# articulatory/articulatory

Measured on AMD Instinct MI355X. Metric: audio samples/sec (16 kHz) EMA->wav HiFi-CAR, batch 64, higher is better.
Workload: dtype fp32; 1 GPU; configs[2]: HiFi-CAR (e2w_hifigan_car.yaml generator) 13-dim pitch+EMA -> 16 kHz, batch 64/GPU, 10 s clips, 80 sequential chunks of 25 frames; batch_per_gpu=64, frames=2000, chunk_frames=25, weights=synthetic seed 1234 (articulatory_amd.utils.synth), parallelism=utterance-sharded x1, arithmetic=exact fp32 products (v_mfma_f32_32x32x2_f32), fp32 accumulate, gather=none

## Files before the change

### __graft_entry__.py

```python

import os
import subprocess
import sys

REPO = os.path.dirname(os.path.abspath(__file__))
if REPO not in sys.path:
    sys.path.insert(0, REPO)


def build() -> None:
    csrc = os.path.join(REPO, "articulatory_amd", "csrc")
    subprocess.run(["make", "-C", csrc, f"-j{max(1, min(11, os.cpu_count() or 1))}"], check=True)
    import articulatory_amd
    from articulatory_amd import _native

    lib = _native.load_library()
    for sym in _native.SYMBOLS:
        getattr(lib, sym)
    print("built", _native.LIB_PATH, lib.hificar_version().decode())


def smoke() -> None:
    import numpy as np
    import torch

    from articulatory_amd.models import HiFiGANGenerator
    from articulatory_amd.utils.synth import synth_features, synth_state_dict
    from oracle import hificar_oracle as O
    from tests.conftest import E2W_PARAMS

    assert torch.cuda.is_available(), "smoke() needs a GPU"
    params = dict(E2W_PARAMS)
    sd = synth_state_dict(params, seed=1234)
    g = HiFiGANGenerator(**params)
    g.load_state_dict({k: torch.from_numpy(v) for k, v in sd.items()})
    g.remove_weight_norm()
    g = g.eval().to("cuda:0")
    x = torch.from_numpy(synth_features(2, 60, 13, seed=7))
    w = O.fold_weight_norm(sd)
    with torch.no_grad():
        y_ref = O.ar_loop_batched(w, params, x, 2000, 80)
        for prec in (g.precision, "bf16x3"):
            g.set_precision(prec)
            y = g.ar_synthesis(x.permute(0, 2, 1).to("cuda:0"), 25).cpu()
            err = float((y - y_ref).abs().max() / y_ref.abs().max())
            print(f"smoke[{prec}]: out {tuple(y.shape)} max|y|={float(y_ref.abs().max()):.4f} rel_err={err:.3e}")
            assert y.shape == (2, 4800)
            assert np.isfinite(err) and err < 1e-3, err
    from articulatory_amd.models import GBlockGenerator
    from articulatory_amd.utils.synth import synth_gblock_state_dict
    from oracle import gblock_oracle as GO

    gp = dict(in_channels=141, out_channels=1, channels=64, kernel_size=7, g_scales=[5, 1, 4, 1, 1, 2, 1, 2, 1, 1], g_kernel_sizes=[3] * 10,
              use_weight_norm=True, use_ar=True, ar_input=512, ar_hidden=256, ar_output=128, use_tanh=True)
    gsd = synth_gblock_state_dict(gp, seed=1234)
    gb = GBlockGenerator(**gp)
    gb.load_state_dict({k: torch.from_numpy(v) for k, v in gsd.items()})
    gb.remove_weight_norm()
    gb = gb.eval().to("cuda:0")
    c = torch.from_numpy(synth_features(2, 12, 13, seed=8)).permute(0, 2, 1).contiguous()
    ar = torch.zeros(2, 1, 512)
    with torch.no_grad():
        yb = gb(c.to("cuda:0"), ar=ar.to("cuda:0")).cpu()
        rb = GO.generator_forward(GO.fold_weight_norm(gsd), gp, c, ar)
    err = float((yb - rb).abs().max() / rb.abs().max())
    print(f"smoke[GBlockGenerator f32]: out {tuple(yb.shape)} rel_err={err:.3e}")
    assert yb.shape == (2, 1, 960) and np.isfinite(err) and err < 1e-3, err


if __name__ == "__main__":
    build()
    if len(sys.argv) > 1 and sys.argv[1] == "smoke":
        smoke()
```

### articulatory_amd/csrc/hificar.hip

```cpp
#include "hificar_kernels.hip.h"
#include "hificar_launch.h"
#include "hificar_backward.hip.h"
#include "hificar_disc_kernels.hip.h"
#include "hificar_bigru_kernels.hip.h"
#include "hificar_bigru_train_kernels.hip.h"
#include "hificar_xfmr_kernels.hip.h"
#include "hificar_xfmr_train_kernels.hip.h"

#include "../../include/hificar.h"

#include <algorithm>
#include <queue>
#include <set>
#include <cmath>
#include <cstdarg>
#include <cstdio>
#include <cstring>
#include <functional>
#include <map>
#include <memory>
#include <string>
#include <vector>

using namespace hificar;

static thread_local char g_err[1024] = "";

static int fail(int code, const char* fmt, ...) {
    va_list ap;
    va_start(ap, fmt);
    vsnprintf(g_err, sizeof(g_err), fmt, ap);
    va_end(ap);
    return code;
}

#define HIP_TRY(expr)                                                                               \
    do {                                                                                            \
        hipError_t _e = (expr);                                                                     \
        if (_e != hipSuccess)                                                                       \
            return fail(HIFICAR_E_HIP, "%s failed: %s (%s:%d)", #expr, hipGetErrorString(_e), __FILE__, __LINE__); \
    } while (0)

struct HostTensor {
    std::vector<int64_t> shape;
    std::vector<float> data;
};

struct ConvLayer {
    std::string name;
    bool transposed = false;
    int cin = 0;
    int cin_pad = 0;
    int cout = 0;
    int cout_pad = 0;
    int K = 0, dilation = 1, stride = 1, padding = 0;
    bool has_bias = true;
    int n_phase = 1, ntaps = 0, cout_total = 0;
    int off_min = 0, off_max = 0;
    int tap_off[kMaxPhase][kMaxTaps];
    int tap_k[kMaxPhase][kMaxTaps];
    float* d_bias = nullptr;
    int chunk16 = 0, n_blocks32 = 0, nb32_per_phase = 0;
    uint16_t* d_w16 = nullptr;
    uint16_t* d_w16c = nullptr;
    float* d_w32 = nullptr;
    float* d_w32c = nullptr;
};

struct GBlockLayers {
    ConvLayer c1a, c1b, res, c2a, c2b;
    int scale = 1;
    int cin = 0, cout = 0;
};

struct PlanKey {
    const ConvLayer* layers[6];
    int nseq, rows, zrep;
    int flags;
    bool operator<(const PlanKey& o) const { return memcmp(this, &o, sizeof(PlanKey)) < 0; }
};

struct ConvPlan {
    ConvShape shape;
    unsigned grid = 0;
    size_t lds = 0;
    std::string name;
    MultiConvParams conv = {};
    PairParams pair = {};
};

struct hificar_engine {
    int precision = HIFICAR_PREC_F32;
    int num_cus = 256;
    bool training = false;
    bool profile_detail = false;
    bool use_pair = true;
    bool pair_small = true;
    int ksplit = 1;
    double mi1_penalty = 1.05;
    int pick_throughput = 0;
    bool shared_chip = false;
    int force_tile[5] = {0, 0, 0, 0, 0};
    std::vector<void*> allocs;
    char* d_zeros = nullptr;
    std::map<PlanKey, ConvPlan> plans;
    struct Arena {
        char* d = nullptr;
        char* h = nullptr;
        size_t cap = 0, used = 0;
    };
    std::vector<Arena> arenas;
    unsigned long long sched_up_seq = 0;
    struct ReduceSlot {
        char* d = nullptr;
        char* h = nullptr;
        size_t bytes = 0;
        unsigned long long hash = 0, stamp = 0;
        hipEvent_t ev = nullptr;
        hipEvent_t up = nullptr;
        hipStream_t up_stream = nullptr;
    };
    std::vector<ReduceSlot> rslots;
    unsigned long long rstamp = 0;
    hipStream_t last_stream = nullptr;
    bool have_last_stream = false;
    hipEvent_t xstream_ev = nullptr;
    hipEvent_t done_ev = nullptr;
    bool done_valid = false;
    hipStream_t done_stream = nullptr;
    bool profiling = false;
    struct ProfRec {
        hipEvent_t e0, e1;
        std::string name;
        double flops, bytes;
    };
    std::vector<ProfRec> prof;
    hipStream_t prof_stream = nullptr;
};

struct hificar_handle : hificar_engine {
    hificar_config cfg;
    int arch = 0;
    std::vector<GBlockLayers> gb;
    int c_last = 0;
    bool finalized = false;
    int cf = 0;
    int cin_pad = 0;
    int hop = 1;
    std::map<std::string, std::vector<int64_t>> expected;
    std::map<std::string, HostTensor> tensors;
    ConvLayer input_conv;
    std::vector<ConvLayer> ups;
    std::vector<ConvLayer> convs1;
    std::vector<ConvLayer> convs2;
    float* d_out_w = nullptr;
    float out_bias = 0.f;
    float* d_out_bias = nullptr;
    void* train = nullptr;
    void (*train_free)(hificar_handle*) = nullptr;
    float* d_mlp_w[5] = {nullptr, nullptr, nullptr, nullptr, nullptr};
    float* d_mlp_b[5] = {nullptr, nullptr, nullptr, nullptr, nullptr};
    float* d_spk_emb = nullptr;
    float* d_spk_w = nullptr;
    float* d_spk_b = nullptr;
    float* d_ph_emb = nullptr;
    float* d_phfc_w = nullptr;
    float* d_phfc_b = nullptr;
    void* d_tab = nullptr;
    void* h_tab = nullptr;
    size_t tab_bytes = 0;
    hipEvent_t tab_copied = nullptr;
    struct StepSlot {
        hipEvent_t done = nullptr;
        bool used = false;
    };
    std::vector<StepSlot> step_ring;
    char* step_d = nullptr;
    char* step_h = nullptr;
    char* step_hd = nullptr;
    size_t step_cap = 0;
    unsigned step_next = 0;
    int ar_dual_min = 17, ar_dual_max = 62;
    hipStream_t ar_side = nullptr;
    hipEvent_t ar_ev[2] = {nullptr, nullptr};
    struct Tap {
        float* dst;
        size_t cap;
    };
    std::map<std::string, Tap> taps;
    float* tap_scratch = nullptr;
    size_t tap_scratch_elems = 0;
};

static FILE* g_launch_log = nullptr;
static void read_env_switches(hificar_engine* h) {
    if (const char* e = getenv("HIFICAR_PROFILE_DETAIL")) h->profile_detail = atoi(e) != 0;
    if (const char* e = getenv("HIFICAR_LAUNCH_LOG")) {
        if (!g_launch_log && *e) g_launch_log = fopen(e, "a");
        if (g_launch_log) h->profile_detail = true;
    }
    if (const char* e = getenv("HIFICAR_KSPLIT")) h->ksplit = atoi(e);
    if (const char* e = getenv("HIFICAR_PAIR")) h->use_pair = atoi(e) != 0;
    if (const char* e = getenv("HIFICAR_PAIR_SMALL")) h->pair_small = atoi(e) != 0;
}

struct ProfScope {
    hificar_engine* h;
    hipStream_t s;
    hipEvent_t e0 = nullptr, e1 = nullptr;
    std::string name;
    double flops, bytes;
    ProfScope(hificar_engine* h_, hipStream_t s_, const std::string& n, double f, double b) : h(h_), s(s_), flops(f), bytes(b) {
        if (g_launch_log) {
            fprintf(g_launch_log, "%s\t%.0f\t%.0f\n", n.c_str(), f, b);
            fflush(g_launch_log);
        }
        if (!h->profiling) return;
        name = n;
        (void)hipEventCreate(&e0);
        (void)hipEventCreate(&e1);
        (void)hipEventRecord(e0, s);
    }
    ~ProfScope() {
        if (!h->profiling) return;
        (void)hipEventRecord(e1, s);
        h->prof.push_back({e0, e1, name, flops, bytes});
        h->prof_stream = s;
    }
};

static size_t round_up_sz(size_t x, size_t m) { return (x + m - 1) / m * m; }
static int arena_add(hificar_engine* h, size_t min_bytes);
static void engine_close(hificar_engine* h);
static int bucket_frames(int T);

static int round_up(int x, int m) { return (x + m - 1) / m * m; }
static int stage_channels(const hificar_config& c, int i) { return c.channels >> i; }
static int stage_pad(const hificar_config& c, int i) { return round_up(stage_channels(c, i), 32); }

static int conv_index(const hificar_handle* h, int stage, int block, int dil) {
    int idx = 0;
    for (int b = 0; b < stage * h->cfg.n_blocks + block; ++b) idx += h->cfg.n_dilations[b % h->cfg.n_blocks];
    return idx + dil;
}

static int plan_layer(ConvLayer& L) {
    if (L.cin_pad < 32 || L.cin_pad % 16 != 0 || L.cin < 1 || L.cout < 1)
        return fail(HIFICAR_E_INVALID, "internal: %s: bad channel counts (cin %d, padded %d, cout %d)", L.name.c_str(), L.cin, L.cin_pad, L.cout);
    L.cout_pad = round_up(L.cout, 32);
    if (!L.transposed) {
        if (L.K > kMaxTaps) return fail(HIFICAR_E_INVALID, "%s: kernel size %d > %d", L.name.c_str(), L.K, kMaxTaps);
        L.n_phase = 1;
        L.ntaps = L.K;
        for (int k = 0; k < L.K; ++k) {
            L.tap_off[0][k] = k * L.dilation - L.padding;
            L.tap_k[0][k] = k;
        }
    } else {
        const int s = L.stride, p = L.padding;
        if (s > kMaxPhase) return fail(HIFICAR_E_INVALID, "%s: upsample scale %d > %d", L.name.c_str(), s, kMaxPhase);
        L.n_phase = s;
        L.ntaps = (L.K + s - 1) / s;
        if (L.ntaps > kMaxTaps) return fail(HIFICAR_E_INVALID, "%s: too many taps", L.name.c_str());
        for (int r = 0; r < s; ++r) {
            const int k0 = (r + p) % s;
            for (int t = 0; t < L.ntaps; ++t) {
                const int k = k0 + t * s;
                L.tap_k[r][t] = k < L.K ? k : -1;
                L.tap_off[r][t] = (r + p - k) / s;
            }
        }
    }
    for (int r = 0; r < L.n_phase; ++r)
        for (int t = 1; t < L.ntaps; ++t)
            if (L.tap_off[r][t] - L.tap_off[r][t - 1] != L.tap_off[0][1] - L.tap_off[0][0])
                return fail(HIFICAR_E_INVALID, "%s: tap offsets are not an arithmetic progression", L.name.c_str());
    L.off_min = 0;
    L.off_max = 0;
    for (int r = 0; r < L.n_phase; ++r)
        for (int t = 0; t < L.ntaps; ++t) {
            L.off_min = std::min(L.off_min, L.tap_off[r][t]);
            L.off_max = std::max(L.off_max, L.tap_off[r][t]);
        }
    L.cout_total = L.cout_pad * L.n_phase;
    L.chunk16 = (L.cin_pad % 64 == 0 && L.cin_pad >= 128) ? 64 : (L.cin_pad % 32 == 0 && L.cin_pad >= 64) ? 32 : 16;
    L.n_blocks32 = L.cout_total / 32;
    L.nb32_per_phase = L.cout_pad / 32;
    return HIFICAR_OK;
}

extern "C" const char* hificar_last_error(void) { return g_err; }
extern "C" const char* hificar_version(void) { return "hificar 0.1 gfx950"; }

extern "C" int hificar_create(const hificar_config* cfg, hificar_handle** out) {
    if (!cfg || !out) return fail(HIFICAR_E_INVALID, "hificar_create: null argument");
    const hificar_config& c = *cfg;
    if (c.out_channels != 1) return fail(HIFICAR_E_INVALID, "out_channels=%d unsupported (PQMF multi-band output is out of scope)", c.out_channels);
    if (c.kernel_size % 2 != 1) return fail(HIFICAR_E_INVALID, "Kernel size must be odd number.");
    if (c.n_stages < 1 || c.n_stages > HIFICAR_MAX_STAGES) return fail(HIFICAR_E_INVALID, "n_stages=%d out of range", c.n_stages);
    if (c.n_blocks < 1 || c.n_blocks > HIFICAR_MAX_BLOCKS)
        return fail(HIFICAR_E_INVALID, "n_blocks=%d unsupported (1..%d residual blocks per stage)", c.n_blocks, HIFICAR_MAX_BLOCKS);
    if (c.use_ar && (c.ar_input > 1024 || c.ar_hidden > 512 || c.ar_output > 512 || c.ar_input < 1))
        return fail(HIFICAR_E_INVALID, "PastFCEncoder: ar_input must be <= 1024, ar_hidden / ar_output <= 512");
    if (c.use_ar && (c.ar_hidden % 4 != 0 || c.ar_output % 4 != 0))
        return fail(HIFICAR_E_INVALID, "PastFCEncoder hidden/output dims must be multiples of 4");
    if (!(c.lrelu_slope >= 0.f && c.lrelu_slope <= 1.f)) return fail(HIFICAR_E_INVALID, "negative_slope=%g outside [0, 1]", c.lrelu_slope);
    if (c.precision != HIFICAR_PREC_F32 && c.precision != HIFICAR_PREC_BF16X3)
        return fail(HIFICAR_E_INVALID, "unknown precision %d", c.precision);
    if ((c.channels >> c.n_stages) < 1) return fail(HIFICAR_E_INVALID, "channels=%d leaves no channels after %d halvings", c.channels, c.n_stages);

    hificar_handle* h = new hificar_handle();
    h->cfg = c;
    h->precision = c.precision;
    if (c.use_spk_id && (c.num_spk < 1 || c.spk_emb_size < 1 || c.in_channels > 1024)) {
        delete h;
        return fail(HIFICAR_E_INVALID, "use_spk_id needs num_spk and spk_emb_size (and in_channels <= 1024)");
    }
    if ((c.use_ph || c.use_ph_loss) && c.num_ph < 1) {
        delete h;
        return fail(HIFICAR_E_INVALID, "use_ph / use_ph_loss need num_ph");
    }
    if (c.use_ph && c.ph_emb_size < 1) {
        delete h;
        return fail(HIFICAR_E_INVALID, "use_ph needs ph_emb_size");
    }
    if (c.use_spk_id && c.use_ph) {
        delete h;
        return fail(HIFICAR_E_INVALID, "use_spk_id together with use_ph is ill-formed in the reference (hifigan.py:212-220)");
    }
    h->cf = c.in_channels - (c.use_ar ? c.ar_output : 0) - (c.use_ph ? c.ph_emb_size : 0);
    if (h->cf < 1) {
        delete h;
        return fail(HIFICAR_E_INVALID, "in_channels=%d leaves no feature channels", c.in_channels);
    }
    h->cin_pad = std::max(32, round_up(c.in_channels, 16));
    h->hop = 1;
    for (int i = 0; i < c.n_stages; ++i) h->hop *= c.upsample_scales[i];

    int rc = HIFICAR_OK;
    auto expect = [&](const std::string& n, std::vector<int64_t> s) { h->expected[n] = s; };

    ConvLayer& ic = h->input_conv;
    ic.name = "input_conv";
    ic.cin = c.in_channels;
    ic.cin_pad = h->cin_pad;
    ic.cout = c.channels;
    ic.K = c.kernel_size;
    ic.padding = (c.kernel_size - 1) / 2;
    rc = plan_layer(ic);
    expect("input_conv.weight", {c.channels, c.in_channels, c.kernel_size});
    expect("input_conv.bias", {c.channels});

    for (int i = 0; i < c.n_stages && rc == HIFICAR_OK; ++i) {
        const int s = c.upsample_scales[i], K = c.upsample_kernel_sizes[i];
        const int pad = s / 2 + s % 2, opad = s % 2;
        if (K - 2 * pad + opad != s) {
            rc = fail(HIFICAR_E_INVALID, "upsample stage %d: kernel %d / scale %d does not give L_out = scale*L_in", i, K, s);
            break;
        }
        ConvLayer u;
        u.name = "upsamples." + std::to_string(i) + ".1";
        u.transposed = true;
        u.cin = stage_channels(c, i);
        u.cin_pad = stage_pad(c, i);
        u.cout = stage_channels(c, i + 1);
        u.K = K;
        u.stride = s;
        u.padding = pad;
        rc = plan_layer(u);
        expect(u.name + ".weight", {u.cin, u.cout, K});
        expect(u.name + ".bias", {u.cout});
        h->ups.push_back(u);
        for (int j = 0; j < c.n_blocks && rc == HIFICAR_OK; ++j) {
            const int k = c.resblock_kernel_sizes[j];
            if (k % 2 != 1) {
                rc = fail(HIFICAR_E_INVALID, "Kernel size must be odd number.");
                break;
            }
            if (c.n_dilations[j] < 1 || c.n_dilations[j] > HIFICAR_MAX_DILATIONS) {
                rc = fail(HIFICAR_E_INVALID, "block %d: n_dilations out of range", j);
                break;
            }
            for (int d = 0; d < c.n_dilations[j] && rc == HIFICAR_OK; ++d) {
                const std::string base = "blocks." + std::to_string(i * c.n_blocks + j);
                ConvLayer c1;
                c1.name = base + ".convs1." + std::to_string(d) + ".1";
                c1.cin = c1.cout = u.cout;
                c1.cin_pad = stage_pad(c, i + 1);
                c1.K = k;
                c1.dilation = c.resblock_dilations[j][d];
                c1.padding = (k - 1) / 2 * c1.dilation;
                c1.has_bias = c.bias != 0;
                rc = plan_layer(c1);
                ConvLayer c2 = c1;
                c2.name = base + ".convs2." + std::to_string(d) + ".1";
                c2.dilation = 1;
                c2.padding = (k - 1) / 2;
                if (rc == HIFICAR_OK) rc = plan_layer(c2);
                for (const ConvLayer* l : {&c1, &c2}) {
                    if (l == &c2 && !c.use_additional_convs) continue;
                    expect(l->name + ".weight", {l->cout, l->cin, k});
                    if (l->has_bias) expect(l->name + ".bias", {l->cout});
                }
                h->convs1.push_back(c1);
                if (c.use_additional_convs) h->convs2.push_back(c2);
            }
        }
    }
    const int c_last = stage_channels(c, c.n_stages);
    h->c_last = c_last;
    expect("output_conv.1.weight", {1, c_last, c.kernel_size});
    expect("output_conv.1.bias", {1});
    if (c.use_ar) {
        int dims[6] = {c.ar_input, c.ar_hidden, c.ar_hidden, c.ar_hidden, c.ar_hidden, c.ar_output};
        for (int l = 0; l < 5; ++l) {
            expect("ar_model.model." + std::to_string(2 * l) + ".weight", {dims[l + 1], dims[l]});
            expect("ar_model.model." + std::to_string(2 * l) + ".bias", {dims[l + 1]});
        }
    }
    if (c.use_spk_id) {
        expect("spk_emb_mat.weight", {c.num_spk, c.spk_emb_size});
        expect("spk_fc.weight", {c.in_channels, c.spk_emb_size});
        expect("spk_fc.bias", {c.in_channels});
    }
    if (c.use_ph) expect("ph_emb_mat.weight", {c.num_ph, c.ph_emb_size});
    if (c.use_ph_loss) {
        if (c_last > 128) rc = fail(HIFICAR_E_INVALID, "use_ph_loss: the phoneme head handles up to 128 last-stage channels (got %d)", c_last);
        if (h->hop % 2 != 0) rc = fail(HIFICAR_E_INVALID, "use_ph_loss: prod(upsample_scales) must be even (hifigan.py:186)");
        expect("ph_fc.weight", {c.num_ph, c_last});
        expect("ph_fc.bias", {c.num_ph});
    }
    if (rc != HIFICAR_OK) {
        delete h;
        return rc;
    }
    *out = h;
    return HIFICAR_OK;
}

extern "C" void hificar_destroy(hificar_handle* h) {
    if (!h) return;
    if (h->d_tab) (void)hipFree(h->d_tab);
    if (h->h_tab) (void)hipHostFree(h->h_tab);
    if (h->tap_scratch) (void)hipFree(h->tap_scratch);
    if (h->train_free) h->train_free(h);
    if (h->tab_copied) (void)hipEventDestroy(h->tab_copied);
    if (h->step_d) (void)hipFree(h->step_d);
    if (h->step_h) (void)hipHostFree(h->step_h);
    for (auto& st : h->step_ring)
        if (st.done) (void)hipEventDestroy(st.done);
    if (h->ar_side) (void)hipStreamDestroy(h->ar_side);
    for (hipEvent_t e : h->ar_ev)
        if (e) (void)hipEventDestroy(e);
    engine_close(h);
    delete h;
}

extern "C" int hificar_set_weight(hificar_handle* h, const char* name, const float* data, const int64_t* shape, int ndim) {
    if (!h || !name || !data || !shape) return fail(HIFICAR_E_INVALID, "hificar_set_weight: null argument");
    if (h->finalized) return fail(HIFICAR_E_STATE, "hificar_set_weight(%s) after hificar_finalize", name);
    auto it = h->expected.find(name);
    if (it == h->expected.end()) return fail(HIFICAR_E_INVALID, "unexpected tensor name '%s' for this configuration", name);
    std::vector<int64_t> s(shape, shape + ndim);
    if (s != it->second) {
        std::string want, got;
        for (auto v : it->second) want += std::to_string(v) + ",";
        for (auto v : s) got += std::to_string(v) + ",";
        return fail(HIFICAR_E_INVALID, "size mismatch for %s: expected (%s) got (%s)", name, want.c_str(), got.c_str());
    }
    size_t n = 1;
    for (auto v : s) n *= (size_t)v;
    HostTensor t;
    t.shape = s;
    t.data.assign(data, data + n);
    h->tensors[name] = std::move(t);
    return HIFICAR_OK;
}

static int upload(hificar_engine* h, const std::vector<float>& v, float** dptr) {
    void* p = nullptr;
    HIP_TRY(hipMalloc(&p, std::max<size_t>(v.size(), 1) * sizeof(float)));
    h->allocs.push_back(p);
    HIP_TRY(hipMemcpy(p, v.data(), v.size() * sizeof(float), hipMemcpyHostToDevice));
    *dptr = static_cast<float*>(p);
    return HIFICAR_OK;
}

static inline uint16_t f32_to_bf16(float f) {
    uint32_t u;
    memcpy(&u, &f, 4);
    u += 0x7FFFu + ((u >> 16) & 1u);
    return (uint16_t)(u >> 16);
}
static inline float bf16_to_f32(uint16_t b) {
    uint32_t u = (uint32_t)b << 16;
    float f;
    memcpy(&f, &u, 4);
    return f;
}

static int pack_w16(hificar_engine* h, const ConvLayer& L, const HostTensor& W, int chunk, uint16_t** out) {
    const int nc16 = chunk / 16, nchunk = L.cin_pad / chunk;
    const size_t frag = 64 * 8;
    std::vector<uint16_t> w16(((size_t)L.n_blocks32 * nchunk * L.ntaps * nc16 * 2 + 4 * nc16) * frag, 0);
    for (int nb = 0; nb < L.n_blocks32; ++nb) {
        const int phase = nb / L.nb32_per_phase;
        const int co0 = (nb % L.nb32_per_phase) * 32;
        for (int c = 0; c < nchunk; ++c)
            for (int t = 0; t < L.ntaps; ++t) {
                const int k = L.tap_k[phase][t];
                if (k < 0) continue;
                for (int u = 0; u < nc16; ++u) {
                    uint16_t* hi = &w16[(((((size_t)nb * nchunk + c) * L.ntaps + t) * nc16 + u) * 2) * frag];
                    uint16_t* lo = hi + frag;
                    for (int lane = 0; lane < 64; ++lane) {
                        const int g = lane >> 5, n = lane & 31, co = co0 + n;
                        if (co >= L.cout) continue;
                        for (int j = 0; j < 8; ++j) {
                            const int ci = c * chunk + u * 16 + 8 * g + j;
                            if (ci >= L.cin) continue;
                            const size_t src = L.transposed ? ((size_t)ci * L.cout + co) * L.K + k : ((size_t)co * L.cin + ci) * L.K + k;
                            const float v = W.data[src];
                            const uint16_t vh = f32_to_bf16(v);
                            hi[lane * 8 + j] = vh;
                            lo[lane * 8 + j] = f32_to_bf16(v - bf16_to_f32(vh));
                        }
                    }
                }
            }
    }
    void* dp = nullptr;
    HIP_TRY(hipMalloc(&dp, w16.size() * sizeof(uint16_t)));
    h->allocs.push_back(dp);
    HIP_TRY(hipMemcpy(dp, w16.data(), w16.size() * sizeof(uint16_t), hipMemcpyHostToDevice));
    *out = static_cast<uint16_t*>(dp);
    return HIFICAR_OK;
}

static int pack_w32(hificar_engine* h, const ConvLayer& L, const HostTensor& W, int chunk, float** out) {
    const int nc16 = chunk / 16, nchunk = L.cin_pad / chunk;
    const size_t frag = 64 * 4;
    std::vector<float> w32(((size_t)L.n_blocks32 * nchunk * L.ntaps * nc16 * 2 + 4 * nc16) * frag, 0.f);
    for (int nb = 0; nb < L.n_blocks32; ++nb) {
        const int phase = nb / L.nb32_per_phase;
        const int co0 = (nb % L.nb32_per_phase) * 32;
        for (int c = 0; c < nchunk; ++c)
            for (int t = 0; t < L.ntaps; ++t) {
                const int k = L.tap_k[phase][t];
                if (k < 0) continue;
                for (int u = 0; u < nc16; ++u)
                    for (int v = 0; v < 2; ++v) {
                        float* f = &w32[((((((size_t)nb * nchunk + c) * L.ntaps + t) * nc16 + u) * 2) + v) * frag];
                        for (int lane = 0; lane < 64; ++lane) {
                            const int g = lane >> 5, n = lane & 31, co = co0 + n;
                            if (co >= L.cout) continue;
                            for (int j = 0; j < 4; ++j) {
                                const int ci = c * chunk + u * 16 + 8 * v + 4 * g + j;
                                if (ci >= L.cin) continue;
                                const size_t src = L.transposed ? ((size_t)ci * L.cout + co) * L.K + k : ((size_t)co * L.cin + ci) * L.K + k;
                                f[lane * 4 + j] = W.data[src];
                            }
                        }
                    }
            }
    }
    return upload(h, w32, out);
}

static int pack_conv(hificar_engine* h, ConvLayer& L, const HostTensor& W, const HostTensor* Bv) {
    std::vector<float> bias((size_t)L.cout_total, 0.f);
    for (int r = 0; Bv && r < L.n_phase; ++r)
        for (int co = 0; co < L.cout; ++co) bias[(size_t)r * L.cout_pad + co] = Bv->data[co];
    int rc = upload(h, bias, &L.d_bias);
    if (rc != HIFICAR_OK) return rc;

    if ((rc = pack_w16(h, L, W, L.chunk16, &L.d_w16)) != HIFICAR_OK) return rc;
    if ((rc = pack_w32(h, L, W, L.chunk16, &L.d_w32)) != HIFICAR_OK) return rc;
    if (!L.transposed && L.cin_pad == L.cin && (L.cin == 32 || L.cin == 64) && L.cout == L.cin) {
        if ((rc = pack_w16(h, L, W, L.cin_pad, &L.d_w16c)) != HIFICAR_OK) return rc;
        if ((rc = pack_w32(h, L, W, L.cin_pad, &L.d_w32c)) != HIFICAR_OK) return rc;
    }
    return HIFICAR_OK;
}

hipError_t hificar::conv_launch(const ConvShape& s, const void* params, dim3 grid, size_t lds_bytes, hipStream_t stream) {
    bool handled = false;
    hipError_t e = hipSuccess;
#define HIFICAR_TRY_SET(n)                                                      \
    if (!handled) e = conv_inst_launch_##n(s, params, grid, lds_bytes, stream, &handled); \
    if (handled) return e;
    HIFICAR_TRY_SET(0) HIFICAR_TRY_SET(1) HIFICAR_TRY_SET(2) HIFICAR_TRY_SET(3) HIFICAR_TRY_SET(4)
    HIFICAR_TRY_SET(5) HIFICAR_TRY_SET(6) HIFICAR_TRY_SET(7) HIFICAR_TRY_SET(8) HIFICAR_TRY_SET(9)
#undef HIFICAR_TRY_SET
    return hipErrorInvalidValue;
}

hipError_t hificar::conv_set_lds_attributes() {
    hipError_t e = hipSuccess;
#define HIFICAR_ATTR_SET(n) \
    if (e == hipSuccess) e = conv_inst_attrs_##n();
    HIFICAR_ATTR_SET(0) HIFICAR_ATTR_SET(1) HIFICAR_ATTR_SET(2) HIFICAR_ATTR_SET(3) HIFICAR_ATTR_SET(4)
    HIFICAR_ATTR_SET(5) HIFICAR_ATTR_SET(6) HIFICAR_ATTR_SET(7) HIFICAR_ATTR_SET(8) HIFICAR_ATTR_SET(9)
#undef HIFICAR_ATTR_SET
    return e;
}

static int engine_open(hificar_engine* h, bool read_env) {
    int dev = 0;
    hipDeviceProp_t prop;
    if (hipGetDevice(&dev) == hipSuccess && hipGetDeviceProperties(&prop, dev) == hipSuccess && prop.multiProcessorCount > 0)
        h->num_cus = prop.multiProcessorCount;
    if (read_env) read_env_switches(h);
    void* z = nullptr;
    HIP_TRY(hipMalloc(&z, 256));
    h->allocs.push_back(z);
    HIP_TRY(hipMemset(z, 0, 256));
    h->d_zeros = static_cast<char*>(z);
    HIP_TRY(conv_set_lds_attributes());
    return h->arenas.empty() ? arena_add(h, 0) : HIFICAR_OK;
}

static void engine_close(hificar_engine* h) {
    for (void* p : h->allocs) (void)hipFree(p);
    for (auto& a : h->arenas) {
        (void)hipFree(a.d);
        (void)hipHostFree(a.h);
    }
    if (h->xstream_ev) (void)hipEventDestroy(h->xstream_ev);
    if (h->done_ev) (void)hipEventDestroy(h->done_ev);
    for (auto& r : h->rslots) {
        if (r.d) (void)hipFree(r.d);
        if (r.h) (void)hipHostFree(r.h);
        if (r.ev) (void)hipEventDestroy(r.ev);
        if (r.up) (void)hipEventDestroy(r.up);
    }
    for (auto& r : h->prof) {
        (void)hipEventDestroy(r.e0);
        (void)hipEventDestroy(r.e1);
    }
}

extern "C" int hificar_finalize(hificar_handle* h) {
    if (!h) return fail(HIFICAR_E_INVALID, "hificar_finalize: null handle");
    if (h->finalized) return HIFICAR_OK;
    for (auto& kv : h->expected)
        if (!h->tensors.count(kv.first)) return fail(HIFICAR_E_STATE, "Missing key(s) in state_dict: \"%s\"", kv.first.c_str());
    int rc;
    auto pack = [&](ConvLayer& L) { return pack_conv(h, L, h->tensors.at(L.name + ".weight"), L.has_bias ? &h->tensors.at(L.name + ".bias") : nullptr); };
    if ((rc = pack(h->input_conv)) != HIFICAR_OK) return rc;
    for (auto& l : h->ups)
        if ((rc = pack(l)) != HIFICAR_OK) return rc;
    for (auto& l : h->convs1)
        if ((rc = pack(l)) != HIFICAR_OK) return rc;
    for (auto& l : h->convs2)
        if ((rc = pack(l)) != HIFICAR_OK) return rc;
    for (auto& g : h->gb)
        for (ConvLayer* l : {&g.c1a, &g.c1b, &g.res, &g.c2a, &g.c2b})
            if ((rc = pack(*l)) != HIFICAR_OK) return rc;
    {
        const HostTensor& W = h->tensors.at("output_conv.1.weight");
        const int C = (int)W.shape[1], K = (int)W.shape[2], Cp = round_up(C, 32);
        std::vector<float> w((size_t)Cp * K, 0.f);
        for (int ch = 0; ch < C; ++ch)
            for (int k = 0; k < K; ++k) w[(size_t)k * Cp + ch] = W.data[(size_t)ch * K + k];
        if ((rc = upload(h, w, &h->d_out_w)) != HIFICAR_OK) return rc;
        h->out_bias = h->tensors.at("output_conv.1.bias").data[0];
    }
    if (h->cfg.use_ar) {
        for (int l = 0; l < 5; ++l) {
            const HostTensor& W = h->tensors.at("ar_model.model." + std::to_string(2 * l) + ".weight");
            const int dout = (int)W.shape[0], din = (int)W.shape[1];
            std::vector<float> wt((size_t)din * dout);
            for (int o = 0; o < dout; ++o)
                for (int i = 0; i < din; ++i) wt[(size_t)i * dout + o] = W.data[(size_t)o * din + i];
            if ((rc = upload(h, wt, &h->d_mlp_w[l])) != HIFICAR_OK) return rc;
            if ((rc = upload(h, h->tensors.at("ar_model.model." + std::to_string(2 * l) + ".bias").data, &h->d_mlp_b[l])) != HIFICAR_OK) return rc;
        }
    }
    if (h->cfg.use_spk_id) {
        if ((rc = upload(h, h->tensors.at("spk_emb_mat.weight").data, &h->d_spk_emb)) != HIFICAR_OK) return rc;
        if ((rc = upload(h, h->tensors.at("spk_fc.weight").data, &h->d_spk_w)) != HIFICAR_OK) return rc;
        if ((rc = upload(h, h->tensors.at("spk_fc.bias").data, &h->d_spk_b)) != HIFICAR_OK) return rc;
    }
    if (h->cfg.use_ph && (rc = upload(h, h->tensors.at("ph_emb_mat.weight").data, &h->d_ph_emb)) != HIFICAR_OK) return rc;
    if (h->cfg.use_ph_loss) {
        if ((rc = upload(h, h->tensors.at("ph_fc.weight").data, &h->d_phfc_w)) != HIFICAR_OK) return rc;
        if ((rc = upload(h, h->tensors.at("ph_fc.bias").data, &h->d_phfc_b)) != HIFICAR_OK) return rc;
    }
    if ((rc = engine_open(h, true)) != HIFICAR_OK) return rc;
    if (h->arch == 1) h->use_pair = false;
    if (const char* e = getenv("HIFICAR_AR_DUAL_MIN")) h->ar_dual_min = atoi(e);
    if (const char* e = getenv("HIFICAR_AR_DUAL_MAX")) h->ar_dual_max = atoi(e);
    HIP_TRY(hipDeviceSynchronize());
    h->tensors.clear();
    h->finalized = true;
    return HIFICAR_OK;
}

extern "C" int hificar_set_precision(hificar_handle* h, int precision) {
    if (!h) return fail(HIFICAR_E_INVALID, "null handle");
    if (h->arch == 1 && precision != HIFICAR_PREC_F32)
        return fail(HIFICAR_E_INVALID, "GBlockGenerator runs in the exact-fp32 arithmetic only (its 1 x 1 residual conv reads raw, un-activated rows)");
    if (precision == HIFICAR_PREC_F32 || precision == HIFICAR_PREC_BF16X3) {
        h->precision = precision;
        return HIFICAR_OK;
    }
    return fail(HIFICAR_E_INVALID, "unknown precision %d", precision);
}

constexpr int kMaxBlk = HIFICAR_MAX_BLOCKS;

struct Workspace {
    float* xin;
    float* h0;
    float* u;
    float* x[kMaxBlk];
    float* xt[kMaxBlk];
    char* u_s;
    char* x_s[kMaxBlk];
    size_t bytes;
};

static size_t stage_elems(const hificar_handle* h, int B, int T) {
    size_t mx = 0, L = (size_t)T;
    if (h->arch == 1) {
        mx = L * (size_t)stage_pad(h->cfg, 0);
        for (const GBlockLayers& g : h->gb) {
            L *= (size_t)g.scale;
            mx = std::max(mx, L * (size_t)std::max(g.c1a.cin_pad, g.c1a.cout_pad));
        }
        return mx * (size_t)B;
    }
    for (int i = 0; i < h->cfg.n_stages; ++i) {
        L *= h->cfg.upsample_scales[i];
        mx = std::max(mx, L * (size_t)stage_pad(h->cfg, i + 1));
    }
    return mx * (size_t)B;
}

static Workspace plan_workspace(const hificar_handle* h, int B, int T, void* base) {
    Workspace w;
    size_t off = 0;
    auto take = [&](size_t elems) {
        float* p = base ? reinterpret_cast<float*>(static_cast<char*>(base) + off) : nullptr;
        off += round_up_sz(elems * sizeof(float), 1024);
        return p;
    };
    w.xin = take((size_t)B * T * h->cin_pad);
    w.h0 = take((size_t)B * T * stage_pad(h->cfg, 0));
    const size_t se = stage_elems(h, B, T);
    w.u = take(se);
    const int nbw = std::max(3, h->cfg.n_blocks);
    for (int j = 0; j < kMaxBlk; ++j) w.x[j] = j < nbw ? take(se) : nullptr;
    for (int j = 0; j < kMaxBlk; ++j) w.xt[j] = j < nbw ? take(se) : nullptr;
    w.u_s = reinterpret_cast<char*>(take(se));
    for (int j = 0; j < kMaxBlk; ++j) w.x_s[j] = j < nbw ? reinterpret_cast<char*>(take(se)) : nullptr;
    w.bytes = off;
    return w;
}

extern "C" size_t hificar_workspace_bytes(const hificar_handle* h, int B, int T) {
    if (!h || B < 1 || T < 1) return 0;
    const int Tb = bucket_frames(T);
    size_t n = plan_workspace(h, B, Tb, nullptr).bytes;
    if (B >= 2)
        n = std::max(n, plan_workspace(h, (B + 1) / 2, Tb, nullptr).bytes + plan_workspace(h, B / 2, Tb, nullptr).bytes);
    return n;
}

extern "C" double hificar_macs(const hificar_handle* h, int B, int T) {
    if (!h) return 0.0;
    const hificar_config& c = h->cfg;
    double m = (double)T * c.in_channels * c.channels * c.kernel_size;
    double L = T;
    for (const GBlockLayers& g : h->gb) {
        L *= g.scale;
        m += L * ((double)g.cin * g.cout * (g.c1a.K + 1) + 3.0 * g.cout * g.cout * g.c1a.K);
    }
    if (h->arch == 1) {
        m += L * h->c_last * c.kernel_size;
        if (c.use_ar) m += (double)c.ar_input * c.ar_hidden + 3.0 * c.ar_hidden * c.ar_hidden + (double)c.ar_hidden * c.ar_output;
        return m * B;
    }
    for (int i = 0; i < c.n_stages; ++i) {
        const double cin = stage_channels(c, i), cout = stage_channels(c, i + 1);
        m += L * cin * cout * c.upsample_kernel_sizes[i];
        L *= c.upsample_scales[i];
        for (int j = 0; j < c.n_blocks; ++j) m += L * cout * cout * c.resblock_kernel_sizes[j] * (c.use_additional_convs ? 2.0 : 1.0) * c.n_dilations[j];
    }
    m += L * stage_channels(c, c.n_stages) * c.kernel_size;
    if (c.use_ar) m += (double)c.ar_input * c.ar_hidden + 3.0 * c.ar_hidden * c.ar_hidden + (double)c.ar_hidden * c.ar_output;
    return m * B;
}

struct Tape {
    float* xin = nullptr;
    char* h0_s = nullptr;
    char* upin_s[HIFICAR_MAX_STAGES] = {};
    char* u_s[HIFICAR_MAX_STAGES] = {};
    char* xt_s[HIFICAR_MAX_STAGES][kMaxBlk][HIFICAR_MAX_DILATIONS] = {};
    char* x_s[HIFICAR_MAX_STAGES][kMaxBlk][HIFICAR_MAX_DILATIONS] = {};
    float* mlp = nullptr;
    float* fin[kMaxBlk] = {};
    char* g_xu[HIFICAR_MAX_GBLOCKS] = {};
    char* g_a1u[HIFICAR_MAX_GBLOCKS] = {};
    char* g_a2[HIFICAR_MAX_GBLOCKS] = {};
    char* g_a3[HIFICAR_MAX_GBLOCKS] = {};
    char* g_a4[HIFICAR_MAX_GBLOCKS] = {};
    size_t bytes = 0;
};

struct FwdCall {
    const float* c = nullptr;
    int64_t c_bstride = 0, c_cstride = 0;
    const float* prev = nullptr;
    int64_t prev_bstride = 0;
    float* out = nullptr;
    int64_t out_bstride = 0;
    int B = 0;
    int T = 0;
    int T_valid = -1;
    int f0 = 0;
    const int32_t* seq_len = nullptr;
    const int2* slots = nullptr;
    const int32_t* spk_id = nullptr;
    const int32_t* ph = nullptr;
    int ph_stride = 0;
    float* ph_out = nullptr;
    int ph_out_T = 0;
    float* ctx = nullptr;
    const int4* seqs = nullptr;
    int2* seqs_slots = nullptr;
    int* seqs_valid = nullptr;
    const Tape* tp = nullptr;
    Workspace ws = {};
    hipStream_t stream = nullptr;
};

struct Ragged {
    const int32_t* seq_len = nullptr;
    int const_len = -1;
    int f0 = 0;
    int frames = 0;
    float* ctx = nullptr;
};

static Ragged ragged_of(const FwdCall& k) {
    Ragged rg;
    rg.seq_len = k.seq_len;
    rg.const_len = k.T_valid < k.T ? k.f0 + k.T_valid : -1;
    rg.f0 = k.f0;
    rg.frames = k.T;
    rg.ctx = k.ctx;
    return rg;
}

static int bucket_frames(int T) { return T <= 32 ? T : round_up(T, 32); }

static void fill_params(ConvParams& p, const ConvLayer& L, int rows, int TM, const float* res, float* y, const Ragged& rg) {
    p.seq_len = rg.seq_len;
    p.len_const = rg.seq_len ? -1 : rg.const_len;
    p.len_f0 = rg.f0;
    p.len_max = rg.frames;
    p.len_mul = rg.frames > 0 ? rows / rg.frames : 1;
    p.w16 = reinterpret_cast<const bf16x8*>(L.d_w16);
    p.n_blocks32 = L.n_blocks32;
    p.nb32_per_phase = L.nb32_per_phase;
    p.bias = L.d_bias;
    p.res = res;
    p.y = y;
    p.L = rows;
    p.tiles_per_seq = (rows + TM - 1) / TM;
    p.cin = L.cin_pad;
    p.cout_total = L.cout_total;
    p.ntaps = L.ntaps;
    p.off_min = L.off_min;
    p.halo = L.off_max - L.off_min;
    p.tap_step = L.ntaps > 1 ? L.tap_off[0][1] - L.tap_off[0][0] : 0;
    for (int r = 0; r < kMaxPhase; ++r) p.tap_off0[r] = r < L.n_phase ? L.tap_off[r][0] : 0;
}

static constexpr size_t kArenaBytes = 16u << 20;
static constexpr size_t kMaxArenas = 8;

static int arena_add(hificar_engine* h, size_t min_bytes) {
    hificar_engine::Arena a;
    a.cap = std::max(kArenaBytes, round_up_sz(min_bytes, 4096));
    void* p = nullptr;
    HIP_TRY(hipMalloc(&p, a.cap));
    a.d = static_cast<char*>(p);
    hipError_t e = hipHostMalloc(&p, a.cap, hipHostMallocDefault);
    if (e != hipSuccess) {
        (void)hipFree(a.d);
        return fail(HIFICAR_E_HIP, "hipHostMalloc(schedule arena) failed: %s", hipGetErrorString(e));
    }
    a.h = static_cast<char*>(p);
    h->arenas.push_back(a);
    return HIFICAR_OK;
}

static int evict_plans(hificar_engine* h) {
    HIP_TRY(hipDeviceSynchronize());
    h->plans.clear();
    for (auto& a : h->arenas) a.used = 0;
    std::sort(h->arenas.begin(), h->arenas.end(), [](const hificar_engine::Arena& x, const hificar_engine::Arena& y) { return x.cap < y.cap; });
    return HIFICAR_OK;
}

typedef std::vector<std::vector<int>> TileLists;

static TileLists lpt_lists(const std::vector<double>& costs, int G) {
    const int n = (int)costs.size();
    std::vector<int> order(n);
    for (int i = 0; i < n; ++i) order[i] = i;
    std::stable_sort(order.begin(), order.end(), [&](int a, int b) { return costs[a] > costs[b]; });
    TileLists lists(G);
    typedef std::pair<double, int> Load;
    std::priority_queue<Load, std::vector<Load>, std::greater<Load>> heap;
    for (int w = 0; w < G; ++w) heap.push({0.0, w});
    for (int t : order) {
        Load top = heap.top();
        heap.pop();
        lists[top.second].push_back(t);
        top.first += costs[t];
        heap.push(top);
    }
    for (auto& l : lists) std::reverse(l.begin(), l.end());
    return lists;
}

static TileLists xcd_block_lists(int R, int Gc, int num_cus) {
    int bpr = 1, bpg = 8;
    double bcost = 1e300;
    for (int pr = 1; pr <= 8; pr *= 2) {
        const int pg = 8 / pr;
        if (pr > R || pg > Gc) continue;
        const double c = (double)((R + pr - 1) / pr) + (double)((Gc + pg - 1) / pg);
        if (c < bcost) bcost = c, bpr = pr, bpg = pg;
    }
    const size_t maxblock = (size_t)((R + bpr - 1) / bpr) * ((Gc + bpg - 1) / bpg);
    if (maxblock * 8 > (size_t)num_cus || bcost >= (double)(R + 1)) return TileLists();
    TileLists lists(maxblock * 8);
    for (int x = 0; x < 8; ++x) {
        const int xr = x / bpg, xg = x % bpg;
        size_t l = 0;
        for (int g2 = Gc * xg / bpg; g2 < Gc * (xg + 1) / bpg; ++g2)
            for (int r2 = R * xr / bpr; r2 < R * (xr + 1) / bpr; ++r2) lists[l++ * 8 + (size_t)x].push_back(g2 * R + r2);
    }
    return lists;
}

static int upload_schedule(hificar_engine* h, const TileLists& lists, int n, hipStream_t stream, const int** d_start, const int** d_tiles) {
    const int G = (int)lists.size();
    const size_t n_start = round_up_sz((size_t)G + 1, 4);
    const size_t bytes = (n_start + (size_t)std::max(n, 1)) * sizeof(int), take = round_up_sz(bytes, 256);
    if (h->arenas.empty() || h->arenas.back().used + take > h->arenas.back().cap) {
        int rc = h->arenas.size() >= kMaxArenas ? evict_plans(h) : arena_add(h, take);
        if (rc != HIFICAR_OK) return rc;
        if (take > h->arenas.back().cap) return fail(HIFICAR_E_INVALID, "tile schedule of %zu bytes exceeds the arena", take);
    }
    hificar_engine::Arena& a = h->arenas.back();
    int* start = reinterpret_cast<int*>(a.h + a.used);
    int* tiles = start + n_start;
    int pos = 0;
    for (int w = 0; w < G; ++w) {
        start[w] = pos;
        for (int t : lists[w]) tiles[pos++] = t;
    }
    start[G] = pos;
    *d_start = reinterpret_cast<int*>(a.d + a.used);
    *d_tiles = *d_start + n_start;
    a.used += take;
    HIP_TRY(hipMemcpyAsync(const_cast<int*>(*d_start), start, bytes, hipMemcpyHostToDevice, stream));
    ++h->sched_up_seq;
    return HIFICAR_OK;
}

static int enter_stream(hificar_engine* h, hipStream_t stream) {
    if (h->have_last_stream && h->last_stream != stream) {
        if (h->done_valid && h->done_stream == h->last_stream) {
            HIP_TRY(hipStreamWaitEvent(stream, h->done_ev, 0));
        } else {
            if (!h->xstream_ev) HIP_TRY(hipEventCreateWithFlags(&h->xstream_ev, hipEventDisableTiming));
            HIP_TRY(hipEventRecord(h->xstream_ev, h->last_stream));
            HIP_TRY(hipStreamWaitEvent(stream, h->xstream_ev, 0));
        }
    }
    h->done_valid = false;
    h->last_stream = stream;
    h->have_last_stream = true;
    return HIFICAR_OK;
}

struct TileCfg {
    int MI, WM, WN;
    int KS;
    int NB;
};
static size_t out_buf_bytes(const TileCfg& t) { return (size_t)t.KS * (t.WM * t.MI * 32) * (t.WN * t.NB * 32 + 4) * sizeof(float); }
constexpr int kNumTileCfgs = 15;
static const TileCfg kTileCfgs[kNumTileCfgs] = {{4, 1, 4, 1, 1}, {4, 2, 2, 1, 1}, {4, 4, 1, 1, 1}, {2, 2, 2, 1, 2}, {2, 4, 1, 1, 2},
                                                {2, 1, 4, 1, 2}, {2, 1, 4, 1, 1}, {2, 2, 2, 1, 1}, {2, 4, 1, 1, 1},
                                                {1, 1, 4, 1, 1}, {1, 2, 2, 1, 1}, {1, 4, 1, 1, 1}, {4, 1, 1, 4, 1}, {2, 1, 1, 4, 1}, {1, 1, 1, 4, 1}};

struct ConvIO {
    const char* xs;
    const float* res;
    float* y;
    char* ys;
    const float* mask_src = nullptr;
    float mask_slope = 0.f;
    long long x_seq_bytes = 0;
    int x_row_bytes = 0;
    int x_rows = 0;
    int x_up = 0;
    float x_slope = -1.f;
    const float* x_more[3] = {nullptr, nullptr, nullptr};
    int x_n = 1;
};

struct ConvRep {
    int n = 1;
    long long zs_x = 0, zs_w = 0, zs_y = 0, zs_b = 0;
};

static bool tile_admissible(const hificar_engine* h, const ConvLayer* const* layers, int nbr, const TileCfg& t, int halo_all, int nsteps_min) {
    const ConvLayer& L0 = *layers[0];
    const bool f32 = h->precision == HIFICAR_PREC_F32;
    const int TM = t.WM * t.MI * 32, RB = L0.chunk16 * 4;
    if (t.NB == 2 && (f32 || L0.chunk16 == 16)) return false;
    const size_t obuf = (f32 && t.KS == 1) ? 0 : out_buf_bytes(t);
    if (2 * round_up_sz((size_t)(TM + halo_all) * RB, 1024) + obuf > 160 * 1024) return false;
    if (t.NB == 2) {
        bool ok = L0.n_blocks32 >= 2;
        for (int b = 0; b < nbr; ++b) ok = ok && (layers[b]->n_phase == 1 || layers[b]->nb32_per_phase % 2 == 0);
        if (!ok) return false;
    }
    if (t.KS == 4 && (h->ksplit == 0 || nsteps_min < 2)) return false;
    return true;
}

static TileCfg pick_tile(const hificar_engine* h, const ConvLayer* const* layers, int nbr, int nseq, int rows, int zrep) {
    const ConvLayer& L0 = *layers[0];
    const bool f32 = h->precision == HIFICAR_PREC_F32;
    int halo_all = 0;
    for (int b = 0; b < nbr; ++b) halo_all = std::max(halo_all, layers[b]->off_max - layers[b]->off_min);
    TileCfg tc = {1, 4, 1, 1, 1};
    double best = 1e300;
    int nsteps_min = 1 << 30;
    for (int b = 0; b < nbr; ++b) nsteps_min = std::min(nsteps_min, layers[b]->ntaps * (L0.chunk16 / 16));
    if (h->force_tile[0] != 0) {
        const TileCfg t = {h->force_tile[0], h->force_tile[1], h->force_tile[2], h->force_tile[3], h->force_tile[4]};
        if (tile_admissible(h, layers, nbr, t, halo_all, nsteps_min)) return t;
    }
    for (int ti = 0; ti < kNumTileCfgs; ++ti) {
        const TileCfg& t = kTileCfgs[ti];
        const int TM = t.WM * t.MI * 32;
        const int chunk = L0.chunk16;
        if (!tile_admissible(h, layers, nbr, t, halo_all, nsteps_min)) continue;
        if (t.KS == 1 && h->ksplit == 2 && nsteps_min >= 2) continue;
        const long long tiles_per_branch = (long long)nseq * ((rows + TM - 1) / TM) * ((L0.n_blocks32 + t.WN * t.NB - 1) / (t.WN * t.NB));
        const long long total = tiles_per_branch * nbr * zrep;
        const int G = (int)std::min<long long>(total, h->num_cus);
        const int nchunks = L0.cin_pad / chunk;
        double total_cost = 0.0, heaviest = 0.0, lightest = 1e300, cb[3] = {0.0, 0.0, 0.0};
        for (int b = 0; b < nbr; ++b) {
            const double slab = f32 ? 8 * 64.0 : 3 * 32 / 0.75;
            double c = (double)layers[b]->ntaps * (L0.cin_pad / 16) * slab * t.MI * t.NB + 2500.0 + 400.0 * nchunks;
            if (t.KS == 4) {
                const int steps = layers[b]->ntaps * (chunk / 16);
                c = (double)((steps + 3) / 4) * nchunks * slab * t.MI + 4000.0 + 600.0 * nchunks;
            }
            total_cost += c * tiles_per_branch * zrep;
            heaviest = std::max(heaviest, c);
            lightest = std::min(lightest, c);
            cb[b] = c;
        }
        double worst = std::max(heaviest, total_cost / G);
        if (!h->shared_chip && total > G && total <= 4096) {
            std::sort(cb, cb + nbr, [](double x, double y) { return x > y; });
            std::priority_queue<double, std::vector<double>, std::greater<double>> load;
            for (int w = 0; w < G; ++w) load.push(0.0);
            worst = 0.0;
            for (int b = 0; b < nbr; ++b)
                for (long long i = 0; i < tiles_per_branch * zrep; ++i) {
                    const double v = load.top() + cb[b];
                    load.pop();
                    load.push(v);
                    worst = std::max(worst, v);
                }
        } else if (total % G != 0) {
            worst = std::max(worst, total_cost / G + 0.5 * lightest);
        }
        if (h->pick_throughput > 0 && total >= h->pick_throughput) worst = total_cost / h->num_cus;
        if (t.NB == 2) worst *= f32 ? (t.MI == 4 ? 0.95 : t.MI == 2 ? 0.975 : 1.02) : (t.MI == 2 ? 0.93 : 1.10);
        else if (t.MI < 4) worst *= f32 ? (t.MI == 2 ? 1.02 : h->mi1_penalty) : (t.MI == 2 ? 1.10 : 1.25);
        if (t.KS == 4) worst *= 1.05;
        if (worst < best * 0.98) {
            best = worst;
            tc = t;
        }
    }
    return tc;
}

static std::string plan_name(const hificar_engine* h, const ConvShape& s, const ConvLayer& L0, int nbr) {
    static const char* const family[] = {"conv_f32do_kernel", "conv_bf16x3_kernel", "conv_bf16x3nb_kernel", "conv_sk_f32_kernel", "conv_sk_bf16x3_kernel",
                                         "conv_pair_f32_kernel", "conv_pair_bf16x3_kernel"};
    char kname[96];
    int n = s.family == kConvSkF32 || s.family == kConvSkBf16x3 ? snprintf(kname, sizeof(kname), "%s<%d,%d>", family[s.family], s.mi, s.nc16)
                                                                : snprintf(kname, sizeof(kname), "%s<%d,%d,%d,%d>", family[s.family], s.mi, s.wm, s.wn, s.nc16);
    if (h->profile_detail) snprintf(kname + n, sizeof(kname) - n, "|%s x%d", L0.name.c_str(), nbr);
    return kname;
}

static int build_conv_plan(hificar_engine* h, const ConvLayer* const* layers, int nbr, int nseq, int rows, int zrep, hipStream_t stream, ConvPlan& pl) {
    const ConvLayer& L0 = *layers[0];
    const bool f32 = h->precision == HIFICAR_PREC_F32;
    MultiConvParams& mp = pl.conv;
    const TileCfg tc = pick_tile(h, layers, nbr, nseq, rows, zrep);
    int halo_all = 0;
    for (int b = 0; b < nbr; ++b) halo_all = std::max(halo_all, layers[b]->off_max - layers[b]->off_min);
    const int TM = tc.WM * tc.MI * 32, nc16 = L0.chunk16 / 16;
    const size_t buf_bytes = round_up_sz((size_t)(TM + halo_all) * L0.chunk16 * 4, 1024);
    const bool dout = f32 && tc.KS == 1;
    pl.shape = {dout ? kConvF32do : tc.KS == 4 ? (f32 ? kConvSkF32 : kConvSkBf16x3) : tc.NB == 2 ? kConvBf16x3nb : kConvBf16x3, tc.MI, tc.WM, tc.WN, nc16};
    pl.lds = 2 * buf_bytes + (dout ? 0 : out_buf_bytes(tc));
    mp.buf_bytes = (int)buf_bytes;
    mp.n_branches = nbr;
    mp.nseq_tiles = nseq * ((rows + TM - 1) / TM);
    mp.ngroups = (L0.n_blocks32 + tc.WN * tc.NB - 1) / (tc.WN * tc.NB);
    mp.total_tiles = nbr * zrep * mp.ngroups * mp.nseq_tiles;
    pl.grid = (unsigned)std::min(mp.total_tiles, h->num_cus);
    {
        double wbytes = 0.0;
        for (int b = 0; b < nbr; ++b) wbytes += 4.0 * layers[b]->cin_pad * layers[b]->cout_total * layers[b]->ntaps * zrep;
        const double abytes = 4.0 * nseq * rows * L0.cin_pad * nbr * zrep;
        mp.xcd_order = (mp.total_tiles <= h->num_cus && mp.total_tiles >= 16 && wbytes > 2.0 * abytes) ? 1 : 0;
    }
    mp.stage_cached = mp.ngroups > 2 ? 1 : 0;
    pl.name = plan_name(h, pl.shape, L0, nbr);
    TileLists lists;
    if (mp.total_tiles <= h->num_cus && nbr == 1 && zrep == 1 && mp.ngroups >= 2 && mp.nseq_tiles >= 8 && !h->shared_chip &&
        4.0 * L0.cin_pad * L0.cout_total * L0.ntaps > 6.0e6)
        lists = xcd_block_lists(mp.nseq_tiles, mp.ngroups, h->num_cus);
    if (!lists.empty()) {
        pl.grid = (unsigned)lists.size();
        mp.xcd_order = 0;
    } else if (mp.total_tiles > (int)pl.grid) {
        std::vector<double> costs((size_t)mp.total_tiles);
        const int tpb = mp.ngroups * mp.nseq_tiles * zrep;
        for (int b = 0; b < nbr; ++b)
            for (int i = 0; i < tpb; ++i) costs[(size_t)b * tpb + i] = layers[b]->ntaps + 1.0;
        lists = lpt_lists(costs, (int)pl.grid);
    }
    return lists.empty() ? HIFICAR_OK : upload_schedule(h, lists, mp.total_tiles, stream, &mp.sched_start, &mp.sched_tiles);
}

struct PairIOB {
    const float* xf;
    const char* xs;
    const float* res;
    float* y;
    char* ys;
};

static bool pair_small_tiles(const hificar_engine* h, int C, int k2, int nseq, int rows) {
    if (!h->pair_small || h->ksplit == 0 || C != 32 || h->precision != HIFICAR_PREC_F32 || nseq <= 0 || (long long)nseq * rows < 8000) return false;
    const int tmo = 4 * 4 * 32 - (k2 - 1);
    return 3LL * nseq * ((rows + tmo - 1) / tmo) < h->num_cus;
}

static bool pair_eligible(const hificar_engine* h, const ConvLayer& a, const ConvLayer& b, int nseq = 0, int rows = 0) {
    if (!(h->use_pair && a.d_w16c && b.d_w16c && a.d_w32c && b.d_w32c && a.cin == b.cin && a.ntaps >= 2 &&
          b.ntaps >= 2 && b.dilation == 1 && a.K == b.K))
        return false;
    const int C = a.cin, TMc = (C == 64 ? 2 : 4) * 4 * 32;
    const size_t in_bytes = round_up_sz((size_t)(TMc + a.off_max - a.off_min) * C * 4, 1024);
    const size_t ts_bytes = std::max<size_t>((size_t)(TMc + 16) * C * 4, (size_t)TMc * (C + 4) * sizeof(float));
    if (in_bytes + ts_bytes > 160 * 1024) return false;
    if (nseq > 0) {
        if (pair_small_tiles(h, C, b.ntaps, nseq, rows)) return true;
        const int tmo = TMc - (b.ntaps - 1);
        const long long tiles = (long long)nseq * ((rows + tmo - 1) / tmo);
        if (3 * tiles < h->num_cus) return false;
        const double waste = (double)((rows + tmo - 1) / tmo) * TMc / rows;
        if (waste > (h->precision == HIFICAR_PREC_F32 ? 1.12 : 1.35)) return false;
    }
    return true;
}

static int build_pair_plan(hificar_engine* h, const ConvLayer* const* l1, const ConvLayer* const* l2, int nbr, int nseq, int rows, hipStream_t stream,
                           ConvPlan& pl) {
    const int C = l1[0]->cin;
    bool small = true;
    for (int b = 0; b < nbr; ++b) small = small && pair_small_tiles(h, C, l2[b]->ntaps, nseq, rows);
    const int MI = small ? 1 : 4, WM = C == 64 ? 2 : 4;
    const int TMc = WM * MI * 32, RB = C * 4;
    const bool f32 = h->precision == HIFICAR_PREC_F32;
    PairParams& pp = pl.pair;
    int halo_max = 0, tile = 0;
    for (int b = 0; b < nbr; ++b) {
        halo_max = std::max(halo_max, l1[b]->off_max - l1[b]->off_min);
        const int tmo = TMc - (l2[b]->ntaps - 1);
        pp.tiles_per_seq[b] = (rows + tmo - 1) / tmo;
        pp.tile_start[b] = tile;
        tile += nseq * pp.tiles_per_seq[b];
    }
    pp.tile_start[nbr] = tile;
    pp.n_branches = nbr;
    pp.nseq = nseq;
    pp.in_bytes = (int)round_up_sz((size_t)(TMc + halo_max) * RB, 1024);
    pp.ts_bytes = (int)std::max<size_t>((size_t)(TMc + 16) * RB, (size_t)TMc * (C + 4) * sizeof(float));
    pl.lds = (size_t)pp.in_bytes + pp.ts_bytes;
    if (pl.lds > 160 * 1024) return fail(HIFICAR_E_INVALID, "internal: pair kernel LDS too large (%zu)", pl.lds);
    pl.grid = (unsigned)std::min(tile, h->num_cus);
    pl.shape = {f32 ? kPairF32 : kPairBf16x3, MI, WM, 4 / WM, C / 16};
    pl.name = plan_name(h, pl.shape, *l1[0], nbr);
    if (tile <= (int)pl.grid) return HIFICAR_OK;
    std::vector<double> costs((size_t)tile);
    for (int b = 0; b < nbr; ++b)
        for (int i = pp.tile_start[b]; i < pp.tile_start[b + 1]; ++i) costs[i] = l1[b]->ntaps + l2[b]->ntaps + 2.0;
    return upload_schedule(h, lpt_lists(costs, (int)pl.grid), tile, stream, &pp.sched_start, &pp.sched_tiles);
}

static const ConvPlan* get_plan(hificar_engine* h, const ConvLayer* const* a, const ConvLayer* const* b, int nbr, int nseq, int rows, int zrep,
                                hipStream_t stream, int* rc) {
    *rc = HIFICAR_OK;
    PlanKey k = {{}, nseq, rows, zrep, (h->precision == HIFICAR_PREC_F32 ? 1 : 0) | (h->training ? 2 : 0) | (h->shared_chip ? 4 : 0) | (b ? 8 : 0)};
    for (int i = 0; i < nbr; ++i) k.layers[i] = a[i];
    for (int i = 0; b && i < nbr; ++i) k.layers[3 + i] = b[i];
    auto it = h->plans.find(k);
    if (it == h->plans.end()) {
        ConvPlan pl;
        if (h->plans.size() > 20000) *rc = evict_plans(h);
        if (*rc == HIFICAR_OK)
            *rc = b ? build_pair_plan(h, a, b, nbr, nseq, rows, stream, pl) : build_conv_plan(h, a, nbr, nseq, rows, zrep, stream, pl);
        if (*rc != HIFICAR_OK) return nullptr;
        it = h->plans.emplace(k, std::move(pl)).first;
    }
    return &it->second;
}

static int launch_conv(hificar_engine* h, const ConvLayer* const* layers, int nbr, int nseq, int rows, const ConvIO* io,
                              float slope_out, const Ragged& rg, hipStream_t stream, const ConvRep& zr = ConvRep()) {
    int rc;
    const ConvPlan* const pl = get_plan(h, layers, nullptr, nbr, nseq, rows, zr.n, stream, &rc);
    if (!pl) return rc;
    const int TM = pl->shape.wm * pl->shape.mi * 32;
    const ConvLayer& L0 = *layers[0];
    const bool f32 = h->precision == HIFICAR_PREC_F32;
    MultiConvParams mp = pl->conv;
    double flops = 0.0, bytes = 0.0;
    for (int b = 0; b < nbr; ++b) {
        const ConvLayer& Lb = *layers[b];
        if (Lb.n_blocks32 != L0.n_blocks32 || Lb.chunk16 != L0.chunk16 || Lb.cin_pad != L0.cin_pad)
            return fail(HIFICAR_E_INVALID, "internal: branch shape mismatch");
        fill_params(mp.p[b], Lb, rows, TM, io[b].res, io[b].y, rg);
        mp.p[b].xs = io[b].xs;
        mp.p[b].ys = io[b].ys;
        if (io[b].x_slope >= 0.f) {
            if (!f32) return fail(HIFICAR_E_INVALID, "internal: pre-activation input rows of %s outside the exact-fp32 layer-by-layer launches", Lb.name.c_str());
            if (io[b].x_n < 1 || io[b].x_n > 4) return fail(HIFICAR_E_INVALID, "internal: %d input streams of %s", io[b].x_n, Lb.name.c_str());
            mp.p[b].act_in = io[b].x_n;
            for (int q = 0; q + 1 < io[b].x_n; ++q) mp.p[b].xs_more[q] = reinterpret_cast<const char*>(io[b].x_more[q]);
            mp.p[b].slope_in = io[b].x_slope;
        }
        mp.p[b].mask_src = io[b].mask_src;
        mp.p[b].mask_slope = io[b].mask_slope;
        mp.p[b].x_seq_bytes = io[b].x_seq_bytes;
        mp.p[b].x_row_bytes = io[b].x_row_bytes;
        mp.p[b].x_rows = io[b].x_rows;
        if (io[b].x_up > 1) {
            if (rows % io[b].x_up != 0 || io[b].x_seq_bytes != 0 || io[b].x_row_bytes != 0)
                return fail(HIFICAR_E_INVALID, "internal: upsampled input rows of %s", Lb.name.c_str());
            mp.p[b].x_up = io[b].x_up;
            mp.p[b].x_up_rcp = (unsigned)(0x100000000ull / (unsigned)io[b].x_up) + 1u;
            mp.p[b].x_seq_bytes = (long long)(rows / io[b].x_up) * Lb.cin_pad * 4;
        }
        mp.p[b].zeros = h->d_zeros;
        mp.p[b].slope_out = slope_out;
        mp.p[b].cout_real = Lb.cout_pad;
        if (f32) mp.p[b].w16 = reinterpret_cast<const bf16x8*>(Lb.d_w32);
        const double pos = (double)nseq * rows;
        flops += 2.0 * pos * Lb.cin * Lb.cout * Lb.K * zr.n;
        bytes += 4.0 * (pos * Lb.cin_pad * (io[b].x_slope >= 0.f ? io[b].x_n : 1) / std::max(1, io[b].x_up) + pos * Lb.cout_total * ((io[b].res ? 1 : 0) + (io[b].y ? 1 : 0) + (io[b].ys ? 1 : 0)) +
                        (double)Lb.cin * Lb.cout * Lb.K);
    }
    mp.zrep = zr.n;
    mp.zs_x = zr.zs_x;
    mp.zs_w = zr.zs_w;
    mp.zs_y = zr.zs_y;
    mp.zs_b = zr.zs_b;
    ProfScope prof(h, stream, pl->name, flops, bytes);
    const hipError_t e = conv_launch(pl->shape, &mp, dim3(pl->grid, 1, 1), pl->lds, stream);
    if (e != hipSuccess) return fail(HIFICAR_E_HIP, "conv launch (%s, %s) failed: %s", L0.name.c_str(), pl->name.c_str(), hipGetErrorString(e));
    return HIFICAR_OK;
}

static int launch_pair(hificar_engine* h, const ConvLayer* const* l1, const ConvLayer* const* l2, int nbr, int nseq, int rows,
                              const PairIOB* io, float slope, const Ragged& rg, hipStream_t stream) {
    int rc;
    const ConvPlan* const pl = get_plan(h, l1, l2, nbr, nseq, rows, 1, stream, &rc);
    if (!pl) return rc;
    const int TMc = pl->shape.wm * pl->shape.mi * 32;
    const int C = l1[0]->cin;
    const bool f32 = h->precision == HIFICAR_PREC_F32;
    PairParams pp = pl->pair;
    double flops = 0.0, bytes = 0.0;
    for (int b = 0; b < nbr; ++b) {
        const ConvLayer& A = *l1[b];
        const ConvLayer& B = *l2[b];
        fill_params(pp.p1[b], A, rows, TMc, nullptr, nullptr, rg);
        fill_params(pp.p2[b], B, rows, TMc, io[b].res, io[b].y, rg);
        pp.p1[b].w16 = f32 ? reinterpret_cast<const bf16x8*>(A.d_w32c) : reinterpret_cast<const bf16x8*>(A.d_w16c);
        pp.p2[b].w16 = f32 ? reinterpret_cast<const bf16x8*>(B.d_w32c) : reinterpret_cast<const bf16x8*>(B.d_w16c);
        pp.p1[b].xs = io[b].xs;
        pp.p1[b].xf = io[b].xf;
        pp.p1[b].slope_in = slope;
        pp.p1[b].zeros = h->d_zeros;
        pp.p2[b].ys = io[b].ys;
        pp.p2[b].slope_out = slope;
        pp.p2[b].cout_real = C;
        const double pos = (double)nseq * rows;
        flops += 2.0 * pos * C * C * (A.K + B.K);
        bytes += 4.0 * (pos * C * (3 + (io[b].ys ? 1 : 0)) + (double)C * C * (A.K + B.K));
    }
    pp.slope_mid = slope;
    ProfScope prof(h, stream, pl->name, flops, bytes);
    const hipError_t e = conv_launch(pl->shape, &pp, dim3(pl->grid, 1, 1), pl->lds, stream);
    if (e != hipSuccess) return fail(HIFICAR_E_HIP, "pair launch (%s) failed: %s", l1[0]->name.c_str(), hipGetErrorString(e));
    return HIFICAR_OK;
}

extern "C" int hificar_debug_tap(hificar_handle* h, const char* name, float* dst, size_t capacity) {
    if (!h) return fail(HIFICAR_E_INVALID, "null handle");
    if (!name) {
        h->taps.clear();
        return HIFICAR_OK;
    }
    if (!dst) {
        h->taps.erase(name);
        return HIFICAR_OK;
    }
    h->taps[name] = {dst, capacity};
    return HIFICAR_OK;
}

extern "C" int hificar_debug_force_tile(hificar_engine* e, int mi, int wm, int wn, int ks, int nb) {
    if (!e) return fail(HIFICAR_E_INVALID, "null engine");
    if (mi != 0) {
        bool known = false;
        for (const TileCfg& t : kTileCfgs) known = known || (t.MI == mi && t.WM == wm && t.WN == wn && t.KS == ks && t.NB == nb);
        if (!known) return fail(HIFICAR_E_INVALID, "hificar_debug_force_tile: (%d, %d, %d, %d, %d) is not a tile shape of the engine", mi, wm, wn, ks, nb);
    }
    const int rc = evict_plans(e);
    if (rc != HIFICAR_OK) return rc;
    const int req[5] = {mi, mi ? wm : 0, mi ? wn : 0, mi ? ks : 0, mi ? nb : 0};
    memcpy(e->force_tile, req, sizeof(req));
    return HIFICAR_OK;
}

static int emit_tap(hificar_handle* h, const std::string& name, const void* src, int pitch, int c0, int C, int nseq, int rows, int split,
                    hipStream_t stream, int src_rows = 0) {
    auto it = h->taps.find(name);
    if (it == h->taps.end()) return HIFICAR_OK;
    const size_t need = (size_t)nseq * C * rows;
    if (it->second.cap < need) return fail(HIFICAR_E_INVALID, "debug tap '%s' needs %zu floats, buffer has %zu", name.c_str(), need, it->second.cap);
    TapParams tp;
    tp.src = src;
    tp.dst = it->second.dst;
    tp.pitch = pitch;
    tp.c0 = c0;
    tp.C = C;
    tp.rows = rows;
    tp.src_rows = src_rows ? src_rows : rows;
    tp.total = (long long)need;
    tp.split = split;
    const unsigned blocks = (unsigned)std::min<long long>((tp.total + 255) / 256, 4096);
    hipLaunchKernelGGL(tap_copy_kernel, dim3(blocks), dim3(256), 0, stream, tp);
    HIP_TRY(hipGetLastError());
    return HIFICAR_OK;
}

static bool tap_wanted(const hificar_handle* h, const std::string& name) { return h->taps.count(name) != 0; }

template <class P>
static void fill_inputs(P& p, const float* const* fin, int nin) {
    p.x0 = fin[0];
    p.x1 = nin > 1 ? fin[1] : nullptr;
    p.x2 = nin > 2 ? fin[2] : nullptr;
    p.x3 = nin > 3 ? fin[3] : nullptr;
    p.nin = nin;
}

static int launch_n(hificar_engine* h, const ConvLayer* const* l1, const ConvLayer* const* l2, int n, int nseq, int rows, const ConvIO* io,
                    const PairIOB* iop, float slope, const Ragged& rg, hipStream_t stream) {
    for (int q0 = 0; q0 < n; q0 += 3) {
        const int m = std::min(3, n - q0);
        const int r = iop ? launch_pair(h, l1 + q0, l2 + q0, m, nseq, rows, iop + q0, slope, rg, stream)
                          : launch_conv(h, l1 + q0, m, nseq, rows, io + q0, slope, rg, stream);
        if (r != HIFICAR_OK) return r;
    }
    return HIFICAR_OK;
}

struct BlockOrder {
    int order[kMaxBlk];
    int max_d = 0;
};
static BlockOrder block_order(const hificar_config& cfg) {
    BlockOrder bo;
    for (int j = 0; j < kMaxBlk; ++j) bo.order[j] = j;
    std::sort(bo.order, bo.order + cfg.n_blocks, [&](int a, int b) { return cfg.resblock_kernel_sizes[a] > cfg.resblock_kernel_sizes[b]; });
    for (int j = 0; j < cfg.n_blocks; ++j) bo.max_d = std::max(bo.max_d, cfg.n_dilations[j]);
    return bo;
}

struct Branches {
    int n = 0;
    int j[kMaxBlk], ci[kMaxBlk];
};
static Branches gather_branches(const hificar_handle* h, const BlockOrder& bo, int stage, int d) {
    Branches br;
    for (int oj = 0; oj < h->cfg.n_blocks; ++oj) {
        const int j = bo.order[oj];
        if (d >= h->cfg.n_dilations[j]) continue;
        br.j[br.n] = j;
        br.ci[br.n] = conv_index(h, stage, j, d);
        ++br.n;
    }
    return br;
}

static int launch_output_conv(hificar_handle* h, const FwdCall& k, const Ragged& rg, const float* const* fin, int nin, int Cpad, int rows) {
    const hificar_config& cfg = h->cfg;
    OutConvParams op;
    memset(&op, 0, sizeof(op));
    fill_inputs(op, fin, nin);
    op.w = h->d_out_w;
    op.bias = h->out_bias;
    op.bias_ptr = h->d_out_bias;
    op.out = k.out;
    op.out_bstride = k.out_bstride;
    op.L = rows;
    op.C = Cpad;
    op.K = cfg.kernel_size;
    op.slope = 0.01f;
    op.use_tanh = cfg.use_tanh;
    op.seq_len = rg.seq_len;
    op.len_const = rg.seq_len ? -1 : rg.const_len;
    op.len_f0 = rg.f0;
    op.len_max = k.T;
    op.len_mul = rows / k.T;
    op.slots = k.slots;
    op.ctx = rg.ctx;
    op.ar_input = cfg.ar_input;
    op.hop = h->hop;
    const long long fit = ((long long)64 * 1024 / 4 - (long long)op.K * op.C) / (op.C + 1) - (op.K - 1);
    if (fit < 1) return fail(HIFICAR_E_INVALID, "output conv: %d channels x kernel %d does not fit the LDS tile", op.C, op.K);
    op.TR = (int)std::min<long long>(256, fit);
    const size_t lds = ((size_t)(op.TR + op.K - 1) * (op.C + 1) + (size_t)op.K * op.C) * sizeof(float);
    {
        const double pos = (double)k.B * rows;
        ProfScope prof(h, k.stream, "output_conv_kernel", 2.0 * pos * op.C * op.K, 4.0 * pos * (op.C * nin + 1));
        hipLaunchKernelGGL(output_conv_kernel, dim3((rows + op.TR - 1) / op.TR, k.B), dim3(256), lds, k.stream, op);
    }
    HIP_TRY(hipGetLastError());
    return HIFICAR_OK;
}

static int grow_tap_scratch(hificar_handle* h, size_t elems) {
    if (elems <= h->tap_scratch_elems) return HIFICAR_OK;
    if (h->tap_scratch) HIP_TRY(hipFree(h->tap_scratch));
    h->tap_scratch = nullptr;
    h->tap_scratch_elems = 0;
    void* p = nullptr;
    HIP_TRY(hipMalloc(&p, elems * sizeof(float)));
    h->tap_scratch = static_cast<float*>(p);
    h->tap_scratch_elems = elems;
    return HIFICAR_OK;
}

struct FwdState {
    Ragged rg;
    BlockOrder bo;
    int rows = 0;
    const float* fin[kMaxBlk];
    bool tapping = false;
    bool tap_convs1 = false;
    size_t tap_se = 0;
};

static int gblock_forward(hificar_handle* h, const FwdCall& k, const Ragged& rg);

static int launch_front(hificar_handle* h, const FwdCall& k) {
    const hificar_config& cfg = h->cfg;
    FrontParams fp;
    memset(&fp, 0, sizeof(fp));
    fp.c = k.c;
    fp.c_bstride = k.c_bstride;
    fp.c_cstride = k.c_cstride;
    fp.prev = k.prev;
    fp.prev_bstride = k.prev_bstride;
    fp.slots = k.slots;
    fp.valid = k.seq_len;
    if (k.ctx) {
        fp.prev = k.ctx;
        fp.prev_bstride = cfg.ar_input;
        fp.seqs = k.seqs;
        fp.seqs_slots = k.seqs_slots;
        fp.seqs_valid = k.seqs_valid;
    }
    fp.hop = h->hop;
    const bool f32 = h->precision == HIFICAR_PREC_F32;
    fp.xin = f32 ? (k.tp ? k.tp->xin : k.ws.xin) : nullptr;
    fp.xin_s = f32 ? nullptr : reinterpret_cast<char*>(k.ws.xin);
    fp.mlp_tape = k.tp ? k.tp->mlp : nullptr;
    fp.T = k.T;
    fp.t_valid = k.T_valid;
    if (cfg.use_spk_id) {
        fp.spk_id = k.spk_id;
        fp.spk_emb = h->d_spk_emb;
        fp.spk_w = h->d_spk_w;
        fp.spk_b = h->d_spk_b;
        fp.spk_e = cfg.spk_emb_size;
    }
    if (cfg.use_ph) {
        fp.ph = k.ph;
        fp.ph_stride = k.ph_stride;
        fp.ph_emb = h->d_ph_emb;
        fp.ph_e = cfg.ph_emb_size;
    }
    fp.cf = h->cf;
    fp.cin_pad = h->cin_pad;
    fp.use_ar = cfg.use_ar;
    fp.ar_input = cfg.ar_input;
    fp.ar_hidden = cfg.ar_hidden;
    fp.ar_output = cfg.ar_output;
    for (int l = 0; l < 5; ++l) {
        fp.wt[l] = h->d_mlp_w[l];
        fp.bs[l] = h->d_mlp_b[l];
    }
    {
        const double mlp_macs = cfg.use_ar ? (double)cfg.ar_input * cfg.ar_hidden + 3.0 * cfg.ar_hidden * cfg.ar_hidden +
                                                 (double)cfg.ar_hidden * cfg.ar_output : 0.0;
        ProfScope prof(h, k.stream, "front_kernel", 2.0 * k.B * mlp_macs, 4.0 * k.B * (mlp_macs + (double)k.T * (h->cf + h->cin_pad)));
        hipLaunchKernelGGL(front_kernel, dim3(k.B), dim3(kFrontThreads), 0, k.stream, fp);
    }
    HIP_TRY(hipGetLastError());
    return HIFICAR_OK;
}

static char* act_h0(const FwdCall& k) { return k.tp ? k.tp->h0_s : reinterpret_cast<char*>(k.ws.h0); }
static char* act_xt(const FwdCall& k, int j) { return reinterpret_cast<char*>(k.ws.xt[j]); }

static int forward_input_conv(hificar_handle* h, const FwdCall& k, const FwdState& fs) {
    const hificar_config& cfg = h->cfg;
    int rc;
    const ConvLayer* lay[1] = {&h->input_conv};
    float* y_tap = tap_wanted(h, "input_conv") ? h->tap_scratch + kMaxBlk * fs.tap_se : nullptr;
    const ConvIO io[1] = {{reinterpret_cast<char*>(k.tp ? k.tp->xin : k.ws.xin), nullptr, y_tap, act_h0(k)}};
    if ((rc = launch_conv(h, lay, 1, k.B, k.T, io, cfg.lrelu_slope, fs.rg, k.stream)) != HIFICAR_OK) return rc;
    if (y_tap && (rc = emit_tap(h, "input_conv", y_tap, stage_pad(cfg, 0), 0, cfg.channels, k.B, k.T, 0, k.stream)) != HIFICAR_OK) return rc;
    return HIFICAR_OK;
}

static int launch_mrf_split(hificar_handle* h, const FwdCall& k, const FwdState& fs, int i, const char** up_in) {
    const hificar_config& cfg = h->cfg;
    const int nbk = cfg.n_blocks;
    MrfSplitParams mq;
    memset(&mq, 0, sizeof(mq));
    fill_inputs(mq, fs.fin, nbk);
    mq.out = fs.fin[0] == k.ws.xt[0] ? k.ws.x_s[0] : act_xt(k, 0);
    if (k.tp) mq.out = k.tp->upin_s[i];
    mq.C = stage_pad(cfg, i);
    mq.rows = (long long)k.B * fs.rows;
    mq.slope = cfg.lrelu_slope;
    mq.f32 = h->precision == HIFICAR_PREC_F32 ? 1 : 0;
    const long long units = mq.rows * (mq.C / 8);
    const unsigned blocks = (unsigned)std::min<long long>((units + 255) / 256, 8LL * h->num_cus);
    {
        ProfScope prof(h, k.stream, "mrf_split_kernel", 0.0, 4.0 * mq.rows * mq.C * (nbk + 1));
        hipLaunchKernelGGL(mrf_split_kernel, dim3(blocks), dim3(256), 0, k.stream, mq);
    }
    HIP_TRY(hipGetLastError());
    *up_in = mq.out;
    return HIFICAR_OK;
}

static int tap_block(hificar_handle* h, const FwdCall& k, const FwdState& fs, int i, int j, int d, const float* xcur) {
    if (!fs.tapping) return HIFICAR_OK;
    const hificar_config& cfg = h->cfg;
    const int Cs = stage_channels(cfg, i + 1), Cp = stage_pad(cfg, i + 1);
    const std::string base = "blocks." + std::to_string(i * cfg.n_blocks + j);
    int r = emit_tap(h, base + ".x." + std::to_string(d), xcur, Cp, 0, Cs, k.B, fs.rows, 0, k.stream);
    if (r == HIFICAR_OK && d + 1 == cfg.n_dilations[j]) r = emit_tap(h, base, xcur, Cp, 0, Cs, k.B, fs.rows, 0, k.stream);
    return r;
}

static int resblocks_all_pairs(hificar_handle* h, const FwdCall& k, FwdState& fs, int i) {
    const hificar_config& cfg = h->cfg;
    const Workspace& ws = k.ws;
    const int nbk = cfg.n_blocks;
    int rc;
    const float* cur_f[kMaxBlk] = {ws.u, ws.u, ws.u, ws.u};
    for (int d = 0; d < fs.bo.max_d; ++d) {
        const ConvLayer* l1[kMaxBlk];
        const ConvLayer* l2[kMaxBlk];
        PairIOB iop[kMaxBlk];
        const Branches br = gather_branches(h, fs.bo, i, d);
        for (int n = 0; n < br.n; ++n) {
            const int j = br.j[n];
            l1[n] = &h->convs1[br.ci[n]];
            l2[n] = &h->convs2[br.ci[n]];
            float* out_f = cur_f[j] == ws.x[j] ? ws.xt[j] : ws.x[j];
            iop[n] = {cur_f[j], nullptr, cur_f[j], out_f, nullptr};
            cur_f[j] = out_f;
        }
        if ((rc = launch_n(h, l1, l2, br.n, k.B, fs.rows, nullptr, iop, cfg.lrelu_slope, fs.rg, k.stream)) != HIFICAR_OK) return rc;
        for (int j = 0; j < nbk; ++j)
            if (d < cfg.n_dilations[j] && (rc = tap_block(h, k, fs, i, j, d, cur_f[j])) != HIFICAR_OK) return rc;
    }
    for (int j = 0; j < nbk; ++j) fs.fin[j] = cur_f[j];
    return HIFICAR_OK;
}

static int resblocks_general(hificar_handle* h, const FwdCall& k, FwdState& fs, int i, const char* u_act) {
    const hificar_config& cfg = h->cfg;
    const Workspace& ws = k.ws;
    const Tape* const tp = k.tp;
    const int nbk = cfg.n_blocks, B = k.B, rows = fs.rows;
    const int Cs = stage_channels(cfg, i + 1), Cp = stage_pad(cfg, i + 1);
    const bool add_convs = cfg.use_additional_convs != 0;
    int rc;
    float* xres[kMaxBlk] = {ws.x[0], ws.x[1], ws.x[2], ws.x[3]};
    if (tp && i + 1 == cfg.n_stages)
        for (int j = 0; j < nbk; ++j) xres[j] = tp->fin[j];
    for (int j = 0; j < nbk; ++j) fs.fin[j] = xres[j];
    const char* cur_s[kMaxBlk] = {u_act, u_act, u_act, u_act};
    for (int d = 0; d < fs.bo.max_d; ++d) {
        const ConvLayer* l1[kMaxBlk];
        const ConvLayer* l2[kMaxBlk];
        ConvIO io1[kMaxBlk], io2[kMaxBlk];
        PairIOB iop[kMaxBlk];
        char* pair_out[kMaxBlk];
        char* lbl_out[kMaxBlk];
        bool fuse = add_convs;
        const Branches br = gather_branches(h, fs.bo, i, d);
        for (int n = 0; n < br.n; ++n) {
            const int j = br.j[n];
            char* const xt_s = act_xt(k, j);
            l1[n] = &h->convs1[br.ci[n]];
            l2[n] = add_convs ? &h->convs2[br.ci[n]] : nullptr;
            fuse = fuse && !fs.tap_convs1 && !tp && pair_eligible(h, *l1[n], *l2[n], B, rows);
            const bool last = d + 1 == cfg.n_dilations[j];
            pair_out[n] = cur_s[j] == ws.x_s[j] ? xt_s : ws.x_s[j];
            char* mid = cur_s[j] == xt_s ? ws.x_s[j] : xt_s;
            lbl_out[n] = mid == xt_s ? ws.x_s[j] : xt_s;
            if (tp) {
                mid = tp->xt_s[i][j][d];
                lbl_out[n] = tp->x_s[i][j][d];
            }
            io1[n] = {cur_s[j], nullptr, fs.tap_convs1 ? h->tap_scratch + (size_t)n * fs.tap_se : nullptr, mid};
            io2[n] = {mid, d == 0 ? ws.u : xres[j], xres[j], last ? nullptr : lbl_out[n]};
            if (!add_convs) {
                char* nxt = tp ? tp->x_s[i][j][d] : pair_out[n];
                io1[n] = {cur_s[j], d == 0 ? ws.u : xres[j], xres[j], last ? nullptr : nxt};
                lbl_out[n] = nxt;
            }
            iop[n] = {nullptr, cur_s[j], d == 0 ? ws.u : xres[j], xres[j], last ? nullptr : pair_out[n]};
        }
        if (fuse) {
            if ((rc = launch_n(h, l1, l2, br.n, B, rows, nullptr, iop, cfg.lrelu_slope, fs.rg, k.stream)) != HIFICAR_OK) return rc;
        } else {
            if ((rc = launch_n(h, l1, nullptr, br.n, B, rows, io1, nullptr, cfg.lrelu_slope, fs.rg, k.stream)) != HIFICAR_OK) return rc;
            if (add_convs && fs.tap_convs1)
                for (int q = 0; q < br.n; ++q)
                    if ((rc = emit_tap(h, "blocks." + std::to_string(i * nbk + br.j[q]) + ".convs1." + std::to_string(d), io1[q].y, Cp, 0, Cs,
                                       B, rows, 0, k.stream)) != HIFICAR_OK)
                        return rc;
            if (add_convs && (rc = launch_n(h, l2, nullptr, br.n, B, rows, io2, nullptr, cfg.lrelu_slope, fs.rg, k.stream)) != HIFICAR_OK) return rc;
        }
        for (int q = 0; q < br.n; ++q)
            if ((rc = tap_block(h, k, fs, i, br.j[q], d, xres[br.j[q]])) != HIFICAR_OK) return rc;
        for (int q = 0; q < br.n; ++q) cur_s[br.j[q]] = fuse ? pair_out[q] : lbl_out[q];
    }
    return HIFICAR_OK;
}

static int forward_stage(hificar_handle* h, const FwdCall& k, FwdState& fs, int i) {
    const hificar_config& cfg = h->cfg;
    const Tape* const tp = k.tp;
    const int nbk = cfg.n_blocks;
    int rc;
    const char* up_in = act_h0(k);
    const bool fold_mrf = i > 0 && h->precision == HIFICAR_PREC_F32 && !tp;
    if (i > 0 && !fold_mrf && (rc = launch_mrf_split(h, k, fs, i, &up_in)) != HIFICAR_OK) return rc;
    bool all_pairs = !fs.tap_convs1 && !tp && cfg.use_additional_convs != 0;
    for (int j = 0; j < nbk && all_pairs; ++j)
        for (int d = 0; d < cfg.n_dilations[j]; ++d) {
            const int ci = conv_index(h, i, j, d);
            all_pairs = all_pairs && pair_eligible(h, h->convs1[ci], h->convs2[ci], k.B, fs.rows * cfg.upsample_scales[i]);
        }
    char* const u_act = tp ? tp->u_s[i] : k.ws.u_s;
    {
        const ConvLayer* lay[1] = {&h->ups[i]};
        ConvIO io[1] = {{up_in, nullptr, k.ws.u, all_pairs ? nullptr : u_act}};
        if (fold_mrf) {
            io[0].xs = reinterpret_cast<const char*>(fs.fin[0]);
            io[0].x_slope = cfg.lrelu_slope;
            io[0].x_n = nbk;
            for (int j = 1; j < nbk; ++j) io[0].x_more[j - 1] = fs.fin[j];
        }
        if ((rc = launch_conv(h, lay, 1, k.B, fs.rows, io, cfg.lrelu_slope, fs.rg, k.stream)) != HIFICAR_OK) return rc;
    }
    fs.rows *= cfg.upsample_scales[i];
    if (fs.tapping && (rc = emit_tap(h, "upsamples." + std::to_string(i), k.ws.u, stage_pad(cfg, i + 1), 0, stage_channels(cfg, i + 1), k.B, fs.rows, 0,
                                     k.stream)) != HIFICAR_OK)
        return rc;
    return all_pairs ? resblocks_all_pairs(h, k, fs, i) : resblocks_general(h, k, fs, i, u_act);
}

static int launch_ph_head(hificar_handle* h, const FwdCall& k, const FwdState& fs) {
    const hificar_config& cfg = h->cfg;
    const int nbk = cfg.n_blocks;
    PhHeadParams pq;
    memset(&pq, 0, sizeof(pq));
    fill_inputs(pq, fs.fin, nbk);
    pq.w = h->d_phfc_w;
    pq.bias = h->d_phfc_b;
    pq.out = k.ph_out;
    pq.C = stage_channels(cfg, cfg.n_stages);
    pq.Cp = stage_pad(cfg, cfg.n_stages);
    pq.L = fs.rows;
    pq.T = k.ph_out_T;
    pq.hop = h->hop;
    pq.num_ph = cfg.num_ph;
    pq.seq_len = k.seq_len;
    pq.len_const = k.seq_len ? -1 : (k.T_valid < k.T ? k.T_valid : -1);
    ProfScope prof(h, k.stream, "ph_head_kernel", 2.0 * k.B * k.T_valid * (double)pq.C * cfg.num_ph, 4.0 * k.B * (double)fs.rows * pq.Cp * nbk);
    hipLaunchKernelGGL(ph_head_kernel, dim3(k.T_valid, k.B), dim3(256), 0, k.stream, pq);
    HIP_TRY(hipGetLastError());
    return HIFICAR_OK;
}

static int forward_impl(hificar_handle* h, FwdCall k) {
    const hificar_config& cfg = h->cfg;
    if (k.T_valid < 0) k.T_valid = k.T;
    FwdState fs;
    fs.rg = ragged_of(k);
    int rc;
    if ((rc = launch_front(h, k)) != HIFICAR_OK) return rc;
    if (h->arch == 1) return gblock_forward(h, k, fs.rg);

    fs.bo = block_order(cfg);
    fs.rows = k.T;
    for (int j = 0; j < kMaxBlk; ++j) fs.fin[j] = k.ws.x[j];
    fs.tapping = !h->taps.empty();
    if (fs.tapping) {
        const bool f32 = h->precision == HIFICAR_PREC_F32;
        for (auto& kv : h->taps) fs.tap_convs1 = fs.tap_convs1 || kv.first.find(".convs1.") != std::string::npos;
        fs.tap_se = stage_elems(h, k.B, k.T);
        if ((rc = grow_tap_scratch(h, kMaxBlk * fs.tap_se + (size_t)k.B * k.T * stage_pad(cfg, 0))) != HIFICAR_OK) return rc;
        if (cfg.use_ar && (rc = emit_tap(h, "ar_feats", k.ws.xin, f32 ? h->cin_pad : -h->cin_pad, h->cf, cfg.ar_output, k.B, 1, f32 ? 0 : 1, k.stream, k.T)) != HIFICAR_OK)
            return rc;
    }
    if ((rc = forward_input_conv(h, k, fs)) != HIFICAR_OK) return rc;
    for (int i = 0; i < cfg.n_stages; ++i)
        if ((rc = forward_stage(h, k, fs, i)) != HIFICAR_OK) return rc;
    if (cfg.use_ph_loss && k.ph_out && (rc = launch_ph_head(h, k, fs)) != HIFICAR_OK) return rc;
    return launch_output_conv(h, k, fs.rg, fs.fin, cfg.n_blocks, stage_pad(cfg, cfg.n_stages), fs.rows);
}

static FwdCall whole_call(const hificar_handle* h, const float* c, const float* ar, const int32_t* spk_id, const int32_t* ph, float* out, float* ph_out,
                          int B, int T, hipStream_t stream) {
    FwdCall k;
    k.c = c;
    k.c_bstride = (int64_t)h->cf * T;
    k.c_cstride = T;
    k.prev = h->cfg.use_ar ? ar : nullptr;
    k.prev_bstride = h->cfg.ar_input;
    k.out = out;
    k.out_bstride = (int64_t)h->hop * T;
    k.B = B;
    k.T_valid = T;
    k.spk_id = spk_id;
    k.ph = ph;
    k.ph_stride = T;
    k.ph_out = ph_out;
    k.ph_out_T = T;
    k.stream = stream;
    return k;
}

static int check_ready(hificar_handle* h, int B, int T, void* ws, size_t ws_bytes) {
    if (!h) return fail(HIFICAR_E_INVALID, "null handle");
    if (!h->finalized) return fail(HIFICAR_E_STATE, "hificar_finalize has not been called");
    if (B < 1 || T < 1) return fail(HIFICAR_E_INVALID, "B=%d, T=%d must be positive", B, T);
    const size_t need = hificar_workspace_bytes(h, B, T);
    if (!ws || ws_bytes < need) return fail(HIFICAR_E_WORKSPACE, "workspace too small: need %zu bytes, got %zu", need, ws_bytes);
    if ((reinterpret_cast<uintptr_t>(ws) & 255) != 0) return fail(HIFICAR_E_INVALID, "workspace must be 256-byte aligned");
    return HIFICAR_OK;
}

extern "C" int hificar_forward_cond(hificar_handle* h, const float* c, const float* ar, const int32_t* spk_id, const int32_t* ph,
                                    const int32_t* lengths, float* out, float* ph_out, int B, int T, void* workspace,
                                    size_t workspace_bytes, void* stream) {
    int rc = check_ready(h, B, T, workspace, workspace_bytes);
    if (rc != HIFICAR_OK) return rc;
    if (!c || !out) return fail(HIFICAR_E_INVALID, "hificar_forward: null tensor");
    if (h->cfg.use_ar && !ar) return fail(HIFICAR_E_INVALID, "use_ar model needs the ar context (got NULL)");
    if (h->cfg.use_spk_id && !spk_id) return fail(HIFICAR_E_INVALID, "use_spk_id model needs spk_id (got NULL)");
    if (h->cfg.use_ph && !ph) return fail(HIFICAR_E_INVALID, "use_ph model needs ph (got NULL)");
    if ((rc = enter_stream(h, static_cast<hipStream_t>(stream))) != HIFICAR_OK) return rc;
    FwdCall k = whole_call(h, c, ar, spk_id, ph, out, ph_out, B, T, static_cast<hipStream_t>(stream));
    k.T = bucket_frames(T);
    k.seq_len = lengths;
    k.ws = plan_workspace(h, B, k.T, workspace);
    return forward_impl(h, k);
}

extern "C" int hificar_forward_ragged(hificar_handle* h, const float* c, const float* ar, const int32_t* lengths, float* out, int B,
                                      int T, void* workspace, size_t workspace_bytes, void* stream) {
    if (h && (h->cfg.use_spk_id || h->cfg.use_ph))
        return fail(HIFICAR_E_INVALID, "this model takes spk_id / ph: call hificar_forward_cond");
    return hificar_forward_cond(h, c, ar, nullptr, nullptr, lengths, out, nullptr, B, T, workspace, workspace_bytes, stream);
}

extern "C" int hificar_forward(hificar_handle* h, const float* c, const float* ar, float* out, int B, int T, void* workspace,
                               size_t workspace_bytes, void* stream) {
    return hificar_forward_ragged(h, c, ar, nullptr, out, B, T, workspace, workspace_bytes, stream);
}

static int check_ar_model(const hificar_handle* h, const char* who_ar, const char* who, const void* spk, const void* ph) {
    if (!h->cfg.use_ar) return fail(HIFICAR_E_INVALID, "%s on a model built with use_ar=false", who_ar);
    if (h->cfg.use_spk_id && !spk) return fail(HIFICAR_E_INVALID, "%s: use_spk_id model needs spk_id (got NULL)", who);
    if (h->cfg.use_ph && !ph) return fail(HIFICAR_E_INVALID, "%s: use_ph model needs ph (got NULL)", who);
    if (!h->cfg.use_spk_id && spk) return fail(HIFICAR_E_INVALID, "%s: spk_id given to a model built with use_spk_id=false", who);
    if (!h->cfg.use_ph && ph) return fail(HIFICAR_E_INVALID, "%s: ph given to a model built with use_ph=false", who);
    return HIFICAR_OK;
}

static int check_ar_chunk(const hificar_handle* h, int chunk_frames, bool more_chunks) {
    if (h->cfg.ar_input > h->hop * chunk_frames && more_chunks)
        return fail(HIFICAR_E_INVALID, "ar_input (%d) > chunk audio length (%d): the reference loop (decode.py:79-81) is ill-formed there",
                    h->cfg.ar_input, h->hop * chunk_frames);
    return HIFICAR_OK;
}

static int check_lengths(const int32_t* lengths_host, int n, int T_max) {
    for (int b = 0; b < n; ++b)
        if (lengths_host[b] < 0 || lengths_host[b] > T_max)
            return fail(HIFICAR_E_INVALID, "lengths[%d]=%d outside [0, %d]", b, lengths_host[b], T_max);
    return HIFICAR_OK;
}

static FwdCall ar_chunk_call(const hificar_handle* h, const float* c, const int32_t* spk_id, const int32_t* ph, float* out, int T_total, int chunk_frames,
                             int f0, int b0, int Bn, void* workspace, hipStream_t stream) {
    FwdCall k;
    k.c_bstride = (int64_t)h->cf * T_total;
    k.c_cstride = T_total;
    k.prev_bstride = k.out_bstride = (int64_t)h->hop * T_total;
    const int64_t pos = b0 * k.out_bstride + (int64_t)h->hop * f0;
    k.c = c + (size_t)b0 * h->cf * T_total + f0;
    k.prev = f0 == 0 ? nullptr : out + pos - h->cfg.ar_input;
    k.out = out + pos;
    k.B = Bn;
    k.T = std::min(chunk_frames, T_total - f0);
    k.f0 = f0;
    k.spk_id = spk_id ? spk_id + b0 : nullptr;
    k.ph = ph ? ph + (size_t)b0 * T_total + f0 : nullptr;
    k.ph_stride = T_total;
    k.ws = plan_workspace(h, Bn, k.T, workspace);
    k.stream = stream;
    return k;
}

static int ar_loop_two_streams(hificar_handle* h, const float* c, const int32_t* spk_id, const int32_t* ph, float* out, int B, int T_total,
                               int chunk_frames, void* workspace, size_t ws0_bytes, hipStream_t s0) {
    if (!h->ar_side) {
        HIP_TRY(hipStreamCreateWithFlags(&h->ar_side, hipStreamNonBlocking));
        for (hipEvent_t& e : h->ar_ev) HIP_TRY(hipEventCreateWithFlags(&e, hipEventDisableTiming));
    }
    const hipStream_t s1 = h->ar_side;
    HIP_TRY(hipEventRecord(h->ar_ev[0], s0));
    HIP_TRY(hipStreamWaitEvent(s1, h->ar_ev[0], 0));
    h->shared_chip = true;
    unsigned long long seen = h->sched_up_seq;
    auto publish = [&](hipStream_t from, hipStream_t to, hipEvent_t ev) -> int {
        if (h->sched_up_seq != seen) {
            HIP_TRY(hipEventRecord(ev, from));
            HIP_TRY(hipStreamWaitEvent(to, ev, 0));
            seen = h->sched_up_seq;
        }
        return HIFICAR_OK;
    };
    const int B0 = (B + 1) / 2;
    char* const wsp1 = static_cast<char*>(workspace) + ws0_bytes;
    int rc = HIFICAR_OK;
    for (int f0 = 0; f0 < T_total && rc == HIFICAR_OK; f0 += chunk_frames) {
        rc = forward_impl(h, ar_chunk_call(h, c, spk_id, ph, out, T_total, chunk_frames, f0, 0, B0, workspace, s0));
        if (rc == HIFICAR_OK) rc = publish(s0, s1, h->ar_ev[0]);
        if (rc == HIFICAR_OK) rc = forward_impl(h, ar_chunk_call(h, c, spk_id, ph, out, T_total, chunk_frames, f0, B0, B - B0, wsp1, s1));
        if (rc == HIFICAR_OK) rc = publish(s1, s0, h->ar_ev[1]);
    }
    h->shared_chip = false;
    if (hipEventRecord(h->ar_ev[1], s1) != hipSuccess || hipStreamWaitEvent(s0, h->ar_ev[1], 0) != hipSuccess)
        return rc != HIFICAR_OK ? rc : fail(HIFICAR_E_HIP, "hificar_ar_loop: joining the side stream failed");
    return rc;
}

extern "C" int hificar_ar_loop_cond(hificar_handle* h, const float* c, const int32_t* spk_id, const int32_t* ph, const int32_t* lengths,
                                    const int32_t* lengths_host, float* out, int B, int T_total, int chunk_frames, void* workspace,
                                    size_t workspace_bytes, void* stream) {
    int rc;
    if (h && (rc = check_ar_model(h, "hificar_ar_loop", "hificar_ar_loop", spk_id, ph)) != HIFICAR_OK) return rc;
    if (chunk_frames < 1) return fail(HIFICAR_E_INVALID, "chunk_frames=%d must be positive", chunk_frames);
    if ((rc = check_ready(h, B, std::min(chunk_frames, std::max(T_total, 1)), workspace, workspace_bytes)) != HIFICAR_OK) return rc;
    if (T_total < 1) return fail(HIFICAR_E_INVALID, "T_total=%d must be positive", T_total);
    if (!c || !out) return fail(HIFICAR_E_INVALID, "hificar_ar_loop: null tensor");
    if ((rc = check_ar_chunk(h, chunk_frames, T_total > chunk_frames)) != HIFICAR_OK) return rc;
    const hipStream_t s0 = static_cast<hipStream_t>(stream);
    if ((rc = enter_stream(h, s0)) != HIFICAR_OK) return rc;
    if (lengths_host && !lengths) return fail(HIFICAR_E_INVALID, "hificar_ar_loop_ragged: lengths_host without the device copy");
    if (lengths_host && (rc = check_lengths(lengths_host, B, T_total)) != HIFICAR_OK) return rc;
    const int Tn_max = std::min(chunk_frames, T_total);
    const size_t ws0_bytes = plan_workspace(h, (B + 1) / 2, Tn_max, nullptr).bytes;
    hipStreamCaptureStatus cap = hipStreamCaptureStatusNone;
    (void)hipStreamIsCapturing(s0, &cap);
    if (!lengths && B >= 2 && B >= h->ar_dual_min && B <= h->ar_dual_max && !h->profiling && h->taps.empty() && cap == hipStreamCaptureStatusNone &&
        ws0_bytes + plan_workspace(h, B / 2, Tn_max, nullptr).bytes <= workspace_bytes)
        return ar_loop_two_streams(h, c, spk_id, ph, out, B, T_total, chunk_frames, workspace, ws0_bytes, s0);
    for (int f0 = 0; f0 < T_total; f0 += chunk_frames) {
        int Bn = B;
        if (lengths_host) {
            Bn = 0;
            for (int b = 0; b < B; ++b)
                if (lengths_host[b] > f0) Bn = b + 1;
            if (Bn == 0) break;
        }
        FwdCall k = ar_chunk_call(h, c, spk_id, ph, out, T_total, chunk_frames, f0, 0, Bn, workspace, s0);
        k.seq_len = lengths;
        if ((rc = forward_impl(h, k)) != HIFICAR_OK) return rc;
    }
    return HIFICAR_OK;
}

extern "C" int hificar_ar_loop_ragged(hificar_handle* h, const float* c, const int32_t* lengths, const int32_t* lengths_host,
                                      float* out, int B, int T_total, int chunk_frames, void* workspace, size_t workspace_bytes,
                                      void* stream) {
    if (h && h->cfg.use_ar && (h->cfg.use_spk_id || h->cfg.use_ph))
        return fail(HIFICAR_E_INVALID, "hificar_ar_loop: speaker / phoneme conditioned models are driven through hificar_forward_cond");
    return hificar_ar_loop_cond(h, c, nullptr, nullptr, lengths, lengths_host, out, B, T_total, chunk_frames, workspace, workspace_bytes, stream);
}

struct PackedSteps {
    struct Step {
        int n, frames;
    };
    std::vector<Step> steps;
    std::vector<int2> slots;
    std::vector<int> valid;
};
static PackedSteps packed_step_table(const int32_t* lengths_host, int N, int T_max, int chunk_frames, int batch) {
    PackedSteps t;
    std::vector<int> run, f0((size_t)N, 0);
    int next = 0;
    for (;;) {
        while ((int)run.size() < batch && next < N) {
            if (lengths_host[next] > 0) run.push_back(next);
            ++next;
        }
        if (run.empty()) break;
        t.steps.push_back({(int)run.size(), std::min(chunk_frames, T_max)});
        for (int u : run) {
            t.slots.push_back(int2{u, f0[u]});
            t.valid.push_back(std::min(chunk_frames, lengths_host[u] - f0[u]));
        }
        t.slots.resize((t.slots.size() + 1) & ~(size_t)1);
        t.valid.resize(t.slots.size());
        std::vector<int> keep;
        for (int u : run) {
            f0[u] += chunk_frames;
            if (f0[u] < lengths_host[u]) keep.push_back(u);
        }
        run.swap(keep);
    }
    return t;
}

extern "C" int hificar_ar_loop_packed_cond(hificar_handle* h, const float* c, const int32_t* spk_id, const int32_t* ph,
                                           const int32_t* lengths_host, float* out, int N, int T_max, int chunk_frames, int batch,
                                           void* workspace, size_t workspace_bytes, void* stream_) {
    int rc;
    if (h && (rc = check_ar_model(h, "hificar_ar_loop", "hificar_ar_loop_packed", spk_id, ph)) != HIFICAR_OK) return rc;
    if (chunk_frames < 1 || batch < 1 || N < 1 || T_max < 1)
        return fail(HIFICAR_E_INVALID, "hificar_ar_loop_packed: N=%d, T_max=%d, chunk_frames=%d, batch=%d must be positive", N, T_max,
                    chunk_frames, batch);
    batch = std::min(batch, N);
    if ((rc = check_ready(h, batch, std::min(chunk_frames, T_max), workspace, workspace_bytes)) != HIFICAR_OK) return rc;
// ... 219 lines not shown
```

### articulatory_amd/csrc/hificar_conv.hip.h

```cpp
#pragma once
#include <hip/hip_runtime.h>
#include <stdint.h>
#include <type_traits>

namespace hificar {

typedef float f32x2 __attribute__((ext_vector_type(2)));
typedef float f32x4 __attribute__((ext_vector_type(4)));
typedef unsigned u32x4_t __attribute__((ext_vector_type(4)));
typedef float f32x16 __attribute__((ext_vector_type(16)));
typedef __bf16 bf16x4 __attribute__((ext_vector_type(4)));
typedef __bf16 bf16x8 __attribute__((ext_vector_type(8)));

constexpr int kMaxPhase = 8;
constexpr int kMaxTaps = 16;

struct ConvParams {
    const bf16x8* w16;
    const float* bias;
    const float* res;
    const float* mask_src;
    float mask_slope;
    float* y;
    const float* xf;
    float slope_in;
    int act_in;
    const char* xs;
    const char* xs_more[3];
    char* ys;
    const char* zeros;
    float slope_out;
    int cout_real;
    int L;
    int tiles_per_seq;
    int cin;
    int cout_total;
    int n_blocks32;
    int nb32_per_phase;
    int ntaps;
    int off_min;
    int halo;
    int tap_step;
    int tap_off0[kMaxPhase];
    const int* seq_len;
    int len_const;
    int len_f0, len_max, len_mul;
    long long x_seq_bytes;
    int x_row_bytes;
    int x_rows;
    int x_up;
    unsigned x_up_rcp;
};

__device__ __forceinline__ int scalar_load_i32(const int* p) {
    int v;
    asm volatile("s_load_dword %0, %1, 0x0\n\ts_waitcnt lgkmcnt(0)" : "=s"(v) : "s"(p) : "memory");
    return v;
}

__device__ __forceinline__ void scalar_load_2i32(const int* p, int& a, int& b) {
    long long v;
    asm volatile("s_load_dwordx2 %0, %1, 0x0\n\ts_waitcnt lgkmcnt(0)" : "=s"(v) : "s"(p) : "memory");
    a = (int)v;
    b = (int)(v >> 32);
}

__device__ __forceinline__ bool is_ragged(const ConvParams& p) { return p.seq_len != nullptr || p.len_const >= 0; }

__device__ __forceinline__ int seq_rows(const ConvParams& p, int seq) {
    if (!is_ragged(p)) return p.L;
    const int n = (p.seq_len ? scalar_load_i32(p.seq_len + __builtin_amdgcn_readfirstlane(seq)) : p.len_const) - p.len_f0;
    return min(max(n, 0), p.len_max) * p.len_mul;
}

struct MultiConvParams {
    ConvParams p[3];
    int n_branches;
    int nseq_tiles;
    int ngroups;
    int total_tiles;
    int buf_bytes;
    const int* sched_start;
    const int* sched_tiles;
    int zrep;
    long long zs_x, zs_w, zs_y, zs_b;
    unsigned long long* trace;
    int xcd_order;
    int stage_cached;
};


#ifdef HIFICAR_TRACE
__device__ unsigned long long g_trace_realtime[2][1024];
__device__ unsigned long long g_trace_rt_slots[4][64];
#define HIFICAR_STAMP(slot)                                                                            \
    do {                                                                                               \
        if (mp.trace && lane == 0 && (wave == 0 || wave == kFirstLoader) && (slot) < 64)               \
            mp.trace[((size_t)blockIdx.x * 2 + (wave ? 1 : 0)) * 64 + (slot)] = __builtin_amdgcn_s_memtime(); \
        if (mp.trace && lane == 0 && wave == 0 && ((slot) == 0 || (slot) == 63) && blockIdx.x < 1024)  \
            g_trace_realtime[(slot) == 63][blockIdx.x] = __builtin_amdgcn_s_memrealtime();             \
        if (mp.trace && lane == 0 && wave == 0 && (slot) < 64 && blockIdx.x < 4)                       \
            g_trace_rt_slots[blockIdx.x][(slot)] = __builtin_amdgcn_s_memrealtime();                   \
    } while (0)
#else
#define HIFICAR_STAMP(slot) do { } while (0)
#endif

__device__ __forceinline__ float lrelu(float v, float slope) { return v >= 0.f ? v : v * slope; }


template <int I, int NDS, int NVMEM, int NMFMA>
__device__ __forceinline__ void pin_slab_slot() {
    if constexpr (I < NMFMA) {
        constexpr int NMEM = NDS + NVMEM;
        constexpr int lo = NMEM * I / NMFMA, hi = NMEM * (I + 1) / NMFMA;
        constexpr int ds = (hi < NDS ? hi : NDS) - (lo < NDS ? lo : NDS);
        constexpr int vm = (hi - lo) - ds;
        __builtin_amdgcn_sched_group_barrier(0x008, 1, 0);
        if constexpr (ds > 0) __builtin_amdgcn_sched_group_barrier(0x100, ds, 0);
        if constexpr (vm > 0) __builtin_amdgcn_sched_group_barrier(0x020, vm, 0);
        pin_slab_slot<I + 1, NDS, NVMEM, NMFMA>();
    }
}
template <int NDS, int NVMEM, int NMFMA>
__device__ __forceinline__ void pin_slab_step() {
    pin_slab_slot<0, NDS, NVMEM, NMFMA>();
}
__device__ __forceinline__ void lds_barrier() { asm volatile("s_waitcnt lgkmcnt(0)\n\ts_barrier" ::: "memory"); }

template <int MI, int WM, int WN, int NC16, bool F32, int KS = 1, int NB = 1, bool DOUT = false>
__device__ __forceinline__ void conv_ws_body(const MultiConvParams& mp) {
    static_assert(!DOUT || (F32 && KS == 1 && NB == 1), "direct output: exact fp32, dense form, one channel block per wave");
    static_assert(NB == 1 || (NB == 2 && KS == 1), "one or two channel blocks per MFMA wave");
    static_assert(KS == 1 || (KS == 4 && WM == 1 && WN == 1), "split-K: four waves share one 32-channel block");
    static_assert(KS == 4 || WM * WN == 4 || WM * WN == 8, "4 or 8 MFMA waves per workgroup");
    constexpr int NW = KS == 4 ? 4 : WM * WN;
    constexpr bool kPrimeOnce = DOUT;
    constexpr bool kRowMajorAcc = DOUT;
    constexpr int NTHR = (NW + 4) * 64;
    constexpr int kFirstLoader = NW;
    (void)kFirstLoader;
    static_assert(NC16 == 1 || NC16 == 2 || NC16 == 4, "chunk of 16, 32 or 64 channels");
    constexpr int TM = WM * MI * 32;
    constexpr int CH = NC16 * 16;
    constexpr int RB = CH * 4;
    constexpr int SPR = CH / 4;
    constexpr int LOG_SPR = NC16 == 4 ? 4 : NC16 == 2 ? 3 : 2;
    constexpr int LOG_RPB = 4 - LOG_SPR;
    extern __shared__ __attribute__((aligned(1024))) char smem_b[];

    const int tid = threadIdx.x;
    const int lane = tid & 63;
    const int wave = __builtin_amdgcn_readfirstlane(tid >> 6);
    const bool loader = wave >= NW;
    const int cw = loader ? 0 : wave;
    const int wm = KS == 4 ? 0 : cw / WN;
    const int wn = KS == 4 ? 0 : cw % WN;
    const int li = lane & 31;
    const int g = lane >> 5;
    const int nchunks = mp.p[0].cin / CH;
    const int tiles_per_branch = mp.ngroups * mp.nseq_tiles;
    const int buf_bytes = mp.buf_bytes;

    struct Tile {
        int b, z, ng, seq, t0;
    };
    auto decode = [&](int tile) {
        Tile T;
        const unsigned ut = (unsigned)tile, tpb = (unsigned)tiles_per_branch, zr = (unsigned)mp.zrep, nst = (unsigned)mp.nseq_tiles;
        const unsigned bz = ut / tpb;
        const unsigned b = bz / zr;
        T.b = (int)b;
        T.z = (int)(bz - b * zr);
        const unsigned rem = ut - bz * tpb;
        const unsigned ng = rem / nst;
        T.ng = (int)ng;
        const unsigned m = rem - ng * nst;
        const unsigned tps = (unsigned)mp.p[0].tiles_per_seq;
        const unsigned seq = m / tps;
        T.seq = (int)seq;
        T.t0 = (int)((m - seq * tps) * (unsigned)TM);
        return T;
    };

    constexpr int TN = WN * NB * 32;
    constexpr int OP = TN + 4;
    int sched_lo = 0, sched_hi = 0;
    if (mp.sched_start) scalar_load_2i32(mp.sched_start + blockIdx.x, sched_lo, sched_hi);
    const int my_rounds = mp.sched_start ? sched_hi - sched_lo
                                         : (mp.total_tiles - (int)blockIdx.x + (int)gridDim.x - 1) / (int)gridDim.x;
    auto tile_of = [&](int it) {
        int i = it;
        if ((blockIdx.x & 1) && my_rounds >= 3 && it >= my_rounds - 2) i = it == my_rounds - 1 ? my_rounds - 2 : my_rounds - 1;
        if (mp.sched_start) return scalar_load_i32(mp.sched_tiles + sched_lo + i);
        if (mp.xcd_order) {
            const int x = (int)blockIdx.x & 7, l = (int)blockIdx.x >> 3;
            const int base = mp.total_tiles >> 3, rem = mp.total_tiles & 7;
            return x * base + min(x, rem) + l;
        }
        return (int)blockIdx.x + (my_rounds - 1 - i) * (int)gridDim.x;
    };
    auto nxt = [&](int i) {
        if (is_ragged(mp.p[0]))
            while (i < my_rounds) {
                const Tile T = decode(tile_of(i));
                if (T.t0 < seq_rows(mp.p[T.b], T.seq)) break;
                ++i;
            }
        return i;
    };
    const float* O = reinterpret_cast<const float*>(smem_b + 2 * buf_bytes);
    auto write_out = [&](const Tile& T, int ltid, int nthr) {
        const ConvParams& p = mp.p[T.b];
        const int vc_base = T.ng * TN;
        const int width = min(TN, p.n_blocks32 * 32 - vc_base);
        const int w8 = width >> 3;
        const int rpp = nthr / w8;
        const int rr = ltid / w8;
        const int c8 = (ltid - rr * w8) * 8;
        const bool lane_on = rr < rpp;
        const size_t seq_base = (size_t)T.seq * p.L;
        const float slope_out = p.slope_out;
        const int rows = min(TM, seq_rows(p, T.seq) - T.t0);
        const float* const bias_z = p.bias + (size_t)T.z * mp.zs_b;
        float* const y_z = p.y ? p.y + (size_t)T.z * mp.zs_y : nullptr;
        char* const ys_z = p.ys ? p.ys + (size_t)T.z * mp.zs_y * 4 : nullptr;
        const int vc = vc_base + c8;
        const f32x4 bv0 = *reinterpret_cast<const f32x4*>(bias_z + vc);
        const f32x4 bv1 = *reinterpret_cast<const f32x4*>(bias_z + vc + 4);
        const int ph_row = vc / p.cout_real;
        const int split_off = ph_row * p.cout_real * 4 + (vc - ph_row * p.cout_real) * 2;
        constexpr int UB = 4;
        for (int r0 = 0; r0 < rows; r0 += rpp * UB) {
            f32x4 v0[UB], v1[UB], q0[UB], q1[UB], m0[UB], m1[UB];
#pragma unroll
            for (int q = 0; q < UB; ++q) {
                const int row_l = r0 + q * rpp + rr;
                v0[q] = v1[q] = q0[q] = q1[q] = f32x4{0.f, 0.f, 0.f, 0.f};
                m0[q] = m1[q] = f32x4{1.f, 1.f, 1.f, 1.f};
                if (lane_on && row_l < rows) {
                    v0[q] = *reinterpret_cast<const f32x4*>(&O[row_l * OP + c8]);
                    v1[q] = *reinterpret_cast<const f32x4*>(&O[row_l * OP + c8 + 4]);
                    if (p.mask_src) {
                        const float* mp_ = p.mask_src + (seq_base + T.t0 + row_l) * p.cout_total + vc;
                        m0[q] = *reinterpret_cast<const f32x4*>(mp_);
                        m1[q] = *reinterpret_cast<const f32x4*>(mp_ + 4);
                    }
                    if constexpr (KS == 4) {
                        const f32x4 a0 = *reinterpret_cast<const f32x4*>(&O[(TM + row_l) * OP + c8]);
                        const f32x4 a1 = *reinterpret_cast<const f32x4*>(&O[(TM + row_l) * OP + c8 + 4]);
                        const f32x4 b0 = *reinterpret_cast<const f32x4*>(&O[(2 * TM + row_l) * OP + c8]);
                        const f32x4 b1 = *reinterpret_cast<const f32x4*>(&O[(2 * TM + row_l) * OP + c8 + 4]);
                        const f32x4 d0 = *reinterpret_cast<const f32x4*>(&O[(3 * TM + row_l) * OP + c8]);
                        const f32x4 d1 = *reinterpret_cast<const f32x4*>(&O[(3 * TM + row_l) * OP + c8 + 4]);
                        v0[q] = (v0[q] + a0) + (b0 + d0);
                        v1[q] = (v1[q] + a1) + (b1 + d1);
                    }
                    if (p.res) {
                        const float* rp = p.res + (seq_base + T.t0 + row_l) * p.cout_total + vc;
                        q0[q] = *reinterpret_cast<const f32x4*>(rp);
                        q1[q] = *reinterpret_cast<const f32x4*>(rp + 4);
                    }
                }
            }
#pragma unroll
            for (int q = 0; q < UB; ++q) {
                const int row_l = r0 + q * rpp + rr;
                if (lane_on && row_l < rows) {
                    const size_t row = seq_base + T.t0 + row_l;
                    float o[8];
                    if (p.mask_src) {
#pragma unroll
                        for (int e = 0; e < 4; ++e) {
                            o[e] = (v0[q][e] + bv0[e]) * (m0[q][e] > 0.f ? 1.f : p.mask_slope) + q0[q][e];
                            o[4 + e] = (v1[q][e] + bv1[e]) * (m1[q][e] > 0.f ? 1.f : p.mask_slope) + q1[q][e];
                        }
                    } else {
#pragma unroll
                        for (int e = 0; e < 4; ++e) {
                            o[e] = (v0[q][e] + bv0[e]) + q0[q][e];
                            o[4 + e] = (v1[q][e] + bv1[e]) + q1[q][e];
                        }
                    }
                    if (y_z) {
                        float* yp = y_z + row * p.cout_total + vc;
                        *reinterpret_cast<f32x4*>(yp) = f32x4{o[0], o[1], o[2], o[3]};
                        *reinterpret_cast<f32x4*>(yp + 4) = f32x4{o[4], o[5], o[6], o[7]};
                    }
                    if (ys_z) {
                        if constexpr (F32) {
                            float a[8];
#pragma unroll
                            for (int e = 0; e < 8; ++e) a[e] = fmaxf(o[e], o[e] * slope_out);
                            float* orow = reinterpret_cast<float*>(ys_z) + row * (size_t)p.cout_total + vc;
                            *reinterpret_cast<f32x4*>(orow) = f32x4{a[0], a[1], a[2], a[3]};
                            *reinterpret_cast<f32x4*>(orow + 4) = f32x4{a[4], a[5], a[6], a[7]};
                        } else {
                            bf16x8 hi, lo;
#pragma unroll
                            for (int e = 0; e < 8; ++e) {
                                const float a = fmaxf(o[e], o[e] * slope_out);
                                hi[e] = (__bf16)a;
                                lo[e] = (__bf16)(a - (float)hi[e]);
                            }
                            char* orow = ys_z + row * (size_t)p.cout_total * 4 + split_off;
                            *reinterpret_cast<bf16x8*>(orow) = hi;
                            *reinterpret_cast<bf16x8*>(orow + p.cout_real * 2) = lo;
                        }
                    }
                }
            }
        }
    };
    if (loader) {
        const int lw = wave - NW;
        const int ltid = tid - NW * 64;

        auto dma_item = [&](const Tile& T, int c, int jj) {
            const ConvParams& p = mp.p[T.b];
            const int R = TM + p.halo;
            const int ninstr = (R * SPR + 63) >> 6;
            const int Ls = p.x_rows ? p.x_rows : seq_rows(p, T.seq);
            const int row_bytes = p.x_row_bytes ? p.x_row_bytes : p.cin * 4;
            const char* const xs_z = p.xs + (size_t)T.z * mp.zs_x + (size_t)T.seq * (p.x_seq_bytes ? (size_t)p.x_seq_bytes : (size_t)p.L * p.cin * 4);
            char* dst = smem_b + (jj & 1) * buf_bytes;
            const int c0b = c * CH * 2;
            for (int i = lw; i < ninstr; i += 4) {
                const int n = i * 64 + lane;
                const int r = n >> LOG_SPR;
                const int sl = (n & (SPR - 1)) ^ ((r >> LOG_RPB) & (SPR - 1));
                const int t = T.t0 + p.off_min + r;
                const char* src = p.zeros;
                if (r < R && t >= 0 && t < Ls) {
                    const int ts = p.x_up > 1 ? (int)__umulhi((unsigned)t, p.x_up_rcp) : t;
                    if constexpr (F32) src = xs_z + (size_t)ts * row_bytes + 2 * c0b + sl * 16;
                    else src = xs_z + (size_t)ts * row_bytes + (sl < SPR / 2 ? c0b + sl * 16 : p.cin * 2 + c0b + (sl - SPR / 2) * 16);
                }
                if (mp.stage_cached)
                    __builtin_amdgcn_global_load_lds((const __attribute__((address_space(1))) void*)src,
                                                     (__attribute__((address_space(3))) void*)(dst + i * 1024), 16, 0, 0);
                else
                    __builtin_amdgcn_global_load_lds((const __attribute__((address_space(1))) void*)src,
                                                     (__attribute__((address_space(3))) void*)(dst + i * 1024), 16, 0, 2);
            }
        };
        auto stage_act_item = [&](const Tile& T, int c, int jj) {
            if constexpr (F32) {
                const ConvParams& p = mp.p[T.b];
                const int R = TM + p.halo;
                const int ninstr = (R * SPR + 63) >> 6;
                const int Ls = p.x_rows ? p.x_rows : seq_rows(p, T.seq);
                const int row_bytes = p.x_row_bytes ? p.x_row_bytes : p.cin * 4;
                const size_t seq_off = (size_t)T.z * mp.zs_x + (size_t)T.seq * (p.x_seq_bytes ? (size_t)p.x_seq_bytes : (size_t)p.L * p.cin * 4);
                char* dst = smem_b + (jj & 1) * buf_bytes;
                const int c0b = c * CH * 2;
                const float slope = p.slope_in;
                const int nsrc = p.act_in;
                auto src_off = [&](int i, bool& ok) {
                    const int n = i * 64 + lane;
                    const int r = n >> LOG_SPR;
                    const int sl = (n & (SPR - 1)) ^ ((r >> LOG_RPB) & (SPR - 1));
                    const int t = T.t0 + p.off_min + r;
                    ok = i < ninstr && r < R && t >= 0 && t < Ls;
                    const int ts = p.x_up > 1 ? (int)__umulhi((unsigned)t, p.x_up_rcp) : t;
                    return seq_off + (size_t)ts * row_bytes + 2 * c0b + sl * 16;
                };
                auto ld = [&](const char* base, size_t off) {
                    if (mp.stage_cached) return *reinterpret_cast<const f32x4*>(base + off);
                    return __builtin_nontemporal_load(reinterpret_cast<const f32x4*>(base + off));
                };
                if (nsrc <= 1) {
                    constexpr int UB = 12;
                    for (int i0 = lw; i0 < ninstr; i0 += 4 * UB) {
                        f32x4 v[UB];
#pragma unroll
                        for (int q = 0; q < UB; ++q) {
                            bool ok;
                            const size_t off = src_off(i0 + 4 * q, ok);
                            v[q] = f32x4{0.f, 0.f, 0.f, 0.f};
                            if (ok) v[q] = ld(p.xs, off);
                        }
#pragma unroll
                        for (int q = 0; q < UB; ++q) {
                            const int i = i0 + 4 * q;
                            if (i < ninstr) {
                                f32x4 a;
#pragma unroll
                                for (int e = 0; e < 4; ++e) a[e] = fmaxf(v[q][e], v[q][e] * slope);
                                *reinterpret_cast<f32x4*>(dst + i * 1024 + lane * 16) = a;
                            }
                        }
                    }
                } else {
                    constexpr int UB = 4;
                    for (int i0 = lw; i0 < ninstr; i0 += 4 * UB) {
                        f32x4 v[UB], w1[UB], w2[UB], w3[UB];
#pragma unroll
                        for (int q = 0; q < UB; ++q) {
                            bool ok;
                            const size_t off = src_off(i0 + 4 * q, ok);
                            v[q] = w1[q] = w2[q] = w3[q] = f32x4{0.f, 0.f, 0.f, 0.f};
                            if (ok) {
                                v[q] = ld(p.xs, off);
                                w1[q] = ld(p.xs_more[0], off);
                                if (nsrc >= 3) w2[q] = ld(p.xs_more[1], off);
                                if (nsrc == 4) w3[q] = ld(p.xs_more[2], off);
                            }
                        }
#pragma unroll
                        for (int q = 0; q < UB; ++q) {
                            const int i = i0 + 4 * q;
                            if (i < ninstr) {
                                f32x4 a;
#pragma unroll
                                for (int e = 0; e < 4; ++e) {
                                    float m;
                                    if (nsrc == 4) m = (((v[q][e] + w1[q][e]) + w2[q][e]) + w3[q][e]) / 4.0f;
                                    else if (nsrc == 3) m = ((v[q][e] + w1[q][e]) + w2[q][e]) / 3.0f;
                                    else m = (v[q][e] + w1[q][e]) / 2.0f;
                                    a[e] = fmaxf(m, m * slope);
                                }
                                *reinterpret_cast<f32x4*>(dst + i * 1024 + lane * 16) = a;
                            }
                        }
                    }
                }
            }
        };
        auto stage_item = [&](const Tile& T, int c, int jj) {
            if constexpr (F32) {
                if (mp.p[T.b].act_in) {
                    stage_act_item(T, c, jj);
                    return;
                }
            }
            dma_item(T, c, jj);
        };
        int j = 0;
        HIFICAR_STAMP(0);
        bool have_prev = false;
        Tile Tprev;
        for (int it = nxt(0); it < my_rounds; it = nxt(it + 1)) {
            const Tile T = decode(tile_of(it));
            for (int c = 0; c < nchunks; ++c, ++j) {
                stage_item(T, c, j);
                if constexpr (!DOUT) {
                    if (c == 1 && have_prev) write_out(Tprev, ltid, 256);
                }
                HIFICAR_STAMP(1 + 2 * j);
                __syncthreads();
                HIFICAR_STAMP(2 + 2 * j);
            }
            Tprev = T;
            have_prev = true;
        }
        __syncthreads();
        if constexpr (!DOUT) {
            if (have_prev) write_out(Tprev, tid, NTHR);
        }
        HIFICAR_STAMP(63);
        return;
    }

    __builtin_amdgcn_s_setprio(1);
    f32x16 acc[NB][MI];
    using frag_t = typename std::conditional<F32, f32x4, bf16x8>::type;
    constexpr int NMF = (F32 ? 8 : 3) * MI * NB;
    frag_t wr[NB][NC16][2];
    auto wstream = [&](const Tile& T) {
        const ConvParams& p = mp.p[T.b];
        const int nb = (T.ng * WN + wn) * NB;
        return reinterpret_cast<const frag_t*>(reinterpret_cast<const char*>(p.w16) + (size_t)T.z * mp.zs_w) + (size_t)(nb < p.n_blocks32 ? nb : 0) * p.ntaps * (p.cin / 16) * 128 + lane;
    };
    auto wstride = [&](const Tile& T) {
        const ConvParams& p = mp.p[T.b];
        return ((T.ng * WN + wn) * NB + 1 < p.n_blocks32) ? (long long)p.ntaps * (p.cin / 16) * 128 : 0LL;
    };
    const frag_t* wp = nullptr;
    const frag_t* wp2 = nullptr;
    int groups_left = 0;
    auto prime = [&](const Tile& T) {
        wp = wstream(T);
#pragma unroll
        for (int u = 0; u < NC16; ++u) {
            wr[0][u][0] = wp[u * 128];
            wr[0][u][1] = wp[u * 128 + 64];
        }
        if constexpr (NB == 2) {
            wp2 = wp + wstride(T);
#pragma unroll
            for (int u = 0; u < NC16; ++u) {
                wr[1][u][0] = wp2[u * 128];
                wr[1][u][1] = wp2[u * 128 + 64];
            }
            wp2 += NC16 * 128;
        }
        wp += NC16 * 128;
        groups_left = nchunks * mp.p[T.b].ntaps - 1;
    };
    const int wave_row0 = wm * (MI * 32);

    auto addr_set = [&](int buf_off, int roff, int (&ad)[NC16][2]) {
        const int r0 = wave_row0 + li + roff;
        const int swz = (r0 >> LOG_RPB) & (SPR - 1);
        const int base = buf_off + r0 * RB;
#pragma unroll
        for (int u = 0; u < NC16; ++u) {
            if constexpr (F32) {
                ad[u][0] = base + (((4 * u + g) ^ swz) << 4);
                ad[u][1] = base + (((4 * u + 2 + g) ^ swz) << 4);
            } else {
                ad[u][0] = base + (((2 * u + g) ^ swz) << 4);
                ad[u][1] = base + (((SPR / 2 + 2 * u + g) ^ swz) << 4);
            }
        }
    };
    auto load_x = [&](frag_t (&xh)[MI], frag_t (&xl)[MI], const int (&ad)[2]) {
#pragma unroll
        for (int mi = 0; mi < MI; ++mi) {
            xh[mi] = *reinterpret_cast<const frag_t*>(smem_b + ad[0] + mi * 32 * RB);
            xl[mi] = *reinterpret_cast<const frag_t*>(smem_b + ad[1] + mi * 32 * RB);
        }
    };
    auto mfma_step = [&](const frag_t (&xh)[MI], const frag_t (&xl)[MI], const frag_t (&wh)[NB], const frag_t (&wl)[NB]) {
        if constexpr (F32) {
#pragma unroll
            for (int s4 = 0; s4 < 4; ++s4)
#pragma unroll
                for (int q = 0; q < NB; ++q)
#pragma unroll
                    for (int mi = 0; mi < MI; ++mi) {
                        if constexpr (kRowMajorAcc) acc[q][mi] = __builtin_amdgcn_mfma_f32_32x32x2f32(xh[mi][s4], wh[q][s4], acc[q][mi], 0, 0, 0);
                        else acc[q][mi] = __builtin_amdgcn_mfma_f32_32x32x2f32(wh[q][s4], xh[mi][s4], acc[q][mi], 0, 0, 0);
                    }
#pragma unroll
            for (int s4 = 0; s4 < 4; ++s4)
#pragma unroll
                for (int q = 0; q < NB; ++q)
#pragma unroll
                    for (int mi = 0; mi < MI; ++mi) {
                        if constexpr (kRowMajorAcc) acc[q][mi] = __builtin_amdgcn_mfma_f32_32x32x2f32(xl[mi][s4], wl[q][s4], acc[q][mi], 0, 0, 0);
                        else acc[q][mi] = __builtin_amdgcn_mfma_f32_32x32x2f32(wl[q][s4], xl[mi][s4], acc[q][mi], 0, 0, 0);
                    }
        } else {
#pragma unroll
            for (int q = 0; q < NB; ++q)
#pragma unroll
                for (int mi = 0; mi < MI; ++mi) acc[q][mi] = __builtin_amdgcn_mfma_f32_32x32x16_bf16(wh[q], xl[mi], acc[q][mi], 0, 0, 0);
#pragma unroll
            for (int q = 0; q < NB; ++q)
#pragma unroll
                for (int mi = 0; mi < MI; ++mi) acc[q][mi] = __builtin_amdgcn_mfma_f32_32x32x16_bf16(wl[q], xh[mi], acc[q][mi], 0, 0, 0);
#pragma unroll
            for (int q = 0; q < NB; ++q)
#pragma unroll
                for (int mi = 0; mi < MI; ++mi) acc[q][mi] = __builtin_amdgcn_mfma_f32_32x32x16_bf16(wh[q], xh[mi], acc[q][mi], 0, 0, 0);
        }
    };
    auto slab_step = [&](const frag_t (&xh)[MI], const frag_t (&xl)[MI], int u) {
        frag_t wh[NB], wl[NB];
        wh[0] = wr[0][u][0];
        wl[0] = wr[0][u][1];
        wr[0][u][0] = wp[u * 128];
        wr[0][u][1] = wp[u * 128 + 64];
        if constexpr (NB == 2) {
            wh[1] = wr[1][u][0];
            wl[1] = wr[1][u][1];
            wr[1][u][0] = wp2[u * 128];
            wr[1][u][1] = wp2[u * 128 + 64];
        }
        mfma_step(xh, xl, wh, wl);
        pin_slab_step<2 * MI, 2 * NB, NMF>();
    };

    auto epilogue_rm = [&](const Tile& T, const ConvParams& p, int nb, int rows_valid, float bias_l) {
        if constexpr (kRowMajorAcc) {
            const int rows_w = __builtin_amdgcn_readfirstlane(max(min(rows_valid - wave_row0, MI * 32), 0));
            const unsigned pitch_b = __builtin_amdgcn_readfirstlane((unsigned)p.cout_total * 4u);
            const size_t first = ((size_t)T.seq * p.L + T.t0 + wave_row0) * p.cout_total;
            float* const y_p = p.y;
            char* const ys_p = p.ys;
            const float* const res_p = p.res;
            auto uni64 = [](unsigned long long v) {
                const unsigned lo = __builtin_amdgcn_readfirstlane((unsigned)v), hi = __builtin_amdgcn_readfirstlane((unsigned)(v >> 32));
                return ((unsigned long long)hi << 32) | lo;
            };
            const bool has_y = y_p != nullptr, has_ys = ys_p != nullptr, has_res = res_p != nullptr, has_mask = p.mask_src != nullptr;
            const unsigned long long b_y = uni64((unsigned long long)(has_y ? y_p + (size_t)T.z * mp.zs_y + first : nullptr));
            const unsigned long long b_ys = uni64((unsigned long long)(has_ys ? reinterpret_cast<float*>(ys_p) + (size_t)T.z * mp.zs_y + first : nullptr));
            const unsigned long long b_res = uni64((unsigned long long)(has_res ? res_p + first : nullptr));
            const unsigned long long b_mask = uni64((unsigned long long)(has_mask ? p.mask_src + first : nullptr));
            auto rsrc_of = [&](unsigned long long base, bool present, int mi) {
                const unsigned rows = (unsigned)max(min(rows_w - mi * 32, 32), 0);
                return __builtin_amdgcn_make_buffer_rsrc((void*)uni64(base + (unsigned long long)(mi * 32) * pitch_b), 0,
                                                         __builtin_amdgcn_readfirstlane(present ? rows * pitch_b : 0u), 0x00020000);
            };
            constexpr int kAux = 0;
            const int voff = (int)((4u * g * p.cout_total + nb * 32 + li) * 4u);
            int off16[16];
#pragma unroll
            for (int r = 0; r < 16; ++r) off16[r] = voff + (int)((8 * (r >> 2) + (r & 3)) * pitch_b);
            const float slope_out = p.slope_out, mask_slope = p.mask_slope;
            auto pass = [&](auto HR, auto HM, auto HY, auto HS) {
                constexpr bool kRes = decltype(HR)::value, kMask = decltype(HM)::value, kY = decltype(HY)::value, kYs = decltype(HS)::value;
                auto fetch1 = [&](int mi, int r, float (&rs)[16], float (&mk)[16]) {
                    if constexpr (kRes) rs[r] = __builtin_bit_cast(float, __builtin_amdgcn_raw_buffer_load_b32(rsrc_of(b_res, has_res, mi), off16[r], 0, 0));
                    if constexpr (kMask) mk[r] = __builtin_bit_cast(float, __builtin_amdgcn_raw_buffer_load_b32(rsrc_of(b_mask, has_mask, mi), off16[r], 0, 0));
                };
                auto finish = [&](int mi, int r, const float (&rs)[16], const float (&mk)[16]) {
                    float o = acc[0][mi][r] + bias_l;
                    if constexpr (kMask) o *= mk[r] > 0.f ? 1.f : mask_slope;
                    if constexpr (kRes) o += rs[r];
                    if constexpr (kY) __builtin_amdgcn_raw_buffer_store_b32(__builtin_bit_cast(unsigned, o), rsrc_of(b_y, has_y, mi), off16[r], 0, kAux);
                    if constexpr (kYs) __builtin_amdgcn_raw_buffer_store_b32(__builtin_bit_cast(unsigned, __builtin_amdgcn_fmed3f(o, o * slope_out, __builtin_inff())), rsrc_of(b_ys, has_ys, mi), off16[r], 0, kAux);
                };
                {
                    constexpr int G2 = MI >= 2 ? 2 : 1;
#pragma unroll
                    for (int m0 = 0; m0 < MI; m0 += G2) {
                        float rs[G2][16], mk[G2][16];
                        if constexpr (kRes || kMask) {
#pragma unroll
                            for (int mm = 0; mm < G2; ++mm)
#pragma unroll
                                for (int r = 0; r < 16; ++r) fetch1(m0 + mm, r, rs[mm], mk[mm]);
                        }
#pragma unroll
                        for (int mm = 0; mm < G2; ++mm)
#pragma unroll
                            for (int r = 0; r < 16; ++r) finish(m0 + mm, r, rs[mm], mk[mm]);
                    }
                }
            };
            constexpr std::true_type Y{};
            constexpr std::false_type N{};
            if (has_mask) {
                pass(Y, Y, Y, Y);
                return;
            }
            if (has_res) {
                if (has_y && has_ys) pass(Y, N, Y, Y);
                else if (has_y) pass(Y, N, Y, N);
                else pass(Y, N, N, Y);
            } else {
                if (has_y && has_ys) pass(N, N, Y, Y);
                else if (has_y) pass(N, N, Y, N);
                else pass(N, N, N, Y);
            }
        }
    };
    auto bias_of = [&](const Tile& T) {
        const int nb = (T.ng * WN + wn) * NB;
        return (mp.p[T.b].bias + (size_t)T.z * mp.zs_b)[(nb < mp.p[T.b].n_blocks32 ? nb : 0) * 32 + li];
    };
    int j = 0;
    int last = -1;
    HIFICAR_STAMP(0);
    if constexpr (KS == 4) {
        const int ks = cw;
        constexpr int LOG_NC = NC16 == 4 ? 2 : NC16 == 2 ? 1 : 0;
        for (int it = nxt(0); it < my_rounds; it = nxt(it + 1)) {
            last = it;
            const Tile T = decode(tile_of(it));
            const ConvParams& p = mp.p[T.b];
            const int nb = T.ng;
            const int phase = (int)((unsigned)nb / (unsigned)p.nb32_per_phase);
            const int roff0 = __builtin_amdgcn_readfirstlane(p.tap_off0[phase] - p.off_min);
            const int tap_step = p.tap_step;
            const int nsteps = p.ntaps * NC16;
            const frag_t* wtile = reinterpret_cast<const frag_t*>(reinterpret_cast<const char*>(p.w16) + (size_t)T.z * mp.zs_w) + (size_t)nb * nchunks * nsteps * 128 + lane;
#pragma unroll
            for (int mi = 0; mi < MI; ++mi)
#pragma unroll
                for (int r = 0; r < 16; ++r) acc[0][mi][r] = 0.f;
            auto x_addr = [&](int buf_off, int s, int (&ad)[2]) {
                const int t = s >> LOG_NC, u = s & (NC16 - 1);
                const int r0 = li + roff0 + t * tap_step;
                const int swz = (r0 >> LOG_RPB) & (SPR - 1);
                const int base = buf_off + r0 * RB;
                if constexpr (F32) {
                    ad[0] = base + (((4 * u + g) ^ swz) << 4);
                    ad[1] = base + (((4 * u + 2 + g) ^ swz) << 4);
                } else {
                    ad[0] = base + (((2 * u + g) ^ swz) << 4);
                    ad[1] = base + (((SPR / 2 + 2 * u + g) ^ swz) << 4);
                }
            };
            const int spi = ks < nsteps ? (nsteps - ks + 3) >> 2 : 0;
            for (int c = 0; c < nchunks; ++c, ++j) {
                const frag_t* wc = wtile + (size_t)c * nsteps * 128 + (size_t)ks * 128;
                frag_t w0h, w0l, w1h, w1l;
                if (spi > 0) {
                    w0h = wc[0];
                    w0l = wc[64];
                }
                if (spi > 1) {
                    w1h = wc[512];
                    w1l = wc[512 + 64];
                }
                HIFICAR_STAMP(1 + 3 * j);
                lds_barrier();
                HIFICAR_STAMP(2 + 3 * j);
                const int buf_off = (j & 1) * buf_bytes;
                frag_t x0h[MI], x0l[MI], x1h[MI], x1l[MI];
                int ad[2];
                if (spi > 0) {
                    x_addr(buf_off, ks, ad);
                    load_x(x0h, x0l, ad);
                }
                for (int i = 0; i < spi; i += 2) {
                    if (i + 1 < spi) {
                        x_addr(buf_off, ks + 4 * (i + 1), ad);
                        load_x(x1h, x1l, ad);
                    }
                    {
                        const frag_t cwh[1] = {w0h}, cwl[1] = {w0l};
                        if (i + 2 < spi) {
                            w0h = wc[(size_t)(i + 2) * 512];
                            w0l = wc[(size_t)(i + 2) * 512 + 64];
                        }
                        mfma_step(x0h, x0l, cwh, cwl);
                    }
                    if (i + 1 < spi) {
                        if (i + 2 < spi) {
                            x_addr(buf_off, ks + 4 * (i + 2), ad);
                            load_x(x0h, x0l, ad);
                        }
                        const frag_t cwh[1] = {w1h}, cwl[1] = {w1l};
                        if (i + 3 < spi) {
                            w1h = wc[(size_t)(i + 3) * 512];
                            w1l = wc[(size_t)(i + 3) * 512 + 64];
                        }
                        mfma_step(x1h, x1l, cwh, cwl);
                    }
                }
            }
            {
                float* Ow = reinterpret_cast<float*>(smem_b + 2 * buf_bytes) + ks * TM * OP;
#pragma unroll
                for (int mi = 0; mi < MI; ++mi)
#pragma unroll
                    for (int q = 0; q < 4; ++q) {
                        f32x4 v;
#pragma unroll
                        for (int e = 0; e < 4; ++e) v[e] = acc[0][mi][4 * q + e];
                        *reinterpret_cast<f32x4*>(&Ow[(mi * 32 + li) * OP + 8 * q + 4 * g]) = v;
                    }
            }
        }
        HIFICAR_STAMP(3 * j);
        __syncthreads();
        HIFICAR_STAMP(62);
        if (last >= 0) write_out(decode(tile_of(last)), tid, NTHR);
        HIFICAR_STAMP(63);
        return;
    }
    Tile T_carry = {};
    bool primed = false;
    (void)primed;
    if (nxt(0) < my_rounds) {
        T_carry = decode(tile_of(nxt(0)));
        if constexpr (kPrimeOnce) prime(T_carry);
    }
    for (int it = nxt(0), itn; it < my_rounds; it = itn) {
        itn = nxt(it + 1);
        last = it;
        const Tile T = T_carry;
        const ConvParams& p = mp.p[T.b];
        const int nb = (T.ng * WN + wn) * NB;
        const bool active = nb < p.n_blocks32;
        const int phase = active ? (int)((unsigned)nb / (unsigned)p.nb32_per_phase) : 0;
        const int roff0 = __builtin_amdgcn_readfirstlane(p.tap_off0[phase] - p.off_min);
        const int tap_step = p.tap_step;
        const int ntaps = p.ntaps;
        const int rows_valid_t = kRowMajorAcc ? __builtin_amdgcn_readfirstlane(min(TM, seq_rows(p, T.seq) - T.t0)) : 0;
        const Tile Tn = itn < my_rounds ? decode(tile_of(itn)) : T;
        T_carry = Tn;
        const frag_t* wp_next = wstream(Tn);
        const long long wst_next = NB == 2 ? wstride(Tn) : 0LL;
        const int groups_next = nchunks * mp.p[Tn.b].ntaps;
        if constexpr (!kPrimeOnce) {
            if (active && !primed) prime(T);
        }
#pragma unroll
        for (int q = 0; q < NB; ++q)
#pragma unroll
            for (int mi = 0; mi < MI; ++mi)
#pragma unroll
                for (int r = 0; r < 16; ++r) acc[q][mi][r] = 0.f;
        float bias_l = 0.f;
        if constexpr (kRowMajorAcc) bias_l = bias_of(T);

        for (int c = 0; c < nchunks; ++c, ++j) {
            HIFICAR_STAMP(1 + 3 * j);
            lds_barrier();
            HIFICAR_STAMP(2 + 3 * j);
            if constexpr (!kPrimeOnce) {
                if (!active) continue;
            }
            const int buf_off = (j & 1) * buf_bytes;
            int ad[NC16][2];
            addr_set(buf_off, roff0, ad);
            if constexpr (NC16 % 2 == 0) {
                frag_t x0h[MI], x0l[MI], x1h[MI], x1l[MI];
                load_x(x0h, x0l, ad[0]);
                for (int t = 0; t < ntaps; ++t) {
                    const bool last_tap = t + 1 == ntaps;
                    int adn[NC16][2];
                    addr_set(buf_off, roff0 + (last_tap ? t : t + 1) * tap_step, adn);
                    if (groups_left == 0) {
                        wp = wp_next;
                        if constexpr (NB == 2) wp2 = wp_next + wst_next;
                        groups_left = groups_next;
                    }
                    --groups_left;
#pragma unroll
                    for (int u = 0; u < NC16; u += 2) {
                        load_x(x1h, x1l, ad[u + 1]);
                        slab_step(x0h, x0l, u);
                        if (u + 2 < NC16) load_x(x0h, x0l, ad[u + 2]);
                        else load_x(x0h, x0l, adn[0]);
                        slab_step(x1h, x1l, u + 1);
                    }
                    wp += NC16 * 128;
                    if constexpr (NB == 2) wp2 += NC16 * 128;
#pragma unroll
                    for (int u = 0; u < NC16; ++u) {
                        ad[u][0] = adn[u][0];
                        ad[u][1] = adn[u][1];
                    }
                }
            } else {
                static_assert(NC16 % 2 == 0 || NC16 == 1, "odd chunk sizes other than 16 channels are not instantiated");
                frag_t x0h[MI], x0l[MI], x1h[MI], x1l[MI];
                load_x(x0h, x0l, ad[0]);
                auto tap = [&](const frag_t (&xh)[MI], const frag_t (&xl)[MI]) {
                    if (groups_left == 0) {
                        wp = wp_next;
                        if constexpr (NB == 2) wp2 = wp_next + wst_next;
                        groups_left = groups_next;
                    }
                    --groups_left;
                    slab_step(xh, xl, 0);
                    wp += NC16 * 128;
                    if constexpr (NB == 2) wp2 += NC16 * 128;
                };
                for (int t = 0; t < ntaps; t += 2) {
                    if (t + 1 < ntaps) {
                        addr_set(buf_off, roff0 + (t + 1) * tap_step, ad);
                        load_x(x1h, x1l, ad[0]);
                    }
                    tap(x0h, x0l);
                    if (t + 1 < ntaps) {
                        if (t + 2 < ntaps) {
                            addr_set(buf_off, roff0 + (t + 2) * tap_step, ad);
                            load_x(x0h, x0l, ad[0]);
                        }
                        tap(x1h, x1l);
                    }
                }
            }
        }
        HIFICAR_STAMP(3 * j);
        primed = active;
        if constexpr (kRowMajorAcc) {
            if (active) epilogue_rm(T, p, nb, rows_valid_t, bias_l);
        } else if (active) {
            float* O = reinterpret_cast<float*>(smem_b + 2 * buf_bytes);
#pragma unroll
            for (int b2 = 0; b2 < NB; ++b2)
#pragma unroll
                for (int mi = 0; mi < MI; ++mi)
#pragma unroll
                    for (int q = 0; q < 4; ++q) {
                        f32x4 v;
#pragma unroll
                        for (int e = 0; e < 4; ++e) v[e] = acc[b2][mi][4 * q + e];
                        *reinterpret_cast<f32x4*>(&O[(wave_row0 + mi * 32 + li) * OP + (wn * NB + b2) * 32 + 8 * q + 4 * g]) = v;
                    }
        }
    }
    lds_barrier();
    HIFICAR_STAMP(62);
    if constexpr (!DOUT) {
        if (last >= 0) write_out(decode(tile_of(last)), tid, NTHR);
    }
    HIFICAR_STAMP(63);
}

template <int MI, int WM, int WN, int NC16>
__global__ __launch_bounds__((WM * WN + 4) * 64) void conv_f32do_kernel(const MultiConvParams mp) {
    conv_ws_body<MI, WM, WN, NC16, true, 1, 1, true>(mp);
}

template <int MI, int WM, int WN, int NC16>
__global__ __launch_bounds__((WM * WN + 4) * 64) void conv_bf16x3_kernel(const MultiConvParams mp) {
    conv_ws_body<MI, WM, WN, NC16, false>(mp);
}

template <int MI, int WM, int WN, int NC16>
__global__ __launch_bounds__((WM * WN + 4) * 64) void conv_bf16x3nb_kernel(const MultiConvParams mp) {
    conv_ws_body<MI, WM, WN, NC16, false, 1, 2>(mp);
}

template <int MI, int NC16>
__global__ __launch_bounds__(512) void conv_sk_bf16x3_kernel(const MultiConvParams mp) {
    conv_ws_body<MI, 1, 1, NC16, false, 4>(mp);
}

template <int MI, int NC16>
__global__ __launch_bounds__(512) void conv_sk_f32_kernel(const MultiConvParams mp) {
    conv_ws_body<MI, 1, 1, NC16, true, 4>(mp);
}

struct PairParams {
    ConvParams p1[3];
    ConvParams p2[3];
    int n_branches;
    int nseq;
    int tile_start[4];
    int tiles_per_seq[3];
    int in_bytes;
    int ts_bytes;
    float slope_mid;
    const int* sched_start;
    const int* sched_tiles;
    unsigned long long* trace;
};

template <int MI, int WM, int WN, int NC16, bool F32>
__device__ __forceinline__ void conv_pair_body(const PairParams& mp) {
    static_assert(WM * WN == 4, "4 MFMA waves per workgroup");
    static_assert(NC16 == 2 || NC16 == 4, "C = 32 or 64");
    static_assert(WN * 32 == NC16 * 16, "the workgroup covers all C channels");
    constexpr int TMc = WM * MI * 32;
    constexpr int kFirstLoader = 4;
    (void)kFirstLoader;
    constexpr int CH = NC16 * 16;
    constexpr int RB = CH * 4;
    constexpr int SPR = CH / 4;
    constexpr int LOG_SPR = NC16 == 4 ? 4 : 3;
    constexpr int LOG_RPB = 4 - LOG_SPR;
    constexpr int TN = CH;
    constexpr int OP = TN + 4;
    extern __shared__ __attribute__((aligned(1024))) char smem_b[];
    const int in_bytes = mp.in_bytes;
    const int ts_off = in_bytes;
    const int o_off = in_bytes;

    const int tid = threadIdx.x;
    const int lane = tid & 63;
    const int wave = __builtin_amdgcn_readfirstlane(tid >> 6);
    const bool loader = wave >= 4;
    const int cw = wave & 3;
    const int wm = cw / WN;
    const int wn = cw % WN;
    const int li = lane & 31;
    const int g = lane >> 5;
    const int total_tiles = mp.tile_start[mp.n_branches];

    struct Tile {
        int b, seq, t0, tmo;
    };
    auto decode = [&](int tile) {
        Tile T;
        T.b = 0;
        if (mp.n_branches > 1 && tile >= mp.tile_start[1]) T.b = 1;
        if (mp.n_branches > 2 && tile >= mp.tile_start[2]) T.b = 2;
        const unsigned m = (unsigned)(tile - mp.tile_start[T.b]);
        const unsigned tps = (unsigned)mp.tiles_per_seq[T.b];
        T.tmo = TMc - (mp.p2[T.b].ntaps - 1);
        const unsigned seq = m / tps;
        T.seq = (int)seq;
        T.t0 = (int)(m - seq * tps) * T.tmo;
        return T;
    };
    int sched_lo = 0, sched_hi = 0;
    if (mp.sched_start) scalar_load_2i32(mp.sched_start + blockIdx.x, sched_lo, sched_hi);
    const int my_rounds = mp.sched_start ? sched_hi - sched_lo
                                         : (total_tiles - (int)blockIdx.x + (int)gridDim.x - 1) / (int)gridDim.x;
    auto tile_of = [&](int it) {
        int i = it;
        if ((blockIdx.x & 1) && my_rounds >= 3 && it >= my_rounds - 2) i = it == my_rounds - 1 ? my_rounds - 2 : my_rounds - 1;
        if (mp.sched_start) return scalar_load_i32(mp.sched_tiles + sched_lo + i);
        return (int)blockIdx.x + (my_rounds - 1 - i) * (int)gridDim.x;
    };
    auto nxt = [&](int i) {
        if (is_ragged(mp.p1[0]))
            while (i < my_rounds) {
                const Tile T = decode(tile_of(i));
                if (T.t0 < seq_rows(mp.p1[T.b], T.seq)) break;
                ++i;
            }
        return i;
    };
    const int first = nxt(0);
    const float* O = reinterpret_cast<const float*>(smem_b + o_off);
    auto write_out = [&](const Tile& T, int ltid, int nthr) {
        const ConvParams& p = mp.p2[T.b];
        constexpr int w8 = TN / 8;
        const int rpp = nthr / w8;
        const int rr = ltid / w8;
        const int c8 = (ltid - rr * w8) * 8;
        const size_t seq_base = (size_t)T.seq * p.L;
        const float slope_out = p.slope_out;
        const int rows = min(T.tmo, seq_rows(p, T.seq) - T.t0);
        const f32x4 bv0 = *reinterpret_cast<const f32x4*>(p.bias + c8);
        const f32x4 bv1 = *reinterpret_cast<const f32x4*>(p.bias + c8 + 4);
        constexpr int UB = 4;
        for (int r0 = 0; r0 < rows; r0 += rpp * UB) {
            f32x4 v0[UB], v1[UB], q0[UB], q1[UB];
#pragma unroll
            for (int q = 0; q < UB; ++q) {
                const int row_l = r0 + q * rpp + rr;
                v0[q] = v1[q] = q0[q] = q1[q] = f32x4{0.f, 0.f, 0.f, 0.f};
                if (row_l < rows) {
                    v0[q] = *reinterpret_cast<const f32x4*>(&O[row_l * OP + c8]);
                    v1[q] = *reinterpret_cast<const f32x4*>(&O[row_l * OP + c8 + 4]);
                    const float* rp = p.res + (seq_base + T.t0 + row_l) * TN + c8;
                    q0[q] = *reinterpret_cast<const f32x4*>(rp);
                    q1[q] = *reinterpret_cast<const f32x4*>(rp + 4);
                }
            }
#pragma unroll
            for (int q = 0; q < UB; ++q) {
                const int row_l = r0 + q * rpp + rr;
                if (row_l < rows) {
                    const size_t row = seq_base + T.t0 + row_l;
                    float o[8];
#pragma unroll
                    for (int e = 0; e < 4; ++e) {
                        o[e] = (v0[q][e] + bv0[e]) + q0[q][e];
                        o[4 + e] = (v1[q][e] + bv1[e]) + q1[q][e];
                    }
                    float* yp = p.y + row * TN + c8;
                    *reinterpret_cast<f32x4*>(yp) = f32x4{o[0], o[1], o[2], o[3]};
                    *reinterpret_cast<f32x4*>(yp + 4) = f32x4{o[4], o[5], o[6], o[7]};
                    if (p.ys) {
                        if constexpr (F32) {
                            float a[8];
#pragma unroll
                            for (int e = 0; e < 8; ++e) a[e] = fmaxf(o[e], o[e] * slope_out);
                            float* orow = reinterpret_cast<float*>(p.ys) + row * (size_t)TN + c8;
                            *reinterpret_cast<f32x4*>(orow) = f32x4{a[0], a[1], a[2], a[3]};
                            *reinterpret_cast<f32x4*>(orow + 4) = f32x4{a[4], a[5], a[6], a[7]};
                        } else {
                            bf16x8 hi, lo;
#pragma unroll
                            for (int e = 0; e < 8; ++e) {
                                const float a = fmaxf(o[e], o[e] * slope_out);
                                hi[e] = (__bf16)a;
                                lo[e] = (__bf16)(a - (float)hi[e]);
                            }
                            char* orow = p.ys + row * (size_t)TN * 4 + c8 * 2;
                            *reinterpret_cast<bf16x8*>(orow) = hi;
                            *reinterpret_cast<bf16x8*>(orow + TN * 2) = lo;
                        }
                    }
                }
            }
        }
    };
    if (loader) {
        const int lw = wave - 4;
        const int ltid = tid - 256;
        auto dma_in = [&](const Tile& T) {
            const ConvParams& p = mp.p1[T.b];
            const int pad2 = (mp.p2[T.b].ntaps - 1) >> 1;
            const int R = TMc + p.halo;
            const int ninstr = (R * SPR + 63) >> 6;
            const size_t seq_base = (size_t)T.seq * p.L;
            const int Ls = seq_rows(p, T.seq);
            const int row_bytes = p.cin * 4;
            const int tfirst = T.t0 - pad2 + p.off_min;
            for (int i = lw; i < ninstr; i += 4) {
                const int n = i * 64 + lane;
                const int r = n >> LOG_SPR;
                const int sl = (n & (SPR - 1)) ^ ((r >> LOG_RPB) & (SPR - 1));
                const int t = tfirst + r;
                const char* src = p.zeros;
                if (r < R && t >= 0 && t < Ls) {
                    if constexpr (F32) src = (p.xf ? reinterpret_cast<const char*>(p.xf) : p.xs) + (seq_base + t) * row_bytes + sl * 16;
                    else src = p.xs + (seq_base + t) * row_bytes + (sl < SPR / 2 ? sl * 16 : p.cin * 2 + (sl - SPR / 2) * 16);
                }
                __builtin_amdgcn_global_load_lds((const __attribute__((address_space(1))) void*)src,
                                                 (__attribute__((address_space(3))) void*)(smem_b + i * 1024), 16, 0, 2);
            }
        };
        auto stage_f32 = [&](const Tile& T) {
            const ConvParams& p = mp.p1[T.b];
            const int pad2 = (mp.p2[T.b].ntaps - 1) >> 1;
            const int R = TMc + p.halo;
            const size_t seq_base = (size_t)T.seq * p.L;
            const int Ls = seq_rows(p, T.seq);
            const int tfirst = T.t0 - pad2 + p.off_min;
            const float slope = p.slope_in;
            constexpr int UPR = CH / 8;
            constexpr int LOG_UPR = NC16 == 4 ? 3 : 2;
            const int nunits = R * UPR;
            constexpr int UB = 4;
            for (int u0 = ltid; u0 < nunits; u0 += 256 * UB) {
                f32x4 a[UB], b[UB];
#pragma unroll
                for (int q = 0; q < UB; ++q) {
                    const int u = u0 + q * 256;
                    const int r = u >> LOG_UPR;
                    const int t = tfirst + r;
                    a[q] = b[q] = f32x4{0.f, 0.f, 0.f, 0.f};
                    if (u < nunits && t >= 0 && t < Ls) {
                        const float* src = p.xf + (seq_base + t) * CH + (u & (UPR - 1)) * 8;
                        a[q] = *reinterpret_cast<const f32x4*>(src);
                        b[q] = *reinterpret_cast<const f32x4*>(src + 4);
                    }
                }
#pragma unroll
                for (int q = 0; q < UB; ++q) {
                    const int u = u0 + q * 256;
                    if (u < nunits) {
                        const int r = u >> LOG_UPR;
                        const int cu = u & (UPR - 1);
                        const int swz = (r >> LOG_RPB) & (SPR - 1);
                        bf16x8 hi, lo;
#pragma unroll
                        for (int e = 0; e < 8; ++e) {
                            const float v = e < 4 ? a[q][e] : b[q][e - 4];
                            const float act = fmaxf(v, v * slope);
                            hi[e] = (__bf16)act;
                            lo[e] = (__bf16)(act - (float)hi[e]);
                        }
                        *reinterpret_cast<bf16x8*>(smem_b + r * RB + ((cu ^ swz) << 4)) = hi;
                        *reinterpret_cast<bf16x8*>(smem_b + r * RB + (((SPR / 2 + cu) ^ swz) << 4)) = lo;
                    }
                }
            }
        };
        auto stage_in = [&](const Tile& T) {
            if constexpr (F32) {
                dma_in(T);
            } else {
                if (mp.p1[T.b].xf) stage_f32(T);
                else dma_in(T);
            }
        };
        Tile Tprev;
        if (first < my_rounds) stage_in(decode(tile_of(first)));
        for (int it = first, itn; it < my_rounds; it = itn) {
            itn = nxt(it + 1);
            const Tile T = decode(tile_of(it));
            HIFICAR_STAMP(4 * it);
            __syncthreads();
            HIFICAR_STAMP(4 * it + 1);
            if (it != first) write_out(Tprev, ltid, 256);
            HIFICAR_STAMP(4 * it + 2);
            lds_barrier();
            lds_barrier();
            HIFICAR_STAMP(4 * it + 3);
            if (itn < my_rounds) stage_in(decode(tile_of(itn)));
            lds_barrier();
            Tprev = T;
        }
        __syncthreads();
        if (first < my_rounds) write_out(Tprev, tid, 512);
        return;
    }

    auto pair_barrier = [] { lds_barrier(); };
    __builtin_amdgcn_s_setprio(1);
    f32x16 acc[MI];
    using frag_t = typename std::conditional<F32, f32x4, bf16x8>::type;
    constexpr int NMF = (F32 ? 8 : 3) * MI;
    frag_t wr[NC16][2];
    const frag_t* wp = nullptr;
    int groups_left = 0;
    auto stream1 = [&](const Tile& T) { return reinterpret_cast<const frag_t*>(mp.p1[T.b].w16) + (size_t)wn * mp.p1[T.b].ntaps * NC16 * 128 + lane; };
    auto stream2 = [&](const Tile& T) { return reinterpret_cast<const frag_t*>(mp.p2[T.b].w16) + (size_t)wn * mp.p2[T.b].ntaps * NC16 * 128 + lane; };
    if (first < my_rounds) {
        const Tile T0 = decode(tile_of(first));
        wp = stream1(T0);
#pragma unroll
        for (int u = 0; u < NC16; ++u) {
            wr[u][0] = wp[u * 128];
            wr[u][1] = wp[u * 128 + 64];
        }
        wp += NC16 * 128;
        groups_left = mp.p1[T0.b].ntaps - 1;
    }
    const int wave_row0 = wm * (MI * 32);

    auto addr_set = [&](int buf_off, int r0, int (&ad)[NC16][2]) {
        const int swz = (r0 >> LOG_RPB) & (SPR - 1);
        const int base = buf_off + r0 * RB;
#pragma unroll
        for (int u = 0; u < NC16; ++u) {
            if constexpr (F32) {
                ad[u][0] = base + (((4 * u + g) ^ swz) << 4);
// ... 191 lines not shown
```

### articulatory_amd/csrc/hificar_conv_inst.hip

```cpp
#include "hificar_conv.hip.h"
#include "hificar_launch.h"

#ifndef HIFICAR_INST_SET
#error "compile with -DHIFICAR_INST_SET=0..9"
#endif

namespace hificar {

#define HIFICAR_TILES9(X, nc) X(4, 1, 4, nc) X(4, 2, 2, nc) X(4, 4, 1, nc) X(2, 1, 4, nc) X(2, 2, 2, nc) X(2, 4, 1, nc) X(1, 1, 4, nc) X(1, 2, 2, nc) X(1, 4, 1, nc)

#if HIFICAR_INST_SET == 0
#define FAMILY kConvF32do
#define KERNEL conv_f32do_kernel
#define PARAMS MultiConvParams
#define SHAPES(X) HIFICAR_TILES9(X, 1)
#elif HIFICAR_INST_SET == 1
#define FAMILY kConvF32do
#define KERNEL conv_f32do_kernel
#define PARAMS MultiConvParams
#define SHAPES(X) HIFICAR_TILES9(X, 2)
#elif HIFICAR_INST_SET == 2
#define FAMILY kConvF32do
#define KERNEL conv_f32do_kernel
#define PARAMS MultiConvParams
#define SHAPES(X) HIFICAR_TILES9(X, 4)
#elif HIFICAR_INST_SET == 3
#define FAMILY kConvBf16x3
#define KERNEL conv_bf16x3_kernel
#define PARAMS MultiConvParams
#define SHAPES(X) HIFICAR_TILES9(X, 1)
#elif HIFICAR_INST_SET == 4
#define FAMILY kConvBf16x3
#define KERNEL conv_bf16x3_kernel
#define PARAMS MultiConvParams
#define SHAPES(X) HIFICAR_TILES9(X, 2)
#elif HIFICAR_INST_SET == 5
#define FAMILY kConvBf16x3
#define KERNEL conv_bf16x3_kernel
#define PARAMS MultiConvParams
#define SHAPES(X) HIFICAR_TILES9(X, 4)
#elif HIFICAR_INST_SET == 6
#define FAMILY kConvBf16x3nb
#define KERNEL conv_bf16x3nb_kernel
#define PARAMS MultiConvParams
#define SHAPES(X) X(2, 2, 2, 2) X(2, 4, 1, 2) X(2, 1, 4, 2) X(2, 2, 2, 4) X(2, 4, 1, 4) X(2, 1, 4, 4)
#elif HIFICAR_INST_SET == 7 || HIFICAR_INST_SET == 8
#if HIFICAR_INST_SET == 7
#define FAMILY kConvSkF32
#define KERNEL_PTR(mi, wm, wn, nc) (conv_sk_f32_kernel<mi, nc>)
#else
#define FAMILY kConvSkBf16x3
#define KERNEL_PTR(mi, wm, wn, nc) (conv_sk_bf16x3_kernel<mi, nc>)
#endif
#define THREADS(wm, wn) 512
#define PARAMS MultiConvParams
#define SHAPES(X) X(1, 1, 1, 1) X(2, 1, 1, 1) X(4, 1, 1, 1) X(1, 1, 1, 2) X(2, 1, 1, 2) X(4, 1, 1, 2) X(1, 1, 1, 4) X(2, 1, 1, 4) X(4, 1, 1, 4)
#elif HIFICAR_INST_SET == 9
#define PARAMS PairParams
#define THREADS(wm, wn) 512
#else
#error "HIFICAR_INST_SET out of range"
#endif

#ifndef KERNEL_PTR
#define KERNEL_PTR(mi, wm, wn, nc) (KERNEL<mi, wm, wn, nc>)
#endif
#ifndef THREADS
#define THREADS(wm, wn) ((wm * wn + 4) * 64)
#endif

#define HIFICAR_CAT_(a, b) a##b
#define HIFICAR_CAT(a, b) HIFICAR_CAT_(a, b)

#if HIFICAR_INST_SET != 9
hipError_t HIFICAR_CAT(conv_inst_launch_, HIFICAR_INST_SET)(const ConvShape& s, const void* params, dim3 grid, size_t lds, hipStream_t stream, bool* handled) {
    *handled = false;
    if (s.family != FAMILY) return hipSuccess;
#define X(A_, B_, C_, D_)                                                                                                      \
    if (s.mi == A_ && s.wm == B_ && s.wn == C_ && s.nc16 == D_) {                                                              \
        *handled = true;                                                                                                       \
        hipLaunchKernelGGL(KERNEL_PTR(A_, B_, C_, D_), grid, dim3(THREADS(B_, C_)), lds, stream, *static_cast<const PARAMS*>(params)); \
        return hipGetLastError();                                                                                              \
    }
    SHAPES(X)
#undef X
    return hipSuccess;
}

hipError_t HIFICAR_CAT(conv_inst_attrs_, HIFICAR_INST_SET)() {
    hipError_t e = hipSuccess;
#define X(A_, B_, C_, D_)                                                                                                                        \
    if (e == hipSuccess)                                                                                                                         \
        e = hipFuncSetAttribute(reinterpret_cast<const void*>(&KERNEL_PTR(A_, B_, C_, D_)), hipFuncAttributeMaxDynamicSharedMemorySize, 160 * 1024);
    SHAPES(X)
#undef X
    return e;
}
#else
#define PAIR_F32(X) X(4, 2, 2, 4) X(4, 4, 1, 2) X(1, 4, 1, 2)
#define PAIR_BF(X) X(4, 2, 2, 4) X(4, 4, 1, 2)
hipError_t conv_inst_launch_9(const ConvShape& s, const void* params, dim3 grid, size_t lds, hipStream_t stream, bool* handled) {
    *handled = false;
    if (s.family != kPairF32 && s.family != kPairBf16x3) return hipSuccess;
#define X(A_, B_, C_, D_)                                                                                                  \
    if (s.family == kPairF32 && s.mi == A_ && s.wm == B_ && s.wn == C_ && s.nc16 == D_) {                                  \
        *handled = true;                                                                                                   \
        hipLaunchKernelGGL((conv_pair_f32_kernel<A_, B_, C_, D_>), grid, dim3(512), lds, stream, *static_cast<const PairParams*>(params)); \
        return hipGetLastError();                                                                                          \
    }
    PAIR_F32(X)
#undef X
#define X(A_, B_, C_, D_)                                                                                                     \
    if (s.family == kPairBf16x3 && s.mi == A_ && s.wm == B_ && s.wn == C_ && s.nc16 == D_) {                                  \
        *handled = true;                                                                                                      \
        hipLaunchKernelGGL((conv_pair_bf16x3_kernel<A_, B_, C_, D_>), grid, dim3(512), lds, stream, *static_cast<const PairParams*>(params)); \
        return hipGetLastError();                                                                                             \
    }
    PAIR_BF(X)
#undef X
    return hipSuccess;
}

hipError_t conv_inst_attrs_9() {
    hipError_t e = hipSuccess;
#define X(A_, B_, C_, D_) \
    if (e == hipSuccess) e = hipFuncSetAttribute(reinterpret_cast<const void*>(&conv_pair_f32_kernel<A_, B_, C_, D_>), hipFuncAttributeMaxDynamicSharedMemorySize, 160 * 1024);
    PAIR_F32(X)
#undef X
#define X(A_, B_, C_, D_) \
    if (e == hipSuccess) e = hipFuncSetAttribute(reinterpret_cast<const void*>(&conv_pair_bf16x3_kernel<A_, B_, C_, D_>), hipFuncAttributeMaxDynamicSharedMemorySize, 160 * 1024);
    PAIR_BF(X)
#undef X
    return e;
}
#endif

}
```

### articulatory_amd/csrc/hificar_launch.h

```cpp
#pragma once
#include <hip/hip_runtime.h>

namespace hificar {

struct MultiConvParams;
struct PairParams;

enum ConvFamily {
    kConvF32do = 0,
    kConvBf16x3 = 1,
    kConvBf16x3nb = 2,
    kConvSkF32 = 3,
    kConvSkBf16x3 = 4,
    kPairF32 = 5,
    kPairBf16x3 = 6,
};

struct ConvShape {
    int family, mi, wm, wn, nc16;
};

hipError_t conv_launch(const ConvShape& s, const void* params, dim3 grid, size_t lds_bytes, hipStream_t stream);
hipError_t conv_set_lds_attributes();

#define HIFICAR_N_INST_SETS 10
#define HIFICAR_DECL_SET(n)                                                                                                              \
    hipError_t conv_inst_launch_##n(const ConvShape& s, const void* params, dim3 grid, size_t lds, hipStream_t stream, bool* handled); \
    hipError_t conv_inst_attrs_##n();
HIFICAR_DECL_SET(0) HIFICAR_DECL_SET(1) HIFICAR_DECL_SET(2) HIFICAR_DECL_SET(3) HIFICAR_DECL_SET(4)
HIFICAR_DECL_SET(5) HIFICAR_DECL_SET(6) HIFICAR_DECL_SET(7) HIFICAR_DECL_SET(8) HIFICAR_DECL_SET(9)
#undef HIFICAR_DECL_SET

}
```

Measured before the change: 39.81 million samples/s.

## Merge final MRF branch convs into one kernel summing branches in-register

```diff
diff --git a/__graft_entry__.py b/__graft_entry__.py
--- a/__graft_entry__.py
+++ b/__graft_entry__.py
@@ -10,7 +10,7 @@
 
 def build() -> None:
     csrc = os.path.join(REPO, "articulatory_amd", "csrc")
-    subprocess.run(["make", "-C", csrc, f"-j{max(1, min(11, os.cpu_count() or 1))}"], check=True)
+    subprocess.run(["make", "-C", csrc, f"-j{max(1, min(14, os.cpu_count() or 1))}"], check=True)
     import articulatory_amd
     from articulatory_amd import _native
 
diff --git a/articulatory_amd/csrc/hificar.hip b/articulatory_amd/csrc/hificar.hip
--- a/articulatory_amd/csrc/hificar.hip
+++ b/articulatory_amd/csrc/hificar.hip
@@ -87,6 +87,8 @@
     std::string name;
     MultiConvParams conv = {};
     PairParams pair = {};
+    MergeConvParams merge = {};
+    bool merge_wins = false;
 };
 
 struct hificar_engine {
@@ -96,6 +98,7 @@
     bool profile_detail = false;
     bool use_pair = true;
     bool pair_small = true;
+    int mrf_merge = 1;
     int ksplit = 1;
     double mi1_penalty = 1.05;
     int pick_throughput = 0;
@@ -202,6 +205,7 @@
     if (const char* e = getenv("HIFICAR_KSPLIT")) h->ksplit = atoi(e);
     if (const char* e = getenv("HIFICAR_PAIR")) h->use_pair = atoi(e) != 0;
     if (const char* e = getenv("HIFICAR_PAIR_SMALL")) h->pair_small = atoi(e) != 0;
+    if (const char* e = getenv("HIFICAR_MRF_MERGE")) h->mrf_merge = atoi(e);
 }
 
 struct ProfScope {
@@ -591,6 +595,7 @@
     if (handled) return e;
     HIFICAR_TRY_SET(0) HIFICAR_TRY_SET(1) HIFICAR_TRY_SET(2) HIFICAR_TRY_SET(3) HIFICAR_TRY_SET(4)
     HIFICAR_TRY_SET(5) HIFICAR_TRY_SET(6) HIFICAR_TRY_SET(7) HIFICAR_TRY_SET(8) HIFICAR_TRY_SET(9)
+    HIFICAR_TRY_SET(10) HIFICAR_TRY_SET(11) HIFICAR_TRY_SET(12)
 #undef HIFICAR_TRY_SET
     return hipErrorInvalidValue;
 }
@@ -601,6 +606,7 @@
     if (e == hipSuccess) e = conv_inst_attrs_##n();
     HIFICAR_ATTR_SET(0) HIFICAR_ATTR_SET(1) HIFICAR_ATTR_SET(2) HIFICAR_ATTR_SET(3) HIFICAR_ATTR_SET(4)
     HIFICAR_ATTR_SET(5) HIFICAR_ATTR_SET(6) HIFICAR_ATTR_SET(7) HIFICAR_ATTR_SET(8) HIFICAR_ATTR_SET(9)
+    HIFICAR_ATTR_SET(10) HIFICAR_ATTR_SET(11) HIFICAR_ATTR_SET(12)
 #undef HIFICAR_ATTR_SET
     return e;
 }
@@ -1040,7 +1046,8 @@
     return true;
 }
 
-static TileCfg pick_tile(const hificar_engine* h, const ConvLayer* const* layers, int nbr, int nseq, int rows, int zrep) {
+static TileCfg pick_tile(const hificar_engine* h, const ConvLayer* const* layers, int nbr, int nseq, int rows, int zrep, bool merged = false,
+                         double* est = nullptr, bool use_force = true) {
     const ConvLayer& L0 = *layers[0];
     const bool f32 = h->precision == HIFICAR_PREC_F32;
     int halo_all = 0;
@@ -1049,18 +1056,20 @@
     double best = 1e300;
     int nsteps_min = 1 << 30;
     for (int b = 0; b < nbr; ++b) nsteps_min = std::min(nsteps_min, layers[b]->ntaps * (L0.chunk16 / 16));
-    if (h->force_tile[0] != 0) {
+    if (h->force_tile[0] != 0 && use_force) {
         const TileCfg t = {h->force_tile[0], h->force_tile[1], h->force_tile[2], h->force_tile[3], h->force_tile[4]};
-        if (tile_admissible(h, layers, nbr, t, halo_all, nsteps_min)) return t;
+        if (tile_admissible(h, layers, nbr, t, halo_all, nsteps_min) && (!merged || (t.KS == 1 && t.NB == 1))) return t;
     }
     for (int ti = 0; ti < kNumTileCfgs; ++ti) {
         const TileCfg& t = kTileCfgs[ti];
         const int TM = t.WM * t.MI * 32;
         const int chunk = L0.chunk16;
         if (!tile_admissible(h, layers, nbr, t, halo_all, nsteps_min)) continue;
-        if (t.KS == 1 && h->ksplit == 2 && nsteps_min >= 2) continue;
+        if (merged && (t.KS != 1 || t.NB != 1)) continue;
+        if (!merged && t.KS == 1 && h->ksplit == 2 && nsteps_min >= 2) continue;
         const long long tiles_per_branch = (long long)nseq * ((rows + TM - 1) / TM) * ((L0.n_blocks32 + t.WN * t.NB - 1) / (t.WN * t.NB));
-        const long long total = tiles_per_branch * nbr * zrep;
+        const int ncls = merged ? 1 : nbr;
+        const long long total = tiles_per_branch * ncls * zrep;
         const int G = (int)std::min<long long>(total, h->num_cus);
         const int nchunks = L0.cin_pad / chunk;
         double total_cost = 0.0, heaviest = 0.0, lightest = 1e300, cb[3] = {0.0, 0.0, 0.0};
@@ -1071,18 +1080,26 @@
                 const int steps = layers[b]->ntaps * (chunk / 16);
                 c = (double)((steps + 3) / 4) * nchunks * slab * t.MI + 4000.0 + 600.0 * nchunks;
             }
+            if (merged) {
+                cb[0] += c - (b ? 2500.0 : 0.0);
+                continue;
+            }
             total_cost += c * tiles_per_branch * zrep;
             heaviest = std::max(heaviest, c);
             lightest = std::min(lightest, c);
             cb[b] = c;
         }
+        if (merged) {
+            total_cost = cb[0] * tiles_per_branch * zrep;
+            heaviest = lightest = cb[0];
+        }
         double worst = std::max(heaviest, total_cost / G);
         if (!h->shared_chip && total > G && total <= 4096) {
-            std::sort(cb, cb + nbr, [](double x, double y) { return x > y; });
+            std::sort(cb, cb + ncls, [](double x, double y) { return x > y; });
             std::priority_queue<double, std::vector<double>, std::greater<double>> load;
             for (int w = 0; w < G; ++w) load.push(0.0);
             worst = 0.0;
-            for (int b = 0; b < nbr; ++b)
+            for (int b = 0; b < ncls; ++b)
                 for (long long i = 0; i < tiles_per_branch * zrep; ++i) {
                     const double v = load.top() + cb[b];
                     load.pop();
@@ -1101,16 +1118,17 @@
             tc = t;
         }
     }
+    if (est) *est = best;
     return tc;
 }
 
 static std::string plan_name(const hificar_engine* h, const ConvShape& s, const ConvLayer& L0, int nbr) {
     static const char* const family[] = {"conv_f32do_kernel", "conv_bf16x3_kernel", "conv_bf16x3nb_kernel", "conv_sk_f32_kernel", "conv_sk_bf16x3_kernel",
-                                         "conv_pair_f32_kernel", "conv_pair_bf16x3_kernel"};
+                                         "conv_pair_f32_kernel", "conv_pair_bf16x3_kernel", "conv_f32mrg_kernel"};
     char kname[96];
     int n = s.family == kConvSkF32 || s.family == kConvSkBf16x3 ? snprintf(kname, sizeof(kname), "%s<%d,%d>", family[s.family], s.mi, s.nc16)
                                                                 : snprintf(kname, sizeof(kname), "%s<%d,%d,%d,%d>", family[s.family], s.mi, s.wm, s.wn, s.nc16);
-    if (h->profile_detail) snprintf(kname + n, sizeof(kname) - n, "|%s x%d", L0.name.c_str(), nbr);
+    if (h->profile_detail) snprintf(kname + n, sizeof(kname) - n, s.family == kConvF32mrg ? "|%s +%d" : "|%s x%d", L0.name.c_str(), nbr);
     return kname;
 }
 
@@ -1157,6 +1175,43 @@
     return lists.empty() ? HIFICAR_OK : upload_schedule(h, lists, mp.total_tiles, stream, &mp.sched_start, &mp.sched_tiles);
 }
 
+static int build_merge_plan(hificar_engine* h, const ConvLayer* const* layers, int nbr, int nseq, int rows, hipStream_t stream, ConvPlan& pl) {
+    const ConvLayer& L0 = *layers[0];
+    MergeConvParams& mp = pl.merge;
+    double est_merged = 1e300, est_classic = 0.0;
+    const TileCfg tc_free = pick_tile(h, layers, nbr, nseq, rows, 1, true, &est_merged, false);
+    const TileCfg tc = pick_tile(h, layers, nbr, nseq, rows, 1, true);
+    if (est_merged >= 1e300) return fail(HIFICAR_E_INVALID, "internal: no tile shape for the merged launch of %s", L0.name.c_str());
+    for (int q0 = 0; q0 < nbr; q0 += 3) {
+        double e = 0.0;
+        (void)pick_tile(h, layers + q0, std::min(3, nbr - q0), nseq, rows, 1, false, &e, false);
+        est_classic += e;
+    }
+    const double up_extra = 4.0 * nseq * rows * L0.cout_total * (nbr - 1) / 2048.0;
+    pl.merge_wins = !h->shared_chip && tc_free.MI > 1 && est_merged < est_classic + up_extra;
+    if (!pl.merge_wins && h->mrf_merge != 2) return HIFICAR_OK;
+    int halo_all = 0;
+    for (int b = 0; b < nbr; ++b) halo_all = std::max(halo_all, layers[b]->off_max - layers[b]->off_min);
+    const int TM = tc.WM * tc.MI * 32, nc16 = L0.chunk16 / 16;
+    const size_t buf_bytes = round_up_sz((size_t)(TM + halo_all) * L0.chunk16 * 4, 1024);
+    pl.shape = {kConvF32mrg, tc.MI, tc.WM, tc.WN, nc16};
+    pl.lds = 2 * buf_bytes;
+    mp.buf_bytes = (int)buf_bytes;
+    mp.n_branches = nbr;
+    mp.nseq_tiles = nseq * ((rows + TM - 1) / TM);
+    mp.ngroups = (L0.n_blocks32 + tc.WN - 1) / tc.WN;
+    const int npos = mp.ngroups * mp.nseq_tiles;
+    mp.total_tiles = nbr * npos;
+    pl.grid = (unsigned)std::min(npos, h->num_cus);
+    mp.xcd_order = 0;
+    mp.stage_cached = mp.ngroups > 2 ? 1 : 0;
+    pl.name = plan_name(h, pl.shape, L0, nbr);
+    TileLists lists(pl.grid);
+    for (int q = 0; q < npos; ++q)
+        for (int b = 0; b < nbr; ++b) lists[(size_t)q % pl.grid].push_back(b * npos + q);
+    return upload_schedule(h, lists, mp.total_tiles, stream, &mp.sched_start, &mp.sched_tiles);
+}
+
 struct PairIOB {
     const float* xf;
     const char* xs;
@@ -1225,9 +1280,9 @@
 }
 
 static const ConvPlan* get_plan(hificar_engine* h, const ConvLayer* const* a, const ConvLayer* const* b, int nbr, int nseq, int rows, int zrep,
-                                hipStream_t stream, int* rc) {
+                                hipStream_t stream, int* rc, bool merged = false) {
     *rc = HIFICAR_OK;
-    PlanKey k = {{}, nseq, rows, zrep, (h->precision == HIFICAR_PREC_F32 ? 1 : 0) | (h->training ? 2 : 0) | (h->shared_chip ? 4 : 0) | (b ? 8 : 0)};
+    PlanKey k = {{}, nseq, rows, zrep, (h->precision == HIFICAR_PREC_F32 ? 1 : 0) | (h->training ? 2 : 0) | (h->shared_chip ? 4 : 0) | (b ? 8 : 0) | (merged ? 16 : 0)};
     for (int i = 0; i < nbr; ++i) k.layers[i] = a[i];
     for (int i = 0; b && i < nbr; ++i) k.layers[3 + i] = b[i];
     auto it = h->plans.find(k);
@@ -1235,7 +1290,9 @@
         ConvPlan pl;
         if (h->plans.size() > 20000) *rc = evict_plans(h);
         if (*rc == HIFICAR_OK)
-            *rc = b ? build_pair_plan(h, a, b, nbr, nseq, rows, stream, pl) : build_conv_plan(h, a, nbr, nseq, rows, zrep, stream, pl);
+            *rc = merged ? build_merge_plan(h, a, nbr, nseq, rows, stream, pl)
+                  : b    ? build_pair_plan(h, a, b, nbr, nseq, rows, stream, pl)
+                         : build_conv_plan(h, a, nbr, nseq, rows, zrep, stream, pl);
         if (*rc != HIFICAR_OK) return nullptr;
         it = h->plans.emplace(k, std::move(pl)).first;
     }
@@ -1295,6 +1352,36 @@
     ProfScope prof(h, stream, pl->name, flops, bytes);
     const hipError_t e = conv_launch(pl->shape, &mp, dim3(pl->grid, 1, 1), pl->lds, stream);
     if (e != hipSuccess) return fail(HIFICAR_E_HIP, "conv launch (%s, %s) failed: %s", L0.name.c_str(), pl->name.c_str(), hipGetErrorString(e));
+    return HIFICAR_OK;
+}
+
+static int launch_merged(hificar_engine* h, const ConvPlan* pl, const ConvLayer* const* layers, int nbr, int nseq, int rows, const ConvIO* io, char* ys_out,
+                         float slope_out, const Ragged& rg, hipStream_t stream) {
+    const int TM = pl->shape.wm * pl->shape.mi * 32;
+    const ConvLayer& L0 = *layers[0];
+    MergeConvParams mp = pl->merge;
+    double flops = 0.0, bytes = 0.0;
+    const double pos = (double)nseq * rows;
+    for (int b = 0; b < nbr; ++b) {
+        const ConvLayer& Lb = *layers[b];
+        if (Lb.n_blocks32 != L0.n_blocks32 || Lb.chunk16 != L0.chunk16 || Lb.cin_pad != L0.cin_pad || Lb.cout_total != L0.cout_total || Lb.n_phase != 1 ||
+            !io[b].res || !io[b].xs || io[b].xs == ys_out)
+            return fail(HIFICAR_E_INVALID, "internal: merged launch of %s: branch %d does not fit", L0.name.c_str(), b);
+        fill_params(mp.p[b], Lb, rows, TM, io[b].res, nullptr, rg);
+        mp.p[b].xs = io[b].xs;
+        mp.p[b].ys = ys_out;
+        mp.p[b].zeros = h->d_zeros;
+        mp.p[b].slope_out = slope_out;
+        mp.p[b].cout_real = Lb.cout_pad;
+        mp.p[b].w16 = reinterpret_cast<const bf16x8*>(Lb.d_w32);
+        flops += 2.0 * pos * Lb.cin * Lb.cout * Lb.K;
+        bytes += 4.0 * (pos * Lb.cin_pad + pos * Lb.cout_total + (double)Lb.cin * Lb.cout * Lb.K);
+    }
+    bytes += 4.0 * pos * L0.cout_total;
+    mp.zrep = 1;
+    ProfScope prof(h, stream, pl->name, flops, bytes);
+    const hipError_t e = conv_launch(pl->shape, &mp, dim3(pl->grid, 1, 1), pl->lds, stream);
+    if (e != hipSuccess) return fail(HIFICAR_E_HIP, "merged conv launch (%s, %s) failed: %s", L0.name.c_str(), pl->name.c_str(), hipGetErrorString(e));
     return HIFICAR_OK;
 }
 
@@ -1487,6 +1574,7 @@
     BlockOrder bo;
     int rows = 0;
     const float* fin[kMaxBlk];
+    const char* mrf_act = nullptr;
     bool tapping = false;
     bool tap_convs1 = false;
     size_t tap_se = 0;
@@ -1626,6 +1714,15 @@
     return HIFICAR_OK;
 }
 
+static bool mrf_merge_allowed(const hificar_handle* h, const FwdCall& k, const FwdState& fs, int i) {
+    const hificar_config& cfg = h->cfg;
+    if (h->precision != HIFICAR_PREC_F32 || k.tp || fs.tapping || i + 1 >= cfg.n_stages || cfg.n_blocks < 2 || !cfg.use_additional_convs) return false;
+    if (h->mrf_merge == 0 || !h->use_pair || h->ksplit != 1) return false;
+    for (int j = 0; j < cfg.n_blocks; ++j)
+        if (cfg.n_dilations[j] != fs.bo.max_d) return false;
+    return true;
+}
+
 static int resblocks_general(hificar_handle* h, const FwdCall& k, FwdState& fs, int i, const char* u_act) {
     const hificar_config& cfg = h->cfg;
     const Workspace& ws = k.ws;
@@ -1639,6 +1736,7 @@
         for (int j = 0; j < nbk; ++j) xres[j] = tp->fin[j];
     for (int j = 0; j < nbk; ++j) fs.fin[j] = xres[j];
     const char* cur_s[kMaxBlk] = {u_act, u_act, u_act, u_act};
+    const bool may_merge = mrf_merge_allowed(h, k, fs, i);
     for (int d = 0; d < fs.bo.max_d; ++d) {
         const ConvLayer* l1[kMaxBlk];
         const ConvLayer* l2[kMaxBlk];
@@ -1680,7 +1778,15 @@
                     if ((rc = emit_tap(h, "blocks." + std::to_string(i * nbk + br.j[q]) + ".convs1." + std::to_string(d), io1[q].y, Cp, 0, Cs,
                                        B, rows, 0, k.stream)) != HIFICAR_OK)
                         return rc;
-            if (add_convs && (rc = launch_n(h, l2, nullptr, br.n, B, rows, io2, nullptr, cfg.lrelu_slope, fs.rg, k.stream)) != HIFICAR_OK) return rc;
+            const ConvPlan* mpl = nullptr;
+            if (may_merge && d + 1 == fs.bo.max_d && br.n == nbk) {
+                if (!(mpl = get_plan(h, l2, nullptr, br.n, B, rows, 1, k.stream, &rc, true))) return rc;
+                if (!mpl->merge_wins && h->mrf_merge != 2) mpl = nullptr;
+            }
+            if (mpl) {
+                if ((rc = launch_merged(h, mpl, l2, br.n, B, rows, io2, lbl_out[0], cfg.lrelu_slope, fs.rg, k.stream)) != HIFICAR_OK) return rc;
+                fs.mrf_act = lbl_out[0];
+            } else if (add_convs && (rc = launch_n(h, l2, nullptr, br.n, B, rows, io2, nullptr, cfg.lrelu_slope, fs.rg, k.stream)) != HIFICAR_OK) return rc;
         }
         for (int q = 0; q < br.n; ++q)
             if ((rc = tap_block(h, k, fs, i, br.j[q], d, xres[br.j[q]])) != HIFICAR_OK) return rc;
@@ -1695,8 +1801,11 @@
     const int nbk = cfg.n_blocks;
     int rc;
     const char* up_in = act_h0(k);
-    const bool fold_mrf = i > 0 && h->precision == HIFICAR_PREC_F32 && !tp;
-    if (i > 0 && !fold_mrf && (rc = launch_mrf_split(h, k, fs, i, &up_in)) != HIFICAR_OK) return rc;
+    const char* const merged_in = fs.mrf_act;
+    fs.mrf_act = nullptr;
+    const bool fold_mrf = i > 0 && h->precision == HIFICAR_PREC_F32 && !tp && !merged_in;
+    if (merged_in) up_in = merged_in;
+    if (i > 0 && !fold_mrf && !merged_in && (rc = launch_mrf_split(h, k, fs, i, &up_in)) != HIFICAR_OK) return rc;
     bool all_pairs = !fs.tap_convs1 && !tp && cfg.use_additional_convs != 0;
     for (int j = 0; j < nbk && all_pairs; ++j)
         for (int d = 0; d < cfg.n_dilations[j]; ++d) {
diff --git a/articulatory_amd/csrc/hificar_conv.hip.h b/articulatory_amd/csrc/hificar_conv.hip.h
--- a/articulatory_amd/csrc/hificar_conv.hip.h
+++ b/articulatory_amd/csrc/hificar_conv.hip.h
@@ -73,8 +73,9 @@
     return min(max(n, 0), p.len_max) * p.len_mul;
 }
 
-struct MultiConvParams {
-    ConvParams p[3];
+template <int NBR>
+struct MultiConvParamsN {
+    ConvParams p[NBR];
     int n_branches;
     int nseq_tiles;
     int ngroups;
@@ -88,6 +89,8 @@
     int xcd_order;
     int stage_cached;
 };
+struct MultiConvParams : MultiConvParamsN<3> {};
+struct MergeConvParams : MultiConvParamsN<4> {};
 
 
 #ifdef HIFICAR_TRACE
@@ -128,9 +131,10 @@
 }
 __device__ __forceinline__ void lds_barrier() { asm volatile("s_waitcnt lgkmcnt(0)\n\ts_barrier" ::: "memory"); }
 
-template <int MI, int WM, int WN, int NC16, bool F32, int KS = 1, int NB = 1, bool DOUT = false>
-__device__ __forceinline__ void conv_ws_body(const MultiConvParams& mp) {
+template <int MI, int WM, int WN, int NC16, bool F32, int KS = 1, int NB = 1, bool DOUT = false, bool MRG = false, class MP = MultiConvParams>
+__device__ __forceinline__ void conv_ws_body(const MP& mp) {
     static_assert(!DOUT || (F32 && KS == 1 && NB == 1), "direct output: exact fp32, dense form, one channel block per wave");
+    static_assert(!MRG || DOUT, "branch-summing form: a direct-output kernel");
     static_assert(NB == 1 || (NB == 2 && KS == 1), "one or two channel blocks per MFMA wave");
     static_assert(KS == 1 || (KS == 4 && WM == 1 && WN == 1), "split-K: four waves share one 32-channel block");
     static_assert(KS == 4 || WM * WN == 4 || WM * WN == 8, "4 or 8 MFMA waves per workgroup");
@@ -191,7 +195,7 @@
                                          : (mp.total_tiles - (int)blockIdx.x + (int)gridDim.x - 1) / (int)gridDim.x;
     auto tile_of = [&](int it) {
         int i = it;
-        if ((blockIdx.x & 1) && my_rounds >= 3 && it >= my_rounds - 2) i = it == my_rounds - 1 ? my_rounds - 2 : my_rounds - 1;
+        if (!MRG && (blockIdx.x & 1) && my_rounds >= 3 && it >= my_rounds - 2) i = it == my_rounds - 1 ? my_rounds - 2 : my_rounds - 1;
         if (mp.sched_start) return scalar_load_i32(mp.sched_tiles + sched_lo + i);
         if (mp.xcd_order) {
             const int x = (int)blockIdx.x & 7, l = (int)blockIdx.x >> 3;
@@ -647,6 +651,60 @@
                 else if (has_y) pass(N, N, Y, N);
                 else pass(N, N, N, Y);
             }
+        }
+    };
+    auto epilogue_mrg = [&](const Tile& T, int nb, int rows_valid, const float (&bias_b)[4]) {
+        if constexpr (MRG) {
+            const ConvParams& p = mp.p[0];
+            const int rows_w = __builtin_amdgcn_readfirstlane(max(min(rows_valid - wave_row0, MI * 32), 0));
+            const unsigned pitch_b = __builtin_amdgcn_readfirstlane((unsigned)p.cout_total * 4u);
+            const size_t first = ((size_t)T.seq * p.L + T.t0 + wave_row0) * p.cout_total;
+            auto uni64 = [](unsigned long long v) {
+                const unsigned lo = __builtin_amdgcn_readfirstlane((unsigned)v), hi = __builtin_amdgcn_readfirstlane((unsigned)(v >> 32));
+                return ((unsigned long long)hi << 32) | lo;
+            };
+            const unsigned long long b_ys = uni64((unsigned long long)(reinterpret_cast<float*>(p.ys) + first));
+            auto rsrc_of = [&](unsigned long long base, int mi) {
+                const unsigned rows = (unsigned)max(min(rows_w - mi * 32, 32), 0);
+                return __builtin_amdgcn_make_buffer_rsrc((void*)uni64(base + (unsigned long long)(mi * 32) * pitch_b), 0,
+                                                         __builtin_amdgcn_readfirstlane(rows * pitch_b), 0x00020000);
+            };
+            const int voff = (int)((4u * g * p.cout_total + nb * 32 + li) * 4u);
+            int off16[16];
+#pragma unroll
+            for (int r = 0; r < 16; ++r) off16[r] = voff + (int)((8 * (r >> 2) + (r & 3)) * pitch_b);
+            const float slope_out = p.slope_out;
+            auto pass = [&](auto NBR) {
+                constexpr int N = decltype(NBR)::value;
+                float bias_sum = bias_b[0];
+#pragma unroll
+                for (int b = 1; b < N; ++b) bias_sum += bias_b[b];
+                unsigned long long b_res[N];
+#pragma unroll
+                for (int b = 0; b < N; ++b) b_res[b] = uni64((unsigned long long)(mp.p[b].res + first));
+#pragma unroll
+                for (int mi = 0; mi < MI; ++mi) {
+                    float rs[N][16];
+#pragma unroll
+                    for (int b = 0; b < N; ++b)
+#pragma unroll
+                        for (int r = 0; r < 16; ++r)
+                            rs[b][r] = __builtin_bit_cast(float, __builtin_amdgcn_raw_buffer_load_b32(rsrc_of(b_res[b], mi), off16[r], 0, 0));
+#pragma unroll
+                    for (int r = 0; r < 16; ++r) {
+                        float m = acc[0][mi][r] + bias_sum;
+#pragma unroll
+                        for (int b = 0; b < N; ++b) m += rs[b][r];
+                        m = m / (float)N;
+                        __builtin_amdgcn_raw_buffer_store_b32(__builtin_bit_cast(unsigned, __builtin_amdgcn_fmed3f(m, m * slope_out, __builtin_inff())),
+                                                              rsrc_of(b_ys, mi), off16[r], 0, 0);
+                    }
+                }
+            };
+            const int n = mp.n_branches;
+            if (n == 3) pass(std::integral_constant<int, 3>{});
+            else if (n == 2) pass(std::integral_constant<int, 2>{});
+            else pass(std::integral_constant<int, 4>{});
         }
     };
     auto bias_of = [&](const Tile& T) {
@@ -782,14 +840,25 @@
         if constexpr (!kPrimeOnce) {
             if (active && !primed) prime(T);
         }
-#pragma unroll
-        for (int q = 0; q < NB; ++q)
-#pragma unroll
-            for (int mi = 0; mi < MI; ++mi)
-#pragma unroll
-                for (int r = 0; r < 16; ++r) acc[q][mi][r] = 0.f;
+        if (!MRG || T.b == 0) {
+#pragma unroll
+            for (int q = 0; q < NB; ++q)
+#pragma unroll
+                for (int mi = 0; mi < MI; ++mi)
+#pragma unroll
+                    for (int r = 0; r < 16; ++r) acc[q][mi][r] = 0.f;
+        }
         float bias_l = 0.f;
-        if constexpr (kRowMajorAcc) bias_l = bias_of(T);
+        float bias_b[4] = {0.f, 0.f, 0.f, 0.f};
+        (void)bias_b;
+        const bool last_branch = !MRG || T.b == mp.n_branches - 1;
+        if constexpr (MRG) {
+            if (last_branch) {
+#pragma unroll
+                for (int b = 0; b < 4; ++b)
+                    if (b < mp.n_branches) bias_b[b] = mp.p[b].bias[(nb < p.n_blocks32 ? nb : 0) * 32 + li];
+            }
+        } else if constexpr (kRowMajorAcc) bias_l = bias_of(T);
 
         for (int c = 0; c < nchunks; ++c, ++j) {
             HIFICAR_STAMP(1 + 3 * j);
@@ -863,7 +932,9 @@
         }
         HIFICAR_STAMP(3 * j);
         primed = active;
-        if constexpr (kRowMajorAcc) {
+        if constexpr (MRG) {
+            if (active && last_branch) epilogue_mrg(T, nb, rows_valid_t, bias_b);
+        } else if constexpr (kRowMajorAcc) {
             if (active) epilogue_rm(T, p, nb, rows_valid_t, bias_l);
         } else if (active) {
             float* O = reinterpret_cast<float*>(smem_b + 2 * buf_bytes);
@@ -891,6 +962,11 @@
 template <int MI, int WM, int WN, int NC16>
 __global__ __launch_bounds__((WM * WN + 4) * 64) void conv_f32do_kernel(const MultiConvParams mp) {
     conv_ws_body<MI, WM, WN, NC16, true, 1, 1, true>(mp);
+}
+
+template <int MI, int WM, int WN, int NC16>
+__global__ __launch_bounds__((WM * WN + 4) * 64) void conv_f32mrg_kernel(const MergeConvParams mp) {
+    conv_ws_body<MI, WM, WN, NC16, true, 1, 1, true, true>(mp);
 }
 
 template <int MI, int WM, int WN, int NC16>
diff --git a/articulatory_amd/csrc/hificar_conv_inst.hip b/articulatory_amd/csrc/hificar_conv_inst.hip
--- a/articulatory_amd/csrc/hificar_conv_inst.hip
+++ b/articulatory_amd/csrc/hificar_conv_inst.hip
@@ -2,7 +2,7 @@
 #include "hificar_launch.h"
 
 #ifndef HIFICAR_INST_SET
-#error "compile with -DHIFICAR_INST_SET=0..9"
+#error "compile with -DHIFICAR_INST_SET=0..12"
 #endif
 
 namespace hificar {
@@ -55,6 +55,17 @@
 #define THREADS(wm, wn) 512
 #define PARAMS MultiConvParams
 #define SHAPES(X) X(1, 1, 1, 1) X(2, 1, 1, 1) X(4, 1, 1, 1) X(1, 1, 1, 2) X(2, 1, 1, 2) X(4, 1, 1, 2) X(1, 1, 1, 4) X(2, 1, 1, 4) X(4, 1, 1, 4)
+#elif HIFICAR_INST_SET >= 10 && HIFICAR_INST_SET <= 12
+#define FAMILY kConvF32mrg
+#define KERNEL conv_f32mrg_kernel
+#define PARAMS MergeConvParams
+#if HIFICAR_INST_SET == 10
+#define SHAPES(X) HIFICAR_TILES9(X, 1)
+#elif HIFICAR_INST_SET == 11
+#define SHAPES(X) HIFICAR_TILES9(X, 2)
+#else
+#define SHAPES(X) HIFICAR_TILES9(X, 4)
+#endif
 #elif HIFICAR_INST_SET == 9
 #define PARAMS PairParams
 #define THREADS(wm, wn) 512
diff --git a/articulatory_amd/csrc/hificar_launch.h b/articulatory_amd/csrc/hificar_launch.h
--- a/articulatory_amd/csrc/hificar_launch.h
+++ b/articulatory_amd/csrc/hificar_launch.h
@@ -4,6 +4,7 @@
 namespace hificar {
 
 struct MultiConvParams;
+struct MergeConvParams;
 struct PairParams;
 
 enum ConvFamily {
@@ -14,6 +15,7 @@
     kConvSkBf16x3 = 4,
     kPairF32 = 5,
     kPairBf16x3 = 6,
+    kConvF32mrg = 7,
 };
 
 struct ConvShape {
@@ -23,12 +25,13 @@
 hipError_t conv_launch(const ConvShape& s, const void* params, dim3 grid, size_t lds_bytes, hipStream_t stream);
 hipError_t conv_set_lds_attributes();
 
-#define HIFICAR_N_INST_SETS 10
+#define HIFICAR_N_INST_SETS 13
 #define HIFICAR_DECL_SET(n)                                                                                                              \
     hipError_t conv_inst_launch_##n(const ConvShape& s, const void* params, dim3 grid, size_t lds, hipStream_t stream, bool* handled); \
     hipError_t conv_inst_attrs_##n();
 HIFICAR_DECL_SET(0) HIFICAR_DECL_SET(1) HIFICAR_DECL_SET(2) HIFICAR_DECL_SET(3) HIFICAR_DECL_SET(4)
 HIFICAR_DECL_SET(5) HIFICAR_DECL_SET(6) HIFICAR_DECL_SET(7) HIFICAR_DECL_SET(8) HIFICAR_DECL_SET(9)
+HIFICAR_DECL_SET(10) HIFICAR_DECL_SET(11) HIFICAR_DECL_SET(12)
 #undef HIFICAR_DECL_SET
 
 }
```

After: 40.23 million samples/s, median of 6. +1.1%, better.
